# CouncilmanJeremyJamm/path_tracer

Hardware: AMD Instinct MI355X
Metric: Mray/s at 1920x1080, 256 spp; achieved HBM GB/s in traversal kernel (higher is better)
Workload: dtype f32; 1 GPU; Cornell box (36 triangles, 6 BLAS) 1920x1080, 256 spp, depth 8, NEE+MIS; parallelism=rows/1, bvh_in_lds=True, scene_bytes=4208

## Files before the change

include/pt_api.h:

```cpp
#ifndef PT_API_H
#define PT_API_H
#include <stdint.h>
#ifdef __cplusplus
extern "C" {
#endif

typedef struct pt_ctx pt_ctx;

enum pt_status
{
    PT_OK = 0,
    PT_ERR_ARG = -1,
    PT_ERR_HIP = -2,
    PT_ERR_STATE = -3,
    PT_ERR_NONRIGID = -4,
    PT_ERR_LIMIT = -5,
    PT_ERR_IO = -6,
    PT_ERR_PARSE = -7,
    PT_ERR_NCCL = -8
};

enum pt_material_kind
{
    PT_LAMBERTIAN = 0,
    PT_EMISSIVE = 1,
    PT_SPECULAR = 2,
    PT_GGX_METAL = 3,
    PT_GGX_DIELECTRIC = 4,
    PT_DIELECTRIC = 5
};

typedef struct pt_material_desc
{
    int32_t kind;
    float colour[3];
    float roughness;
    float ior;
    int32_t has_volume;
    float vol_absorption[3];
    float vol_k, vol_c, vol_g;
} pt_material_desc;

typedef struct pt_config
{
    uint32_t width, height;
    uint32_t max_bounces;
    uint32_t n_sobol;
    uint32_t enable_nee;
    uint64_t seed;
    uint32_t rank, world_size, strip_rows;
    uint32_t batch_spp;
    int32_t device;
    uint32_t flags;
    uint32_t stack_lds_levels;
    uint32_t queue_slack;
    uint32_t pipelines;
    uint32_t reserved;
} pt_config;

enum
{
    PT_FLAG_TIMING = 1u,
    PT_FLAG_NO_LDS_SCENE = 2u,
    PT_FLAG_TIMING_ALL = 4u,
    PT_FLAG_NO_PRIMARY_CULL = 8u
};

pt_ctx* pt_create(const pt_config* cfg);
void pt_destroy(pt_ctx* ctx);
const char* pt_last_error(pt_ctx* ctx);
int pt_set_config(pt_ctx* ctx, const pt_config* cfg);

int pt_add_material(pt_ctx* ctx, const pt_material_desc* desc);
int pt_add_model(pt_ctx* ctx, const float* positions_xyz, const float* normals_xyz, uint32_t n_tris, int material,
                 const float* affine3x4_rowmajor, uint32_t n_instances);
int pt_add_model_obj(pt_ctx* ctx, const char* path, int material, const float* affine3x4_rowmajor, uint32_t n_instances);
int pt_model_vertices(pt_ctx* ctx, int model, float* positions_xyz, float* normals_xyz, uint32_t cap_tris, uint32_t* n_tris);
int pt_build(pt_ctx* ctx);

int pt_set_camera(pt_ctx* ctx, const float eye[3], const float target[3], float fov_y_deg, float aspect);
enum pt_event { PT_EV_MOUSE_MOTION = 0, PT_EV_KEY_W = 1, PT_EV_KEY_S = 2, PT_EV_KEY_A = 3, PT_EV_KEY_D = 4 };
int pt_camera_input(pt_ctx* ctx, int event, float a, float b, float dt);
int pt_camera_angles(pt_ctx* ctx, float pitch_yaw[2]);
int pt_camera_matrices(pt_ctx* ctx, float cam_to_world_3x4[12], float inv_proj_4x4_colmajor[16]);
int pt_set_environment(pt_ctx* ctx, uint32_t width, uint32_t height, const float* rgb_linear);
int pt_create_ray(pt_ctx* ctx, float s, float t, float o[3], float d[3]);

int pt_render(pt_ctx* ctx, uint32_t first_sample, uint32_t n_samples, float* data_rgba, float* position_xyzt, uint32_t* id);
int pt_active_pixels(pt_ctx* ctx, uint32_t rect[4], float root_box[6]);
int pt_render_device(pt_ctx* ctx, uint32_t first_sample, uint32_t n_samples);
int pt_reset_accumulation(pt_ctx* ctx);
int pt_accum_device_ptr(pt_ctx* ctx, void** dev_ptr, uint64_t* n_pixels);
int pt_read_accumulation(pt_ctx* ctx, float* data_rgba);
int pt_read_frame(pt_ctx* ctx, float* data_rgba, float* position_xyzt, uint32_t* id);
int pt_write_accumulation(pt_ctx* ctx, const float* data_rgba, const float* position_xyzt, const uint32_t* id);
int pt_render_samples(pt_ctx* ctx, uint32_t first_sample, uint32_t n_samples, float* samples_rgba);
int pt_local_rows(pt_ctx* ctx, uint32_t* n_rows, uint32_t* rows, uint32_t cap);
int pt_set_stream(pt_ctx* ctx, void* hip_stream);
int pt_synchronize(pt_ctx* ctx);

int pt_frame(pt_ctx* ctx, uint32_t frame_index, const float* last_inv_projection, float* data_rgba, float* position_xyzt, uint32_t* id);
int pt_inv_projection(pt_ctx* ctx, float out16_colmajor[16]);
int pt_present(pt_ctx* ctx, float* rgba);
int pt_present_rgb8(pt_ctx* ctx, uint8_t* rgb);
int pt_write_image(pt_ctx* ctx, const char* path);
int pt_post_velocity(pt_ctx* ctx, uint32_t w, uint32_t h, const float* position, const float* last_inv_projection, float* velocity);
int pt_post_reproject(pt_ctx* ctx, uint32_t w, uint32_t h, const float* input, const float* accum, const float* velocity, const uint32_t* id,
                      float* output);
int pt_post_tonemap(pt_ctx* ctx, uint32_t w, uint32_t h, const float* accum, float* out);
int pt_post_rgb8(pt_ctx* ctx, uint32_t w, uint32_t h, const float* accum, uint8_t* rgb);

int pt_trace_closest(pt_ctx* ctx, int which, uint32_t n, const float* o_xyz, const float* d_xyz, const float* t_max, float* t,
                     float* u, float* v, uint32_t* inst, uint32_t* prim);
int pt_trace_any(pt_ctx* ctx, int which, uint32_t n, const float* o_xyz, const float* d_xyz, const float* t_max, uint8_t* hit);
int pt_ss_sobol(pt_ctx* ctx, uint32_t n_points, uint32_t n, const uint32_t* index, const uint32_t* seed, float* out_xy);
int pt_math_batch(pt_ctx* ctx, int fn, uint32_t n, const float* a, const float* b, float* out0, float* out1);
int pt_material_eval(pt_ctx* ctx, int material, uint32_t n, const float* incoming_xyz, const float* normal_xyz, const uint8_t* front,
                     const uint32_t* pixel, const uint32_t* sample, uint32_t draws_consumed, float* out9);
int pt_volume_eval(pt_ctx* ctx, int material, uint32_t n, const float* incoming_xyz, const float* t_max, const float* dist,
                   const uint32_t* pixel, const uint32_t* sample, uint32_t draws_consumed, float* out9);

int pt_blas_count(pt_ctx* ctx);
int pt_blas_dump(pt_ctx* ctx, int blas, uint32_t* n_nodes, uint32_t* root, float* boxes6, uint32_t* kind, uint32_t* a, uint32_t* b,
                 uint32_t* n_prim_ids, uint32_t* prim_ids, uint32_t cap_nodes, uint32_t cap_ids);
int pt_tlas_dump(pt_ctx* ctx, int which, uint32_t* n_nodes, uint32_t* root, float* boxes6, uint32_t* kind, uint32_t* a, uint32_t* b,
                 uint32_t cap_nodes);
int pt_tlas_instances(pt_ctx* ctx, int which, uint32_t* n, float* matrix12, float* inv_matrix12, uint32_t cap);
int pt_instance_materials(pt_ctx* ctx, int which, uint32_t* n, uint32_t* material, uint32_t* blas, uint32_t cap);
int pt_light_cdf(pt_ctx* ctx, uint32_t* n, float* pdf, float* cdf, uint32_t* blas, uint32_t* prim, float* max_weight, uint32_t cap);
int pt_triangle_dump(pt_ctx* ctx, int blas, uint32_t prim, float out36[36]);

typedef struct pt_multi pt_multi;
pt_multi* pt_multi_create(const pt_config* cfg, const int32_t* devices, uint32_t n_devices);
void pt_multi_destroy(pt_multi* m);
const char* pt_multi_last_error(pt_multi* m);
pt_ctx* pt_multi_ctx(pt_multi* m, uint32_t rank);
int pt_multi_render(pt_multi* m, uint32_t first_sample, uint32_t n_samples, float* data_rgba);
int pt_multi_framebuffer_device_ptr(pt_multi* m, void** dev_ptr);
int pt_multi_reset_accumulation(pt_multi* m);
int pt_multi_write_image(pt_multi* m, const char* path);
int pt_multi_used_rccl(pt_multi* m);

typedef struct pt_stats
{
    uint64_t rays_closest;
    uint64_t rays_any;
    uint64_t rays_light_closest;
    uint64_t paths;
    uint64_t launches_trace_closest;
    double ms_trace_closest;
    double ms_trace_any, ms_trace_light, ms_shade, ms_generate, ms_accumulate;
    double ms_total;
    uint64_t scene_bytes;
    uint32_t lds_scene;
    uint32_t stack_entries;
    uint64_t state_bytes;
    uint64_t rays_light_closest_traced;
    uint64_t rays_primary_culled;
} pt_stats;
int pt_get_stats(pt_ctx* ctx, pt_stats* out);
int pt_multi_get_stats(pt_multi* m, pt_stats* sum);
int pt_last_batch_counters(pt_ctx* ctx, uint32_t* rows16, uint32_t cap_rows, uint32_t* n_rows);
int pt_last_batch_shade_pids(pt_ctx* ctx, uint32_t qclass, uint32_t first, uint32_t count, uint32_t* pids);
int pt_last_batch_step_stats(pt_ctx* ctx, uint32_t* rows8, uint32_t cap_rows, uint32_t* n_rows);
int pt_reset_stats(pt_ctx* ctx);

#ifdef __cplusplus
}
#endif
#endif
```

path_tracer_amd/api.py:

```python
from __future__ import annotations

import ctypes as C
import os
from typing import Optional

import numpy as np

from . import build as _build
from .scene_desc import CameraDesc, SceneDesc

PT_OK = 0
FLAG_TIMING = 1
FLAG_NO_LDS_SCENE = 2
FLAG_TIMING_ALL = 4
FLAG_NO_PRIMARY_CULL = 8
DEFAULT_SEED = 0x5EED5EED

EXPORTS = [
    "pt_create", "pt_destroy", "pt_last_error", "pt_set_config", "pt_add_material", "pt_add_model", "pt_add_model_obj", "pt_model_vertices", "pt_build", "pt_set_camera",
    "pt_camera_matrices", "pt_set_environment", "pt_create_ray", "pt_render", "pt_render_device", "pt_reset_accumulation", "pt_accum_device_ptr",
    "pt_read_accumulation", "pt_read_frame", "pt_write_accumulation", "pt_render_samples", "pt_active_pixels", "pt_local_rows", "pt_set_stream", "pt_synchronize", "pt_camera_input", "pt_camera_angles", "pt_frame", "pt_inv_projection", "pt_present", "pt_post_velocity", "pt_post_reproject", "pt_post_tonemap", "pt_post_rgb8", "pt_present_rgb8", "pt_write_image", "pt_trace_closest", "pt_trace_any",
    "pt_ss_sobol", "pt_math_batch", "pt_material_eval", "pt_volume_eval", "pt_blas_count", "pt_blas_dump", "pt_tlas_dump", "pt_tlas_instances", "pt_instance_materials", "pt_light_cdf",
    "pt_triangle_dump", "pt_get_stats", "pt_reset_stats", "pt_last_batch_counters", "pt_last_batch_shade_pids", "pt_last_batch_step_stats",
    "pt_multi_create", "pt_multi_destroy", "pt_multi_last_error", "pt_multi_ctx", "pt_multi_render", "pt_multi_framebuffer_device_ptr",
    "pt_multi_reset_accumulation", "pt_multi_get_stats", "pt_multi_used_rccl", "pt_multi_write_image",
]


EV_MOUSE_MOTION, EV_KEY_W, EV_KEY_S, EV_KEY_A, EV_KEY_D = range(5)


class MaterialDesc(C.Structure):
    _fields_ = [("kind", C.c_int32), ("colour", C.c_float * 3), ("roughness", C.c_float), ("ior", C.c_float), ("has_volume", C.c_int32),
                ("vol_absorption", C.c_float * 3), ("vol_k", C.c_float), ("vol_c", C.c_float), ("vol_g", C.c_float)]


class Config(C.Structure):
    _fields_ = [("width", C.c_uint32), ("height", C.c_uint32), ("max_bounces", C.c_uint32), ("n_sobol", C.c_uint32),
                ("enable_nee", C.c_uint32), ("seed", C.c_uint64), ("rank", C.c_uint32), ("world_size", C.c_uint32),
                ("strip_rows", C.c_uint32), ("batch_spp", C.c_uint32), ("device", C.c_int32), ("flags", C.c_uint32),
                ("stack_lds_levels", C.c_uint32), ("queue_slack", C.c_uint32), ("pipelines", C.c_uint32), ("reserved", C.c_uint32)]


class Stats(C.Structure):
    _fields_ = [("rays_closest", C.c_uint64), ("rays_any", C.c_uint64), ("rays_light_closest", C.c_uint64), ("paths", C.c_uint64),
                ("launches_trace_closest", C.c_uint64), ("ms_trace_closest", C.c_double), ("ms_trace_any", C.c_double),
                ("ms_trace_light", C.c_double), ("ms_shade", C.c_double), ("ms_generate", C.c_double), ("ms_accumulate", C.c_double),
                ("ms_total", C.c_double), ("scene_bytes", C.c_uint64), ("lds_scene", C.c_uint32), ("stack_entries", C.c_uint32),
                ("state_bytes", C.c_uint64), ("rays_light_closest_traced", C.c_uint64), ("rays_primary_culled", C.c_uint64)]

    def as_dict(self):
        return {n: getattr(self, n) for n, _ in self._fields_}

    @property
    def rays(self):
        return self.rays_closest + self.rays_any + self.rays_light_closest


class PtError(RuntimeError):
    def __init__(self, code, msg):
        super().__init__(f"libptmi error {code}: {msg}")
        self.code = code


_lib = None


def lib():
    global _lib
    if _lib is None:
        path = os.environ.get("PTMI_LIB")
        if not path:
            path = _build.LIB_PATH
            if _build.is_stale():
                path = _build.build()
        try:
            import torch
        except ImportError:
            pass
        L = C.CDLL(path)
        vp, u32, f32p = C.c_void_p, C.c_uint32, C.c_void_p
        L.pt_create.restype = vp
        L.pt_create.argtypes = [C.POINTER(Config)]
        L.pt_destroy.argtypes = [vp]
        L.pt_last_error.restype = C.c_char_p
        L.pt_last_error.argtypes = [vp]
        L.pt_set_config.argtypes = [vp, C.POINTER(Config)]
        L.pt_add_material.argtypes = [vp, C.POINTER(MaterialDesc)]
        L.pt_add_model.argtypes = [vp, f32p, f32p, u32, C.c_int, f32p, u32]
        L.pt_add_model_obj.argtypes = [vp, C.c_char_p, C.c_int, f32p, u32]
        L.pt_model_vertices.argtypes = [vp, C.c_int, f32p, f32p, u32, C.POINTER(u32)]
        L.pt_build.argtypes = [vp]
        L.pt_set_camera.argtypes = [vp, C.POINTER(C.c_float), C.POINTER(C.c_float), C.c_float, C.c_float]
        L.pt_camera_matrices.argtypes = [vp, vp, vp]
        L.pt_set_environment.argtypes = [vp, u32, u32, vp]
        L.pt_create_ray.argtypes = [vp, C.c_float, C.c_float, vp, vp]
        L.pt_render.argtypes = [vp, u32, u32, vp, vp, vp]
        L.pt_render_device.argtypes = [vp, u32, u32]
        L.pt_active_pixels.argtypes = [vp, vp, vp]
        L.pt_reset_accumulation.argtypes = [vp]
        L.pt_accum_device_ptr.argtypes = [vp, C.POINTER(vp), C.POINTER(C.c_uint64)]
        L.pt_read_accumulation.argtypes = [vp, vp]
        L.pt_write_accumulation.argtypes = [vp, vp, vp, vp]
        L.pt_read_frame.argtypes = [vp, vp, vp, vp]
        L.pt_render_samples.argtypes = [vp, u32, u32, vp]
        L.pt_local_rows.argtypes = [vp, C.POINTER(u32), vp, u32]
        L.pt_set_stream.argtypes = [vp, vp]
        L.pt_synchronize.argtypes = [vp]
        L.pt_frame.argtypes = [vp, u32, vp, vp, vp, vp]
        L.pt_camera_input.argtypes = [vp, C.c_int, C.c_float, C.c_float, C.c_float]
        L.pt_camera_angles.argtypes = [vp, vp]
        L.pt_inv_projection.argtypes = [vp, vp]
        L.pt_present.argtypes = [vp, vp]
        L.pt_multi_create.restype = vp
        L.pt_multi_create.argtypes = [C.POINTER(Config), vp, u32]
        L.pt_multi_destroy.argtypes = [vp]
        L.pt_multi_last_error.restype = C.c_char_p
        L.pt_multi_last_error.argtypes = [vp]
        L.pt_multi_ctx.restype = vp
        L.pt_multi_ctx.argtypes = [vp, u32]
        L.pt_multi_render.argtypes = [vp, u32, u32, vp]
        L.pt_multi_framebuffer_device_ptr.argtypes = [vp, C.POINTER(vp)]
        L.pt_multi_reset_accumulation.argtypes = [vp]
        L.pt_multi_get_stats.argtypes = [vp, C.POINTER(Stats)]
        L.pt_multi_used_rccl.argtypes = [vp]
        L.pt_multi_write_image.argtypes = [vp, C.c_char_p]
        L.pt_post_velocity.argtypes = [vp, u32, u32, vp, vp, vp]
        L.pt_post_reproject.argtypes = [vp, u32, u32, vp, vp, vp, vp, vp]
        L.pt_post_tonemap.argtypes = [vp, u32, u32, vp, vp]
        L.pt_post_rgb8.argtypes = [vp, u32, u32, vp, vp]
        L.pt_present_rgb8.argtypes = [vp, vp]
        L.pt_write_image.argtypes = [vp, C.c_char_p]
# ... 440 lines not shown
```

path_tracer_amd/csrc/pt_api.cpp:

```cpp
#include "../../include/pt_api.h"

#include <hip/hip_runtime.h>

#include <algorithm>
#include <chrono>
#include <cmath>
#include <cstdio>
#include <cstdlib>
#include <cstring>
#include <mutex>
#include <string>
#include <vector>

#include "pt_kernels.h"
#include "pt_png.h"
#include "pt_scene.h"

using namespace pt;

#ifndef PT_SHADE_BLOCKS_PER_CU
#define PT_SHADE_BLOCKS_PER_CU 16
#endif
#ifndef PT_JOIN_LATE
#define PT_JOIN_LATE 0
// ... 7 lines not shown
#ifndef PT_SIDE_MIN_PATHS
#define PT_SIDE_MIN_PATHS (4u << 20)
#endif
#ifndef PT_SIDE_PRIORITY
#define PT_SIDE_PRIORITY 0
#endif
#ifndef PT_SPLIT_MIN_PATHS
#define PT_SPLIT_MIN_PATHS (24u << 20)
#endif
#ifndef PT_SPLIT_MIN_PATHS_LDS
#define PT_SPLIT_MIN_PATHS_LDS (24u << 20)
#endif
#ifndef PT_PIPES4_MIN_PATHS
#define PT_PIPES4_MIN_PATHS (~0ull)
#endif
#ifndef PT_PID_BLOCK
#define PT_PID_BLOCK 16
#endif
#ifndef PT_FUSED_TRACE
#define PT_FUSED_TRACE 1
#endif
#ifndef PT_TRACE_BLOCKS_PER_CU_MAX
#define PT_TRACE_BLOCKS_PER_CU_MAX 8
#endif

namespace {

enum TimeCat { T_GEN = 0, T_WORLD, T_ANY, T_LIGHT, T_SHADE, T_ACCUM, T_COUNT };

struct DevBuf
{
    void* p = nullptr;
    size_t bytes = 0;
};

}

struct pt_ctx
{
    pt_config cfg{};
    HostScene scene;
    std::string err;
    std::mutex mu;

    bool dev_ready = false;
    int device = 0;
    int n_cus = 256;
    hipStream_t own_stream = nullptr, stream = nullptr;
    hipEvent_t ev_start = nullptr;

    struct Pipe
    {
        hipStream_t own_stream = nullptr, side_stream = nullptr;
        hipEvent_t ev_fork = nullptr, ev_join = nullptr, ev_done = nullptr;
        size_t cap_paths = 0, cap_slots = 0, cap_slots_term = 0;
        uint32_t cap_rows = 0;
        std::vector<DevBuf> pool;
        WavefrontBuffers wb{};
        Counters* h_counters = nullptr;
        uint32_t* h_heads = nullptr;
        struct Ev { hipEvent_t a, b; int cat; };
        std::vector<Ev> ev_pool;
        size_t ev_used = 0;
        uint32_t slack_cfg = 0;
        uint32_t pixels_cfg = 0;
        size_t state_bytes = 0;
        bool busy = false;
        uint32_t busy_rows = 0;
        uint64_t busy_paths = 0, busy_culled = 0;
    };
    static constexpr int kMaxPipes = 4;
    Pipe pipe[kMaxPipes];
    hipStream_t pipe_stream(int i) const { return i == 0 ? stream : pipe[i].own_stream; }

    bool scene_uploaded = false;
    DevBuf d_spill;
    size_t spill_region_words = 0;
    DevBuf d_blob, d_tri_shade, d_tri_pos, d_tri_orig, d_materials, d_lights, d_env;
    std::vector<f4> h_env;
    uint32_t env_w = 0, env_h = 0;
    bool env_uploaded = false;
    SceneView sv{};
    bool lds_scene = false;
    uint32_t block_threads = 256, trace_blocks = 1024;
    bool class_present[Q_COUNT] = {true, false, false, false, false};

    std::vector<uint32_t> rows;
    uint32_t local_pixels = 0;
    uint32_t pad_rows = 0;
    uint64_t scene_version = 0;
    DevBuf d_accum, d_position, d_id;
    DevBuf d_input, d_velocity, d_output;

    pt_stats stats{};
    int last_pipe = 0;
};

namespace {

int fail(pt_ctx* c, int code, const std::string& msg)
{
    c->err = msg;
    return code;
}

#define HIPCHK(c, call)                                                                                       \
    do {                                                                                                      \
        hipError_t e__ = (call);                                                                              \
        if (e__ != hipSuccess) return fail((c), PT_ERR_HIP, std::string(#call) + ": " + hipGetErrorString(e__)); \
    } while (0)

void dev_free(DevBuf& b)
{
    if (b.p) (void)hipFree(b.p);
    b = DevBuf();
}
int dev_alloc(pt_ctx* c, DevBuf& b, size_t bytes)
{
    if (b.bytes >= bytes && b.p) return PT_OK;
    dev_free(b);
    bytes = std::max<size_t>(bytes, 16);
    HIPCHK(c, hipMalloc(&b.p, bytes));
    b.bytes = bytes;
    return PT_OK;
}

void compute_rows(pt_ctx* c)
{
    const pt_config& g = c->cfg;
    c->rows.clear();
    const uint32_t world = std::max(1u, g.world_size), strip = std::max(1u, g.strip_rows);
    for (uint32_t y = 0; y < g.height; ++y)
        if ((y / strip) % world == g.rank) c->rows.push_back(y);
    c->local_pixels = (uint32_t)c->rows.size() * g.width;
    uint32_t r0 = 0;
    for (uint32_t y = 0; y < g.height; ++y) r0 += ((y / strip) % world == 0u) ? 1u : 0u;
    c->pad_rows = r0;
}

int normalise_config(pt_ctx* c, const pt_config* in)
{
    pt_config g = *in;
    if (g.width == 0 || g.height == 0) return fail(c, PT_ERR_ARG, "width/height must be non-zero");
    if (g.n_sobol == 0) g.n_sobol = 512;
    if (g.world_size == 0) g.world_size = 1;
    if (g.strip_rows == 0) g.strip_rows = 4;
    if (g.rank >= g.world_size) return fail(c, PT_ERR_ARG, "rank >= world_size");
    if ((uint64_t)g.width * g.height > 0x7fffffffull) return fail(c, PT_ERR_ARG, "image too large");
    c->cfg = g;
    compute_rows(c);
    return PT_OK;
}

int ensure_device(pt_ctx* c)
{
    if (c->dev_ready)
    {
        HIPCHK(c, hipSetDevice(c->device));
        return PT_OK;
    }
    int n = 0;
    hipError_t e = hipGetDeviceCount(&n);
    if (e != hipSuccess || n == 0) return fail(c, PT_ERR_HIP, "no HIP device available (libptmi has no CPU path)");
    if (c->cfg.device >= 0) HIPCHK(c, hipSetDevice(c->cfg.device));
    HIPCHK(c, hipGetDevice(&c->device));
    hipDeviceProp_t prop;
    HIPCHK(c, hipGetDeviceProperties(&prop, c->device));
    c->n_cus = prop.multiProcessorCount > 0 ? prop.multiProcessorCount : 256;
    HIPCHK(c, hipStreamCreateWithFlags(&c->own_stream, hipStreamNonBlocking));
    HIPCHK(c, hipEventCreateWithFlags(&c->ev_start, hipEventDisableTiming));
    for (int i = 0; i < pt_ctx::kMaxPipes; ++i)
    {
        pt_ctx::Pipe& pp = c->pipe[i];
        if (i > 0) HIPCHK(c, hipStreamCreateWithFlags(&pp.own_stream, hipStreamNonBlocking));
        HIPCHK(c, hipStreamCreateWithFlags(&pp.side_stream, hipStreamNonBlocking));
        HIPCHK(c, hipEventCreateWithFlags(&pp.ev_fork, hipEventDisableTiming));
        HIPCHK(c, hipEventCreateWithFlags(&pp.ev_join, hipEventDisableTiming));
        HIPCHK(c, hipEventCreateWithFlags(&pp.ev_done, hipEventDisableTiming));
    }
    if (!c->stream) c->stream = c->own_stream;
    c->dev_ready = true;
    return PT_OK;
}

int upload_scene(pt_ctx* c)
{
    if (c->scene_uploaded) return ensure_device(c);
    if (!c->scene.built) return fail(c, PT_ERR_STATE, "pt_build has not been called");
    int r = ensure_device(c);
    if (r) return r;
    const FlatScene& f = c->scene.flat;
    const size_t nb = f.nodes.size() * sizeof(DNode), tb = f.tri_isect.size() * sizeof(DTriIsect), ib = f.instances.size() * sizeof(DInstance);
    const size_t lb = (f.big_leaves.size() * 4 + 15) / 16 * 16;
    std::vector<uint8_t> blob(nb + tb + ib + lb);
    std::memcpy(blob.data(), f.nodes.data(), nb);
    std::memcpy(blob.data() + nb, f.tri_isect.data(), tb);
    std::memcpy(blob.data() + nb + tb, f.instances.data(), ib);
    if (lb) std::memcpy(blob.data() + nb + tb + ib, f.big_leaves.data(), f.big_leaves.size() * 4);
    if ((r = dev_alloc(c, c->d_blob, blob.size()))) return r;
    HIPCHK(c, hipMemcpy(c->d_blob.p, blob.data(), blob.size(), hipMemcpyHostToDevice));
    auto up = [&](DevBuf& b, const void* src, size_t bytes) -> int {
        int rr = dev_alloc(c, b, bytes);
        if (rr) return rr;
        if (bytes) HIPCHK(c, hipMemcpy(b.p, src, bytes, hipMemcpyHostToDevice));
        return PT_OK;
    };
    if ((r = up(c->d_tri_shade, f.tri_shade.data(), f.tri_shade.size() * sizeof(DTriVerts)))) return r;
    if ((r = up(c->d_tri_pos, f.tri_pos.data(), f.tri_pos.size() * sizeof(DTriVerts)))) return r;
    if ((r = up(c->d_tri_orig, f.tri_orig.data(), f.tri_orig.size() * 4))) return r;
    if ((r = up(c->d_materials, f.materials.data(), f.materials.size() * sizeof(DMaterial)))) return r;
    if ((r = up(c->d_lights, f.lights.data(), f.lights.size() * sizeof(DLight)))) return r;

    SceneView& sv = c->sv;
    uint8_t* base = (uint8_t*)c->d_blob.p;
    sv.nodes = (const DNode*)base;
    sv.tri_isect = (const DTriIsect*)(base + nb);
    sv.instances = (const DInstance*)(base + nb + tb);
    sv.tri_shade = (const DTriVerts*)c->d_tri_shade.p;
    sv.tri_pos = (const DTriVerts*)c->d_tri_pos.p;
    sv.tri_orig = (const uint32_t*)c->d_tri_orig.p;
    sv.materials = (const DMaterial*)c->d_materials.p;
    sv.lights = (const DLight*)c->d_lights.p;
    sv.n_nodes = (uint32_t)f.nodes.size();
    sv.n_tris = (uint32_t)f.tri_isect.size();
    sv.n_instances = (uint32_t)f.instances.size();
    sv.n_materials = (uint32_t)f.materials.size();
    sv.n_lights = (uint32_t)f.lights.size();
    sv.world_root = f.world_root;
    sv.lights_root = f.lights_root;
    sv.prim_bits = f.prim_bits;
    sv.light_weight_sum = f.light_weight_sum;
    sv.blob_bytes = (uint32_t)blob.size();
    sv.stack_entries = f.stack_entries;
    sv.has_volumes = f.has_volumes ? 1u : 0u;

    c->lds_scene = blob.size() <= 48 * 1024 && !(c->cfg.flags & PT_FLAG_NO_LDS_SCENE);
    uint32_t threads = 256;
#ifndef PT_STACK_LDS_LEVELS
#define PT_STACK_LDS_LEVELS 14
#endif
    sv.stack_lds = std::min<uint32_t>(sv.stack_entries, c->cfg.stack_lds_levels ? c->cfg.stack_lds_levels : PT_STACK_LDS_LEVELS);
    auto lds_need = [&](uint32_t t) { return trace_lds_bytes(c->lds_scene, sv.blob_bytes, sv.stack_lds, t); };
    while (threads > 64 && lds_need(threads) > 64 * 1024) threads >>= 1;
    if (lds_need(threads) > 160 * 1024) return fail(c, PT_ERR_LIMIT, "BVH too deep for the LDS traversal stack");
    c->block_threads = threads;
    const size_t lds = lds_need(threads);
    uint32_t per_cu = (uint32_t)std::min<size_t>((160 * 1024) / std::max<size_t>(lds, 1), 2048 / threads);
    per_cu = std::max(1u, std::min(per_cu, (uint32_t)PT_TRACE_BLOCKS_PER_CU_MAX));
    c->trace_blocks = (uint32_t)c->n_cus * per_cu;
    sv.stack_spill = nullptr;
    if (sv.stack_entries > sv.stack_lds)
    {
        const size_t lanes = (size_t)c->trace_blocks * threads;
        c->spill_region_words = (size_t)(sv.stack_entries - sv.stack_lds) * lanes;
        if ((r = dev_alloc(c, c->d_spill, 2 * pt_ctx::kMaxPipes * c->spill_region_words * 8))) return r;
        sv.stack_spill = (uint64_t*)c->d_spill.p;
    }

    for (uint32_t q = 0; q < Q_COUNT; ++q) c->class_present[q] = (q == Q_TERMINAL);
    for (const DInstance& in : f.instances) c->class_present[in.qclass & 0xffu] = true;
    c->scene_uploaded = true;
    c->stats.scene_bytes = blob.size();
    c->stats.lds_scene = c->lds_scene;
    c->stats.stack_entries = sv.stack_entries;
    return PT_OK;
}

TraceLaunch trace_launch(pt_ctx* c, int pipe = 0, bool side_stream = false)
{
    TraceLaunch tl;
    tl.scene = c->sv;
    if (tl.scene.stack_spill) tl.scene.stack_spill += (size_t)(2 * pipe + (side_stream ? 1 : 0)) * c->spill_region_words;
    tl.blob = c->d_blob.p;
    tl.lds_scene = c->lds_scene;
    tl.grid_blocks = c->trace_blocks;
    tl.n_cus = (uint32_t)c->n_cus;
    tl.block_threads = c->block_threads;
    return tl;
}

struct ActiveRect { uint32_t x0, w, ly0, rows; };
ActiveRect active_rect(pt_ctx* c)
{
    const uint32_t W = c->cfg.width, H = c->cfg.height, local_rows = (uint32_t)c->rows.size();
    const ActiveRect full{0u, W, 0u, local_rows};
    if ((c->cfg.flags & PT_FLAG_NO_PRIMARY_CULL) || c->env_w || !c->scene.built || !c->scene.camera.set) return full;
    const FlatScene& f = c->scene.flat;
    if (f.world_root == MISS_ID || f.world_root >= f.nodes.size()) return full;
    const DNode& root = f.nodes[f.world_root];
    double m[16], inv[16];
    for (int i = 0; i < 16; ++i) m[i] = c->scene.camera.ray_matrix[i];
    {
        double a[4][8];
        for (int r = 0; r < 4; ++r)
            for (int k = 0; k < 4; ++k) { a[r][k] = m[k * 4 + r]; a[r][4 + k] = r == k ? 1.0 : 0.0; }
        for (int col = 0; col < 4; ++col)
        {
            int piv = col;
            for (int r = col + 1; r < 4; ++r)
                if (std::fabs(a[r][col]) > std::fabs(a[piv][col])) piv = r;
            if (std::fabs(a[piv][col]) < 1e-300) return full;
            for (int k = 0; k < 8; ++k) std::swap(a[col][k], a[piv][k]);
            const double d = a[col][col];
            for (int k = 0; k < 8; ++k) a[col][k] /= d;
            for (int r = 0; r < 4; ++r)
                if (r != col)
                {
                    const double fct = a[r][col];
                    for (int k = 0; k < 8; ++k) a[r][k] -= fct * a[col][k];
                }
        }
        for (int r = 0; r < 4; ++r)
            for (int k = 0; k < 4; ++k) inv[k * 4 + r] = a[r][4 + k];
    }
    const double eye[3] = {c->scene.camera.matrix.t.x, c->scene.camera.matrix.t.y, c->scene.camera.matrix.t.z};
    double ctr[4];
    for (int r = 0; r < 4; ++r) ctr[r] = m[12 + r];
    if (!(std::fabs(ctr[3]) > 1e-300)) return full;
    double fwd[3] = {ctr[0] / ctr[3] - eye[0], ctr[1] / ctr[3] - eye[1], ctr[2] / ctr[3] - eye[2]};
    const double fl = std::sqrt(fwd[0] * fwd[0] + fwd[1] * fwd[1] + fwd[2] * fwd[2]);
    if (!(fl > 0.0) || !std::isfinite(fl)) return full;
    double ext = 0.0;
    for (int k = 0; k < 3; ++k) { fwd[k] /= fl; ext = std::max(ext, std::fabs((double)root.mx[k] - (double)root.mn[k])); }
    double px_lo = 1e300, px_hi = -1e300, py_lo = 1e300, py_hi = -1e300;
    for (int corner = 0; corner < 8; ++corner)
    {
        const double X[3] = {corner & 1 ? root.mx[0] : root.mn[0], corner & 2 ? root.mx[1] : root.mn[1], corner & 4 ? root.mx[2] : root.mn[2]};
        if (!std::isfinite(X[0]) || !std::isfinite(X[1]) || !std::isfinite(X[2])) return full;
        const double depth = (X[0] - eye[0]) * fwd[0] + (X[1] - eye[1]) * fwd[1] + (X[2] - eye[2]) * fwd[2];
        if (!(depth > 1e-3 * ext + 1e-6)) return full;
        double q[4];
        for (int r = 0; r < 4; ++r) q[r] = inv[r] * X[0] + inv[4 + r] * X[1] + inv[8 + r] * X[2] + inv[12 + r];
        if (!(std::fabs(q[3]) > 1e-300)) return full;
        const double nx = q[0] / q[3], ny = q[1] / q[3];
        if (!std::isfinite(nx) || !std::isfinite(ny)) return full;
        const double px = (nx + 1.0) * 0.5 * W, py = (ny + 1.0) * 0.5 * H;
        px_lo = std::min(px_lo, px); px_hi = std::max(px_hi, px);
        py_lo = std::min(py_lo, py); py_hi = std::max(py_hi, py);
    }
    const double margin = 3.0;
    const double gx0 = std::floor(px_lo - 0.5 - margin), gx1 = std::ceil(px_hi + 0.5 + margin) + 1.0;
    const double gy0 = std::floor(py_lo - 0.5 - margin), gy1 = std::ceil(py_hi + 0.5 + margin) + 1.0;
    const uint32_t x0 = (uint32_t)std::min<double>(std::max(gx0, 0.0), W), x1 = (uint32_t)std::min<double>(std::max(gx1, 0.0), W);
    const uint32_t y0 = (uint32_t)std::min<double>(std::max(gy0, 0.0), H), y1 = (uint32_t)std::min<double>(std::max(gy1, 0.0), H);
    uint32_t ly0 = 0, n = 0;
    while (ly0 < local_rows && c->rows[ly0] < y0) ++ly0;
    while (ly0 + n < local_rows && c->rows[ly0 + n] < y1) ++n;
    return ActiveRect{x0, x1 > x0 ? x1 - x0 : 0u, ly0, n};
}

int ensure_frame(pt_ctx* c)
{
    int r;
    const size_t px = std::max<size_t>(std::max<size_t>(c->local_pixels, (size_t)c->pad_rows * c->cfg.width), 1);
    const bool fresh = c->d_accum.bytes < px * 16;
    if ((r = dev_alloc(c, c->d_accum, px * 16))) return r;
    if ((r = dev_alloc(c, c->d_position, px * 16))) return r;
// ... 1537 lines not shown
        std::lock_guard<std::mutex> lk(g_rccl_mu);
        std::string e;
        if (!g_rccl.load(&e)) return mfail(m, PT_ERR_NCCL, e);
        if (m->comms.empty())
        {
            m->comms.resize(n);
            const ncclResult_t nr = g_rccl.CommInitAll(m->comms.data(), (int)n, m->devices.data());
            if (nr != ncclSuccess) { m->comms.clear(); return mfail(m, PT_ERR_NCCL, std::string("ncclCommInitAll: ") + g_rccl.GetErrorString(nr)); }
        }
        ncclResult_t nr = g_rccl.GroupStart();
        for (size_t i = 0; i < n && nr == ncclSuccess; ++i)
        {
            pt_ctx* c = m->ctx[i];
            if (hipSetDevice(c->device) != hipSuccess) { nr = ncclUnhandledCudaError; break; }
            nr = g_rccl.Gather(c->d_accum.p, i == 0 ? m->d_parts.p : nullptr, part_px * 4, ncclFloat, 0, m->comms[i], c->stream);
        }
        const ncclResult_t ne = g_rccl.GroupEnd();
        if (nr == ncclSuccess) nr = ne;
        if (nr != ncclSuccess) return mfail(m, PT_ERR_NCCL, std::string("ncclGather: ") + g_rccl.GetErrorString(nr));
        m->used_rccl = true;
        for (size_t i = 1; i < n; ++i)
        {
            MHIPCHK(m, hipSetDevice(m->ctx[i]->device));
            MHIPCHK(m, hipStreamSynchronize(m->ctx[i]->stream));
        }
        MHIPCHK(m, hipSetDevice(c0->device));
    }
    else
    {
        for (size_t i = 0; i < n; ++i)
            MHIPCHK(m, hipMemcpyAsync((uint8_t*)m->d_parts.p + i * part_px * 16, m->ctx[i]->d_accum.p, part_px * 16, hipMemcpyDeviceToDevice, c0->stream));
    }
    launch_post_deinterleave(c0->stream, g.width, g.height, (uint32_t)n, g.strip_rows, c0->pad_rows, (const f4*)m->d_parts.p, (f4*)m->d_full.p);
    if (data_rgba) MHIPCHK(m, hipMemcpyAsync(data_rgba, m->d_full.p, full_px * 16, hipMemcpyDeviceToHost, c0->stream));
    MHIPCHK(m, hipStreamSynchronize(c0->stream));
    MHIPCHK(m, hipGetLastError());
    return PT_OK;
}

int pt_multi_write_image(pt_multi* m, const char* path)
{
    if (!m || !path) return PT_ERR_ARG;
    if (!m->d_full.p) return mfail(m, PT_ERR_STATE, "pt_multi_render has not been called");
    pt_ctx* c0 = m->ctx[0];
    const size_t px = (size_t)c0->cfg.width * c0->cfg.height;
    MHIPCHK(m, hipSetDevice(c0->device));
    DevBuf d_rgb;
    int r = dev_alloc(c0, d_rgb, px * 3);
    if (r) return mfail(m, r, pt_last_error(c0));
    launch_post_rgb8(c0->stream, (uint32_t)px, (const f4*)m->d_full.p, (uint8_t*)d_rgb.p);
    std::vector<uint8_t> host(px * 3);
    hipError_t e = hipMemcpyAsync(host.data(), d_rgb.p, px * 3, hipMemcpyDeviceToHost, c0->stream);
    if (e == hipSuccess) e = hipStreamSynchronize(c0->stream);
    dev_free(d_rgb);
    if (e != hipSuccess) return mfail(m, PT_ERR_HIP, hipGetErrorString(e));
    std::string err;
    if (!write_png_rgb8(path, host.data(), c0->cfg.width, c0->cfg.height, &err)) return mfail(m, PT_ERR_IO, err);
    return PT_OK;
}

int pt_multi_framebuffer_device_ptr(pt_multi* m, void** dev_ptr)
{
    if (!m || !dev_ptr) return PT_ERR_ARG;
    if (!m->d_full.p) return mfail(m, PT_ERR_STATE, "pt_multi_render has not been called");
    *dev_ptr = m->d_full.p;
    return PT_OK;
}

int pt_multi_get_stats(pt_multi* m, pt_stats* sum)
{
    if (!m || !sum) return PT_ERR_ARG;
    *sum = pt_stats();
    for (pt_ctx* c : m->ctx)
    {
        const pt_stats& s = c->stats;
        sum->rays_closest += s.rays_closest; sum->rays_any += s.rays_any; sum->rays_light_closest += s.rays_light_closest;
        sum->rays_light_closest_traced += s.rays_light_closest_traced; sum->rays_primary_culled += s.rays_primary_culled; sum->paths += s.paths;
        sum->launches_trace_closest += s.launches_trace_closest; sum->ms_trace_closest += s.ms_trace_closest;
        sum->ms_trace_any += s.ms_trace_any; sum->ms_trace_light += s.ms_trace_light; sum->ms_shade += s.ms_shade;
        sum->ms_generate += s.ms_generate; sum->ms_accumulate += s.ms_accumulate;
        sum->ms_total = std::max(sum->ms_total, s.ms_total);
        sum->state_bytes += s.state_bytes;
        sum->scene_bytes = s.scene_bytes; sum->lds_scene = s.lds_scene; sum->stack_entries = s.stack_entries;
    }
    return PT_OK;
}

int pt_get_stats(pt_ctx* c, pt_stats* out)
{
    if (!c || !out) return PT_ERR_ARG;
    *out = c->stats;
    return PT_OK;
}

int pt_last_batch_counters(pt_ctx* c, uint32_t* rows16, uint32_t cap_rows, uint32_t* n_rows)
{
    if (!c || !rows16 || !n_rows) return PT_ERR_ARG;
    const pt_ctx::Pipe& pp = c->pipe[c->last_pipe];
    if (!pp.h_counters || !pp.h_heads) return PT_ERR_STATE;
    const uint32_t rows = std::min(cap_rows, c->cfg.max_bounces + 2);
    const uint32_t have = std::min(rows, pp.busy_rows);
    std::memset(rows16, 0, (size_t)rows * sizeof(Counters));
    std::memcpy(rows16, pp.h_counters, (size_t)have * sizeof(Counters));
    for (uint32_t r = 0; r < have; ++r)
    {
        uint32_t* o = rows16 + 16 * r;
        o[1] = o[3] = o[5] = 0;
        o[6] = o[7] = o[13] = o[14] = o[15] = 0;
        const uint32_t* hrow = pp.h_heads + (size_t)r * HEADS_PER_ROW * kHeadWordsPerQueue;
        for (uint32_t g = 0; g < kQueueHeads; ++g)
        {
            const uint32_t* cl = hrow + HEADS_CLOSEST * kHeadWordsPerQueue + g * kHeadStrideWords;
            const uint32_t* sh = hrow + HEADS_SHADOW * kHeadWordsPerQueue + g * kHeadStrideWords;
            const uint32_t* lc = hrow + HEADS_LCHAIN * kHeadWordsPerQueue + g * kHeadStrideWords;
            o[6] += lc[HEAD_TALLY0]; o[7] += lc[HEAD_TALLY1]; o[13] += cl[HEAD_TALLY0]; o[14] += sh[HEAD_TALLY0]; o[15] += lc[HEAD_TALLY2];
        }
    }
    *n_rows = rows;
    return PT_OK;
}

int pt_last_batch_shade_pids(pt_ctx* c, uint32_t qclass, uint32_t first, uint32_t count, uint32_t* pids)
{
    if (!c || !pids || qclass == Q_TERMINAL || qclass >= Q_COUNT) return PT_ERR_ARG;
    const pt_ctx::Pipe& pp = c->pipe[c->last_pipe];
    if (!pp.wb.q_shade_base || !((pp.wb.class_mask >> qclass) & 1u)) return PT_ERR_STATE;
    if ((uint64_t)first + count > pp.wb.q_stride) return PT_ERR_ARG;
    HIPCHK(c, hipSetDevice(c->device));
    const ShadeQueue q = shade_queue(pp.wb, qclass);
    HIPCHK(c, hipMemcpy2D(pids, 4, reinterpret_cast<const uint8_t*>(q.a + first) + 12, 16, 4, count, hipMemcpyDeviceToHost));
    return PT_OK;
}

int pt_last_batch_step_stats(pt_ctx* c, uint32_t* rows8, uint32_t cap_rows, uint32_t* n_rows)
{
    if (!c || !rows8 || !n_rows) return PT_ERR_ARG;
    const pt_ctx::Pipe& pp = c->pipe[c->last_pipe];
    if (!pp.h_heads) return PT_ERR_STATE;
    const uint32_t rows = std::min(cap_rows, c->cfg.max_bounces + 2);
#if PT_WAVE_TIMES
    {
        std::vector<uint32_t> rec((size_t)rows * kWaveTimeSlots * 4);
        const char* which = std::getenv("PTMI_WAVE_TIMES_KERNEL");
        const uint4* src = (which && which[0] == 'a') ? pp.wb.wave_times_any : pp.wb.wave_times;
        if (hipMemcpy(rec.data(), src, rec.size() * 4, hipMemcpyDeviceToHost) != hipSuccess) return PT_ERR_HIP;
        for (uint32_t r = 0; r < rows; ++r)
        {
            uint32_t* o = rows8 + 8 * r;
            std::memset(o, 0, 32);
            uint32_t t0 = 0; bool any = false;
            for (uint32_t w = 0; w < kWaveTimeSlots; ++w)
            {
                const uint32_t* q = &rec[((size_t)r * kWaveTimeSlots + w) * 4];
                if (q[3] == 0u) continue;
                if (!any || (int32_t)(q[0] - t0) < 0) t0 = q[0];
                any = true;
            }
            if (!any) continue;
            uint32_t max_end = 0, min_dr = 0xffffffffu, max_dr = 0;
            for (uint32_t w = 0; w < kWaveTimeSlots; ++w)
            {
                const uint32_t* q = &rec[((size_t)r * kWaveTimeSlots + w) * 4];
                if (q[3] == 0u) continue;
                max_end = std::max(max_end, q[3] - t0);
                min_dr = std::min(min_dr, q[2] - t0);
                max_dr = std::max(max_dr, q[2] - t0);
                o[2] += q[3] - q[0];
                o[3] += q[2] - q[0];
                o[4] += 1u;
                o[7] += q[1] - q[0];
            }
            o[0] = ~t0; o[1] = t0 + max_end; o[5] = ~(t0 + min_dr); o[6] = t0 + max_dr;
            if (std::getenv("PTMI_WAVE_TIMES_DUMP"))
            {
// ... 46 lines not shown
```

path_tracer_amd/csrc/pt_kernels.h:

```cpp
#pragma once
#include <hip/hip_runtime.h>

#include "pt_materials.h"
#include "pt_types.h"

namespace pt {

struct TraceLaunch
{
    SceneView scene;
    const void* blob;
    bool lds_scene;
    uint32_t grid_blocks;
    uint32_t n_cus;
    uint32_t block_threads;
};

inline size_t trace_lds_bytes(bool lds_scene, uint32_t blob_bytes, uint32_t stack_lds, uint32_t block_threads)
{
    return (lds_scene ? (size_t)blob_bytes : 0) + (size_t)stack_lds * block_threads * 8;
}
inline size_t trace_lds_bytes(const TraceLaunch& tl) { return trace_lds_bytes(tl.lds_scene, tl.scene.blob_bytes, tl.scene.stack_lds, tl.block_threads); }

struct WavefrontBuffers
{
    PathState st;
    RayQueue rq[2];
    RayQueue rq_shadow;
    RayQueue rq_lchain[2];
    f4* lchain_nb[2];
    f4* lchain_hit;
    f4* hits;
    f4* q_shade_base;
    uint32_t q_stride;
    uint32_t q_class_slot;
    uint2* q_term[2];
    Counters* counters;
    uint32_t* heads;
    uint4* wave_times;
    uint4* wave_times_any;
    uint32_t* tails;
    uint32_t cap_slots;
    uint32_t cap_slots_shade;
    uint32_t cap_slots_term;
    uint32_t class_mask;
};

inline ShadeQueue shade_queue(const WavefrontBuffers& wb, uint32_t q)
{
    const size_t slot = (wb.q_class_slot >> (4u * q)) & 0xfu;
    f4* a = wb.q_shade_base + 3u * slot * (size_t)wb.q_stride;
    return ShadeQueue{a, a + wb.q_stride, a + 2u * (size_t)wb.q_stride};
}

void launch_generate(hipStream_t s, const RenderParams& rp, const CameraView& cam, const WavefrontBuffers& wb);
void launch_trace_world(hipStream_t s, const TraceLaunch& tl, const WavefrontBuffers& wb, uint32_t b, const RenderParams& rp, const CameraView& cam,
                        const EnvView& env);
void launch_trace_fused(hipStream_t s, const TraceLaunch& tl, const WavefrontBuffers& wb, uint32_t b, const RenderParams& rp, const EnvView& env);
void launch_trace_shadow(hipStream_t s, const TraceLaunch& tl, const WavefrontBuffers& wb, uint32_t b);
void launch_trace_lchain(hipStream_t s, const TraceLaunch& tl, const WavefrontBuffers& wb, uint32_t b);
void launch_shade(hipStream_t s, uint32_t qclass, const SceneView& sv, const RenderParams& rp, const WavefrontBuffers& wb, uint32_t b,
                  uint32_t grid_blocks, const CameraView& cam, const EnvView& env, const TraceLaunch* tl = nullptr);
bool shade_traces_shadow(const TraceLaunch& tl);
void launch_accumulate(hipStream_t s, const RenderParams& rp, const CameraView& cam, const WavefrontBuffers& wb, f4* accum, f4* position, uint32_t* id,
                       uint32_t write_position, uint32_t add_to_accum);
void launch_store_samples(hipStream_t s, const RenderParams& rp, const WavefrontBuffers& wb, f4* out);

void launch_post_accumulate(hipStream_t s, uint32_t n, const f4* input, f4* accum);
void launch_post_velocity(hipStream_t s, int w, int h, const f4* position, const float* m16, float* velocity_xy);
void launch_post_reproject(hipStream_t s, int w, int h, const f4* input, const f4* accum, const float* velocity_xy, const uint32_t* id, f4* output);
void launch_post_tonemap(hipStream_t s, uint32_t n, const f4* accum, f4* out);
void launch_post_rgb8(hipStream_t s, uint32_t n, const f4* accum, uint8_t* out);
void launch_post_deinterleave(hipStream_t s, uint32_t w, uint32_t h, uint32_t world, uint32_t strip, uint32_t pad_rows, const f4* parts, f4* full);

void launch_trace_rays_closest(hipStream_t s, const TraceLaunch& tl, uint32_t root, RayQueue rq, uint32_t n, uint32_t* n_and_heads, f4* hits);
void launch_trace_rays_any(hipStream_t s, const TraceLaunch& tl, uint32_t root, RayQueue rq, uint32_t n, uint32_t* n_and_heads, uint32_t* occluded);
void launch_sobol_probe(hipStream_t s, uint32_t n_points, uint32_t n, const uint32_t* index, const uint32_t* seed, float* out_xy);
void launch_math_probe(hipStream_t s, int fn, uint32_t n, const float* a, const float* b, float* o0, float* o1, uint64_t seed);
void launch_material_probe(hipStream_t s, const SceneView& sv, int material, uint32_t n, const float* incoming, const float* normal,
                           const uint8_t* front, const uint32_t* pixel, const uint32_t* sample, uint32_t draws, uint64_t seed, float* out9);
void launch_volume_probe(hipStream_t s, const SceneView& sv, int material, uint32_t n, const float* incoming, const float* t_max, const float* dist,
                         const uint32_t* pixel, const uint32_t* sample, uint32_t draws, uint64_t seed, float* out9);

}
```

path_tracer_amd/csrc/pt_kernels.hip:

```cpp
#include "pt_kernels.h"
#include "pt_materials.h"

#include <algorithm>
#include <mutex>
#include <vector>

namespace pt {
namespace {

#ifndef PT_STEPS_PER_ROUND
#define PT_STEPS_PER_ROUND 8
#endif
#ifndef PT_REFILL_BELOW
#define PT_REFILL_BELOW 40
#endif
#ifndef PT_STEPS_PER_ROUND_GLOBAL_BVH
#define PT_STEPS_PER_ROUND_GLOBAL_BVH 4
#endif
#ifndef PT_REFILL_BELOW_GLOBAL_BVH
#define PT_REFILL_BELOW_GLOBAL_BVH 56
#endif
#ifndef PT_STEPS_ANY
#define PT_STEPS_ANY 4
#endif
#ifndef PT_REFILL_BELOW_ANY
#define PT_REFILL_BELOW_ANY PT_REFILL_BELOW
#endif
#ifndef PT_WAVES_LDS_BVH
#define PT_WAVES_LDS_BVH 5
#endif
#ifndef PT_WAVES_LDS_BVH_ANY
#define PT_WAVES_LDS_BVH_ANY 5
#endif
#ifndef PT_WAVES_GLOBAL_BVH
#define PT_WAVES_GLOBAL_BVH 5
#endif
#ifndef PT_WAVES_GLOBAL_BVH_ANY
#define PT_WAVES_GLOBAL_BVH_ANY 5
#endif
#ifndef PT_BRANCH_LEVELS
#define PT_BRANCH_LEVELS 4
#endif
#ifndef PT_BRANCH_LEVELS_ANY
#define PT_BRANCH_LEVELS_ANY 4
#endif
#ifndef PT_BRANCH_LEVELS_INLINE
#define PT_BRANCH_LEVELS_INLINE 6
#endif
#ifndef PT_ACC_QUAD_BELOW
#define PT_ACC_QUAD_BELOW (1u << 30)
#endif
#ifndef PT_STEP_STATS
#define PT_STEP_STATS 0
#endif
#ifndef PT_WAVE_TIMES
#define PT_WAVE_TIMES 0
#endif
#ifndef PT_MIN_GENERATIONS
#define PT_MIN_GENERATIONS 1
#endif
#ifndef PT_STRIPE_DIV
#define PT_STRIPE_DIV 64
#endif
#ifndef PT_REGIONS_PER_STRIPE
#define PT_REGIONS_PER_STRIPE 256
#endif
#ifndef PT_REGION_DIV
#define PT_REGION_DIV 16
#endif
#ifndef PT_TAPER
#define PT_TAPER 2
#endif
#ifndef PT_TAPER_ANY
#define PT_TAPER_ANY 0
#endif
#ifndef PT_RESERVICE
#define PT_RESERVICE 1
#endif
#ifndef PT_CLAIM_AHEAD
#define PT_CLAIM_AHEAD 0
#endif
#ifndef PT_SHADE_WAVES
#define PT_SHADE_WAVES 5
#endif
#ifndef PT_SHADE_WAVES_DIEL
#define PT_SHADE_WAVES_DIEL 5
#endif
#ifndef PT_SHADE_WAVES_GGX
#define PT_SHADE_WAVES_GGX 5
#endif
#ifndef PT_SHADE_WAVES_VOLUMES
#define PT_SHADE_WAVES_VOLUMES 4
#endif
constexpr int shade_waves(uint32_t qclass, bool volumes)
{
    return volumes ? PT_SHADE_WAVES_VOLUMES : (qclass == Q_GGX ? PT_SHADE_WAVES_GGX : (qclass == Q_DIELECTRIC ? PT_SHADE_WAVES_DIEL : PT_SHADE_WAVES));
}
#ifndef PT_INLINE_SHADOW
#define PT_INLINE_SHADOW 1
#endif
#ifndef PT_SHADE_WAVES_INLINE
#define PT_SHADE_WAVES_INLINE 5
#endif
#ifndef PT_SHADE_THREADS
#define PT_SHADE_THREADS 256
#endif
#ifndef PT_CHUNK_MAX
#define PT_CHUNK_MAX 1024
#endif
#ifndef PT_CHUNK_DIV
#define PT_CHUNK_DIV 4
#endif
#ifndef PT_CHUNK_DIV_GLOBAL_BVH
#define PT_CHUNK_DIV_GLOBAL_BVH 16
#endif
template <bool LDS_SCENE> struct Refill
{
    static constexpr int kSteps = LDS_SCENE ? PT_STEPS_PER_ROUND : PT_STEPS_PER_ROUND_GLOBAL_BVH;
    static constexpr int kStepsAny = LDS_SCENE ? PT_STEPS_ANY : PT_STEPS_PER_ROUND_GLOBAL_BVH;
    static constexpr int kBelow = LDS_SCENE ? PT_REFILL_BELOW : PT_REFILL_BELOW_GLOBAL_BVH;
    static constexpr int kBelowAny = LDS_SCENE ? PT_REFILL_BELOW_ANY : PT_REFILL_BELOW_GLOBAL_BVH;
};

__device__ __forceinline__ uint32_t fastdiv(uint32_t n, const FastDiv& f)
{
    const uint32_t q = __umulhi(f.magic, n);
    const uint32_t t = ((n - q) >> 1) + q;
    return f.one ? n : (t >> f.shift);
}
__device__ __forceinline__ uint32_t lane_id() { return threadIdx.x & 63u; }
__device__ __forceinline__ uint32_t mbcnt64(uint64_t m)
{
    return __builtin_amdgcn_mbcnt_hi((uint32_t)(m >> 32), __builtin_amdgcn_mbcnt_lo((uint32_t)m, 0u));
}
struct FetchPlan
{
    uint32_t n;
    uint32_t chunk;
    uint32_t n_static;
    uint32_t psize;
    uint32_t lvl;
    uint32_t blocks;
};
__device__ __forceinline__ bool chunk_of(const FetchPlan& pl, uint32_t i, uint32_t& start, uint32_t& len)
{
    uint32_t rem = pl.psize, base = 0u;
    const uint32_t e64 = min(rem, pl.lvl); rem -= e64;
    const uint32_t e128 = min(rem, 2u * pl.lvl); rem -= e128;
    const uint32_t e256 = min(rem, 4u * pl.lvl); rem -= e256;
    const uint32_t e512 = min(rem, 8u * pl.lvl); rem -= e512;
    const uint32_t e1024 = rem;
#define PT_LEVEL(E, C)                                                                                     \
    {                                                                                                      \
        const uint32_t c = min((uint32_t)(C), pl.chunk), cnt = ((E) + c - 1u) / c;                          \
        if (i < cnt) { start = base + i * c; len = min(c, (E) - i * c); return true; }                      \
        i -= cnt;                                                                                          \
        base += (E);                                                                                       \
    }
    PT_LEVEL(e1024, 1024u) PT_LEVEL(e512, 512u) PT_LEVEL(e256, 256u) PT_LEVEL(e128, 128u) PT_LEVEL(e64, 64u)
#undef PT_LEVEL
    return false;
}
__device__ __forceinline__ FetchPlan fetch_plan(uint32_t n, uint32_t chunk_div, uint32_t taper)
{
    FetchPlan pl;
    const uint32_t wpb = blockDim.x >> 6;
    const uint32_t need_waves = (n + 63u) >> 6;
    pl.blocks = min(gridDim.x, (need_waves + wpb * (uint32_t)PT_MIN_GENERATIONS - 1u) / (wpb * (uint32_t)PT_MIN_GENERATIONS));
    const uint32_t waves = max(pl.blocks, 1u) * wpb;
    uint32_t c = n / (waves * chunk_div);
    c = c < 64u ? 64u : (c > (uint32_t)PT_CHUNK_MAX ? (uint32_t)PT_CHUNK_MAX : c);
    pl.chunk = (c + 63u) & ~63u;
    pl.n = n;
    const uint64_t st = (uint64_t)waves * pl.chunk;
    pl.n_static = st >= n ? n : (uint32_t)st;
    const uint32_t units = (n - pl.n_static + 63u) >> 6;
    pl.psize = ((units + kQueueHeads - 1u) / kQueueHeads) << 6;
    pl.lvl = taper ? ((taper * waves * 64u / kQueueHeads + 63u) & ~63u) : 0u;
    return pl;
}
struct WaveRange
{
// ... 250 lines not shown
    td = -dot4(f4{mo.x, mo.y, mo.z, -1.0f}, n0);
    const bool out_t = sign_differs(td - det * t_min, det * t_mx - td);
    const f3 p = det * mo + td * d;
    const f4 p4{p.x, p.y, p.z, det};
    ud = dot4(p4, f4{asf(p1.x), asf(p1.y), asf(p1.z), asf(p1.w)});
    const bool out_u = sign_differs(ud, det - ud);
    vd = dot4(p4, f4{asf(p2.x), asf(p2.y), asf(p2.z), asf(p2.w)});
    const bool out_v = sign_differs(vd, det - ud - vd);
    return !(out_t | out_u | out_v);
}

struct TriEval { float td, ud, vd, det; bool uv_ok; };
__device__ __forceinline__ TriEval tri_eval(const uint4* tp, const f3 mo, const f3 d)
{
    TriEval e;
    const uint4 p0 = tp[0], p1 = tp[1], p2 = tp[2];
    const f4 n0{asf(p0.x), asf(p0.y), asf(p0.z), asf(p0.w)};
    e.det = dot3(d, xyz(n0));
    e.td = -dot4(f4{mo.x, mo.y, mo.z, -1.0f}, n0);
    const f3 p = e.det * mo + e.td * d;
    const f4 p4{p.x, p.y, p.z, e.det};
    e.ud = dot4(p4, f4{asf(p1.x), asf(p1.y), asf(p1.z), asf(p1.w)});
    e.vd = dot4(p4, f4{asf(p2.x), asf(p2.y), asf(p2.z), asf(p2.w)});
    const bool out_u = sign_differs(e.ud, e.det - e.ud), out_v = sign_differs(e.vd, e.det - e.ud - e.vd);
    e.uv_ok = !out_u && !out_v;
    return e;
}
__device__ __forceinline__ bool tri_in_range(const TriEval& e, float t_min, float t_mx) { return !sign_differs(e.td - e.det * t_min, e.det * t_mx - e.td); }

struct Blob
{
    const uint4* nodes;
    const uint4* tris;
    const uint4* inst;
    const uint2* leaves;
};
__device__ __forceinline__ void leaf_range(const Blob& bl, uint32_t kind, uint32_t payload, uint32_t& first, uint32_t& count)
{
    if (kind == NODE_TRIS) { first = payload & LEAF_FIRST_MASK; count = (payload >> LEAF_FIRST_BITS) + 1u; }
    else { const uint2 lf = bl.leaves[payload]; first = lf.x; count = lf.y; }
}

struct LaneRay { f3 o, d, inv; };

__device__ __forceinline__ void pin(uint4& v) { asm volatile("" : "+v"(v.x), "+v"(v.y), "+v"(v.z), "+v"(v.w)); }
template <bool EAGER, bool ROOT_BOX>
__device__ __forceinline__ LaneRay to_object(const Blob& bl, uint32_t inst, const LaneRay& w, bool ray_finite, uint4& root0, uint4& root1)
{
    const uint4* ip = bl.inst + INST_WORDS * inst;
    uint4 r0, r1, r2;
    if (EAGER)
    {
        r0 = ip[0]; r1 = ip[1]; r2 = ip[2];
    }
    const uint4 meta = ip[INST_META_WORD];
    if (ROOT_BOX) { root0 = ip[INST_ROOT_WORD]; root1 = ip[INST_ROOT_WORD + 1u]; }
    else root0.w = reinterpret_cast<const uint32_t*>(ip + INST_ROOT_WORD)[3];
    if (EAGER) { pin(r0); pin(r1); pin(r2); }
    LaneRay r;
    if ((meta.w & INSTANCE_IDENTITY) != 0u && ray_finite)
    {
        const uint32_t so = asu(w.o.x) & asu(w.o.y) & asu(w.o.z) & 0x80000000u;
        const uint32_t sd = asu(w.d.x) & asu(w.d.y) & asu(w.d.z) & 0x80000000u;
        r.o.x = w.o.x != 0.0f ? w.o.x : asf(so);
        r.o.y = w.o.y != 0.0f ? w.o.y : asf(so);
        r.o.z = w.o.z != 0.0f ? w.o.z : asf(so);
        r.d.x = w.d.x != 0.0f ? w.d.x : asf(sd);
        r.d.y = w.d.y != 0.0f ? w.d.y : asf(sd);
        r.d.z = w.d.z != 0.0f ? w.d.z : asf(sd);
        r.inv.x = w.d.x != 0.0f ? w.inv.x : asf(sd | 0x7f800000u);
        r.inv.y = w.d.y != 0.0f ? w.inv.y : asf(sd | 0x7f800000u);
        r.inv.z = w.d.z != 0.0f ? w.inv.z : asf(sd | 0x7f800000u);
        return r;
    }
    if (!EAGER) { r0 = ip[0]; r1 = ip[1]; r2 = ip[2]; }
    r.o.x = ((asf(r0.x) * w.o.x + asf(r0.y) * w.o.y) + asf(r0.z) * w.o.z) + asf(r0.w);
    r.o.y = ((asf(r1.x) * w.o.x + asf(r1.y) * w.o.y) + asf(r1.z) * w.o.z) + asf(r1.w);
    r.o.z = ((asf(r2.x) * w.o.x + asf(r2.y) * w.o.y) + asf(r2.z) * w.o.z) + asf(r2.w);
    r.d.x = (asf(r0.x) * w.d.x + asf(r0.y) * w.d.y) + asf(r0.z) * w.d.z;
    r.d.y = (asf(r1.x) * w.d.x + asf(r1.y) * w.d.y) + asf(r1.z) * w.d.z;
    r.d.z = (asf(r2.x) * w.d.x + asf(r2.y) * w.d.y) + asf(r2.z) * w.d.z;
    r.inv = rcp3(r.d);
    return r;
}

template <bool LDS_SCENE>
__device__ __forceinline__ Blob stage_scene(const SceneView& sv, const uint4* __restrict__ gblob, uint4* smem, uint32_t& words)
{
    Blob b;
    const uint4* base = gblob;
    words = 0;
    if (LDS_SCENE)
    {
        words = sv.blob_bytes >> 4;
        for (uint32_t i = threadIdx.x; i < words; i += blockDim.x) smem[i] = gblob[i];
        __syncthreads();
        base = smem;
    }
    b.nodes = base;
    b.tris = base + 2u * sv.n_nodes;
    b.inst = base + 2u * sv.n_nodes + 3u * sv.n_tris;
    b.leaves = reinterpret_cast<const uint2*>(base + 2u * sv.n_nodes + 3u * sv.n_tris + INST_WORDS * sv.n_instances);
    return b;
}

enum { CLOSEST_WORLD = 0, CLOSEST_LIGHTS = 1, CLOSEST_HOOK = 2, CLOSEST_PRIMARY = 3 };

struct ClosestOut
{
    f4* hits;
    f4* q_base;
    uint32_t q_stride, q_class_slot;
    uint2* q_term;
    uint32_t* n_shade;
    uint4* wave_times;
    uint32_t* tails;
    uint32_t cap_shade, cap_term;
    uint32_t class_mask;
    uint32_t* overflow;
    uint32_t world_root;
    uint8_t* occl;
    f3 eye;
    f4* radiance;
    f4* first_pos;
    uint32_t* first_id;
    uint32_t keep_s_id, keep_s_pos, blk_log, n_blk, blk_last, act_pixels;
    FastDiv div_blk_paths, div_blk_last;
    uint32_t finalize_miss;
    const DPathRec* rec;
    uint32_t enable_nee;
};

template <bool SPILL>
struct Stack8;
template <>
struct Stack8<false>
{
    char* base;
    uint32_t bottom, step;
    __device__ __forceinline__ static Stack8 make(uint4* smem, uint32_t blob_words, const SceneView&)
    {
        return Stack8{reinterpret_cast<char*>(smem), blob_words * 16u + threadIdx.x * 8u, blockDim.x * 8u};
    }
    __device__ __forceinline__ uint32_t empty() const { return bottom; }
    __device__ __forceinline__ uint32_t up(uint32_t sp) const { return sp + step; }
    __device__ __forceinline__ uint32_t down(uint32_t sp) const { return sp - step; }
    __device__ __forceinline__ uint2 get(uint32_t sp) const { return *reinterpret_cast<const uint2*>(base + sp); }
    __device__ __forceinline__ void put(uint32_t sp, uint2 v) const { *reinterpret_cast<uint2*>(base + sp) = v; }
};
template <>
struct Stack8<true>
{
    uint2* lds;
    uint2* spill;
    uint32_t stride, lds_levels, spill_stride;
    __device__ __forceinline__ static Stack8 make(uint4* smem, uint32_t blob_words, const SceneView& sv)
    {
        return Stack8{reinterpret_cast<uint2*>(smem + blob_words) + threadIdx.x,
                      reinterpret_cast<uint2*>(sv.stack_spill) + (blockIdx.x * blockDim.x + threadIdx.x), blockDim.x, sv.stack_lds, gridDim.x * blockDim.x};
    }
    __device__ __forceinline__ uint32_t empty() const { return 0u; }
    __device__ __forceinline__ uint32_t up(uint32_t sp) const { return sp + 1u; }
    __device__ __forceinline__ uint32_t down(uint32_t sp) const { return sp - 1u; }
    __device__ __forceinline__ uint2 get(uint32_t sp) const
    {
        uint2 v;
        if (sp < lds_levels) v = lds[__umul24(sp, stride)];
        else v = spill[(size_t)(sp - lds_levels) * spill_stride];
        return v;
    }
    __device__ __forceinline__ void put(uint32_t sp, uint2 v) const
    {
        if (sp < lds_levels) lds[__umul24(sp, stride)] = v;
        else spill[(size_t)(sp - lds_levels) * spill_stride] = v;
    }
};

#if PT_WAVE_TIMES
__device__ uint4* g_any_times = nullptr;
#endif
struct ClosestKArgs
{
    SceneView sv;
    const uint4* gblob;
    const f4* ra;
    const f4* rb;
    const uint32_t* n_ptr;
    uint32_t* heads;
    uint32_t root, cap_in;
    ClosestOut out;
};
typedef const __attribute__((address_space(4))) ClosestKArgs* ClosestKArgsPtr;
typedef const __attribute__((address_space(4))) ClosestOut* ClosestOutPtr;
__device__ __forceinline__ ClosestOutPtr launder_args(ClosestOutPtr p)
{
    asm volatile("" : "+s"(p));
    return p;
}
template <int BVH, int MODE, bool SPILL>
__device__ __forceinline__ void closest_body(const SceneView& sv, const Blob& bl, const uint32_t blob_words, uint4* smem, const uint32_t root, const f4* __restrict__ ra,
                                             const f4* __restrict__ rb, const uint32_t* __restrict__ n_ptr, const uint32_t cap_in,
                                             uint32_t* __restrict__ heads, const ClosestOutPtr outp)
{
    constexpr bool LDS_SCENE = BVH != 0;
    const FetchPlan plan = fetch_plan(min(*n_ptr, cap_in), LDS_SCENE ? (uint32_t)PT_CHUNK_DIV : (uint32_t)PT_CHUNK_DIV_GLOBAL_BVH, (uint32_t)PT_TAPER);
    if (blockIdx.x >= plan.blocks) return;
    const Stack8<SPILL> stk = Stack8<SPILL>::make(smem, blob_words, sv);
    const uint32_t prim_bits = sv.prim_bits;

    bool active = false, pending = false, ray_finite = false;
    uint32_t ray_idx = 0, pid = 0;
    LaneRay w{}, ob{};
    float t_max = 0.0f, bt = 0.0f;
    float hud = 0.0f, hvd = 0.0f, hdet = 1.0f;
    uint32_t bid = MISS_ID, sp = stk.empty(), blas_base = 0, inst = 0;
    bool in_blas = false;
    bool any_phase = false;
    uint32_t chain_code = 0u;
    WaveRange wr = first_range(plan, heads);
    uint32_t light_hits = 0, valid_rays = 0;
#if PT_STEP_STATS
    uint32_t st_iter = 0, st_lane_active = 0, st_lane_inst = 0, st_lane_branch = 0, st_lane_leaf = 0, st_wave_inst = 0, st_wave_branch = 0, st_wave_leaf = 0;
#endif
#if PT_WAVE_TIMES
    const uint32_t tw_start = (uint32_t)wall_clock64();
    uint32_t tw_first = 0u, tw_drained = 0u;
#endif
    Region bin_region[Q_COUNT];
#pragma unroll
    for (uint32_t c = 0; c < Q_COUNT; ++c) bin_region[c] = Region{0u, 0u};
    const uint32_t lights_world_root = MODE == CLOSEST_LIGHTS ? outp->world_root : 0u;
    const uint32_t rsize = outp->finalize_miss != 0u ? 64u : region_size(plan.n, plan.blocks * (blockDim.x >> 6), 64u);
    const Stripes stripes = stripes_for(plan.n);
    uint32_t stripe_rot = blockIdx.x * (blockDim.x >> 6) + __builtin_amdgcn_readfirstlane(threadIdx.x >> 6);

    for (;;)
    {
        uint64_t act = __ballot(active);
        const bool no_more = wr.drained && wr.cur >= wr.end;
#if PT_WAVE_TIMES
        if (no_more && tw_drained == 0u) tw_drained = (uint32_t)wall_clock64() | 1u;
#endif
        const bool service = no_more ? (act == 0ull) : (__popcll(act) <= Refill<LDS_SCENE>::kBelow);
        if (service)
        {
            const ClosestOutPtr out = launder_args(outp);
            const uint64_t pm = __ballot(pending);
            if (pm != 0ull)
            {
                if (MODE == CLOSEST_WORLD || MODE == CLOSEST_PRIMARY)
                {
                    uint64_t qm = pm;
                    if (MODE == CLOSEST_PRIMARY)
                    {
                        const bool missed = pending && bid == MISS_ID && out->finalize_miss != 0u;
                        if (pending) out->occl[ray_idx] = missed ? (uint8_t)PRIMARY_MISS : (uint8_t)0u;
                        if (!missed && pending && bid == MISS_ID)
                        {
                            const FastDiv dbp{out->div_blk_paths.magic, out->div_blk_paths.shift, out->div_blk_paths.one, out->div_blk_paths.d};
                            const FastDiv dbl{out->div_blk_last.magic, out->div_blk_last.shift, out->div_blk_last.one, out->div_blk_last.d};
                            const uint32_t b = fastdiv(ray_idx, dbp), rem = ray_idx - b * (out->act_pixels << out->blk_log);
                            const bool short_blk = b + 1u == out->n_blk;
                            const uint32_t k = short_blk ? fastdiv(rem, dbl) : (rem >> out->blk_log);
                            const uint32_t sl = (b << out->blk_log) + (rem - k * (short_blk ? out->blk_last : (1u << out->blk_log)));
                            if (sl >= out->keep_s_id) out->first_id[(sl - out->keep_s_id) * out->act_pixels + k] = 255u;
                            if (sl == out->keep_s_pos)
                            {
                                const f3 far = fma3(w.d, bc3(1e5f), w.o);
                                out->first_pos[k] = f4{far.x, far.y, far.z, 1e5f};
                            }
                        }
                        qm = __ballot(pending && !missed);
                        pending = pending && !missed;
                    }
                    if (MODE == CLOSEST_WORLD)
                    {
                        bool ends = false, emissive = false;
                        uint32_t mat_id = 0;
                        if (pending)
                        {
                            if (bid == MISS_ID) ends = out->finalize_miss != 0u;
                            else
                            {
                                const uint4 meta = bl.inst[INST_WORDS * (bid >> prim_bits) + INST_META_WORD];
                                emissive = ends = (meta.w & 0xffu) == (uint32_t)Q_TERMINAL;
                                mat_id = meta.z;
                            }
                        }
                        if (ends)
                        {
                            const DPathRec& rec = out->rec[pid];
                            const f4 acc4 = rec.acc;
                            const uint32_t flags = asu(acc4.w);
                            if (!(flags & FLAG_BSDF_CAST))
                            {
                                f3 acc = xyz(acc4);
                                if (flags & FLAG_NEE_PENDING) acc = acc + xyz(rec.nee_pw) * (xyz(rec.nee_e) + f3{0.0f, 0.0f, 0.0f});
                                const f3 pw = xyz(rec.pw);
                                if (!emissive) acc = acc + f3{0.006f, 0.006f, 0.006f} * pw;
                                else if (!out->enable_nee || (flags & FLAG_LAST_DELTA))
                                {
                                    const DMaterial& m = sv.materials[mat_id];
                                    acc = fma3(f3{m.colour[0], m.colour[1], m.colour[2]}, pw, acc);
                                }
                                out->radiance[pid] = f4{acc.x, acc.y, acc.z, 0.0f};
                                pending = false;
                            }
                        }
                        qm = __ballot(pending);
                    }
                    if (qm != 0ull)
                    {
                        uint32_t cls = Q_COUNT;
                        if (pending) cls = bid != MISS_ID ? (bl.inst[INST_WORDS * (bid >> prim_bits) + INST_META_WORD].w & 0xffu) : (uint32_t)Q_TERMINAL;
                        const f4 hit{bt, hud / hdet, hvd / hdet, asf(bid)};
#pragma unroll
                        for (uint32_t c = 0; c < Q_COUNT; ++c)
                        {
                            if (!((out->class_mask >> c) & 1u)) continue;
                            const uint64_t m = __ballot(cls == c);
                            if (m == 0ull) continue;
                            const Placement pl = c == Q_TERMINAL
                                ? wave_reserve(bin_region[c], out->n_shade + c, (uint32_t)__popcll(m), rsize, out->cap_term, out->overflow)
                                : wave_reserve_striped(bin_region[c], out->tails + c * kTailWordsPerQueue, stripes, stripe_rot, (uint32_t)__popcll(m), out->cap_shade, out->overflow);
                            if (cls == c)
                            {
                                const uint32_t pos = place(pl, mbcnt64(m));
                                if (c == Q_TERMINAL)
                                {
                                    out->hits[ray_idx] = hit;
                                    out->q_term[pos] = make_uint2(ray_idx, pid);
                                }
                                else
                                {
                                    f4* const qa = out->q_base + (size_t)(3u * ((out->q_class_slot >> (4u * c)) & 0xfu)) * out->q_stride + pos;
                                    nt_store(qa, f4{w.d.x, w.d.y, w.d.z, asf(pid)});
                                    nt_store(qa + out->q_stride, hit);
                                    if (MODE != CLOSEST_PRIMARY) nt_store(qa + 2u * (size_t)out->q_stride, f4{w.o.x, w.o.y, w.o.z, 0.0f});
                                }
                            }
                        }
                    }
                }
                else if (MODE == CLOSEST_LIGHTS)
                {
                    if (pending)
                    {
                        out->occl[pid] = (uint8_t)chain_code;
                        if (chain_code == 0u) out->hits[ray_idx] = f4{bt, hud / hdet, hvd / hdet, asf(bid)};
                    }
                }
                else
                {
                    if (pending) out->hits[ray_idx] = f4{bt, hud / hdet, hvd / hdet, asf(bid)};
                }
                pending = false;
            }
            if (no_more) break;
            const uint64_t idle = ~act;
            uint32_t first;
            const uint32_t take = claim_rays(wr, heads, plan, (uint32_t)__popcll(idle), first);
            const uint32_t rank = mbcnt64(idle);
            if (!active && rank < take)
            {
                const uint32_t mine = first + rank;
                const f4 b = rb[mine];
                ray_idx = mine;
                pid = asu(b.w);
                if (pid != HOLE) {
                valid_rays += 1u;
                if (MODE == CLOSEST_PRIMARY)
                {
                    w.o = f3{out->eye.x, out->eye.y, out->eye.z};
                    t_max = asf(0x7f800000u);
                }
                else
                {
                    const f4 a = ra[mine];
                    w.o = xyz(a);
                    t_max = a.w;
                }
                w.d = xyz(b);
                w.inv = rcp3(w.d);
                ray_finite = finite3(w.o) && finite3(w.d);
                bid = MISS_ID;
                any_phase = false;
                chain_code = 2u;
                bt = asf(0x7f800000u);
                hud = 0.0f;
                hvd = 0.0f;
                hdet = 1.0f;
                in_blas = false;
                sp = stk.empty();
                float te;
                const uint4 root0 = bl.nodes[2u * root];
                const bool ok = (t_max == t_max) && slab(root0, bl.nodes[2u * root + 1u], w.o, w.inv, t_max, te);
                if (ok)
                {
                    stk.put(sp, make_uint2(root0.w, 0u));
                    sp = stk.up(sp);
                    active = true;
                }
                else { pending = true; }
                }
            }
#if PT_WAVE_TIMES
            if (tw_first == 0u && take != 0u) tw_first = (uint32_t)wall_clock64() | 1u;
#endif
            act = __ballot(active);
            if (act == 0ull) continue;
            if (PT_RESERVICE && take < (uint32_t)__popcll(idle) && !wr.drained && (uint32_t)__popcll(act) <= (uint32_t)Refill<LDS_SCENE>::kBelow) continue;
        }

#pragma unroll 1
        for (int it = 0; it < Refill<LDS_SCENE>::kSteps; ++it)
        {
#if PT_STEP_STATS
            {
                const uint64_t am = __ballot(active);
                if (am != 0ull) { st_iter += 1u; st_lane_active += (uint32_t)__popcll(am); }
            }
#endif
            if (!active) continue;
            if (in_blas && sp == blas_base) in_blas = false;
            if (MODE == CLOSEST_LIGHTS && any_phase)
            {
                if (sp == stk.empty()) { active = false; pending = true; chain_code = 0u; continue; }
                sp = stk.down(sp);
                const uint2 e = stk.get(sp);
                uint32_t link = e.x;
                float t_enter = asf(e.y);
                if ((link >> NODE_KIND_SHIFT) == NODE_INSTANCE)
                {
                    uint4 r0, r1;
                    ob = to_object<!LDS_SCENE, true>(bl, link & NODE_PAYLOAD_MASK, w, ray_finite, r0, r1);
                    in_blas = true;
                    blas_base = sp;
                    if (!slab(r0, r1, ob.o, ob.inv, t_max, t_enter)) continue;
                    link = r0.w;
                }
                const uint32_t kkind = link >> NODE_KIND_SHIFT, kpay = link & NODE_PAYLOAD_MASK;
                if (kkind == NODE_BRANCH)
                {
                    const uint4* cp = bl.nodes + 2u * kpay;
                    const uint4 l0 = cp[0], l1 = cp[1], r0 = cp[2], r1 = cp[3];
                    const f3 so = in_blas ? ob.o : w.o, sinv = in_blas ? ob.inv : w.inv;
                    float tl, tr;
                    const bool hl = slab(l0, l1, so, sinv, t_max, tl);
                    const bool hr = slab(r0, r1, so, sinv, t_max, tr);
                    if (hl) { stk.put(sp, make_uint2(l0.w, asu(tl))); sp = stk.up(sp); }
                    if (hr) { stk.put(sp, make_uint2(r0.w, asu(tr))); sp = stk.up(sp); }
                }
                else
                {
                    uint32_t first, count;
                    leaf_range(bl, kkind, kpay, first, count);
                    for (uint32_t k = 0; k < count; ++k)
                    {
                        const uint4* tp = bl.tris + 3u * (first + k);
                        float td, ud, vd, det;
                        if (tri_planes(tp[0], tp[1], tp[2], ob.o, ob.d, t_max, t_enter, td, ud, vd, det))
                        {
                            active = false;
                            pending = true;
                            chain_code = 1u;
                            break;
                        }
                    }
                }
                continue;
            }
            if (sp == stk.empty())
            {
                if (MODE == CLOSEST_LIGHTS && bid != MISS_ID)
                {
                    light_hits += 1u;
                    any_phase = true;
                    in_blas = false;
                    t_max = bt * (1.0f - PT_EPSILON);
                    float te = 0.0f;
                    const uint4 wr0 = bl.nodes[2u * lights_world_root];
                    if (t_max == t_max && slab(wr0, bl.nodes[2u * lights_world_root + 1u], w.o, w.inv, t_max, te)) { stk.put(sp, make_uint2(wr0.w, asu(te))); sp = stk.up(sp); }
                    else { active = false; pending = true; chain_code = 0u; }
                    continue;
                }
                active = false;
                pending = true;
                continue;
            }
            sp = stk.down(sp);
            const uint2 e = stk.get(sp);
            if (asf(e.y) > t_max) continue;
            uint32_t link = e.x;
            float t_est = asf(e.y);
#if PT_STEP_STATS
            { const bool x = (link >> NODE_KIND_SHIFT) == NODE_INSTANCE; const uint64_t m = __ballot(x); st_lane_inst += x ? 1u : 0u; if (m != 0ull && lane_id() == (uint32_t)__builtin_ctzll(m)) st_wave_inst += 1u; }
#endif
            if ((link >> NODE_KIND_SHIFT) == NODE_INSTANCE)
            {
                uint4 root0, root1;
                inst = link & NODE_PAYLOAD_MASK;
                ob = to_object<!LDS_SCENE, false>(bl, inst, w, ray_finite, root0, root1);
                in_blas = true;
                blas_base = sp;
                if (0.0f > t_max) continue;
                link = root0.w;
                t_est = 0.0f;
            }
            uint32_t kind = link >> NODE_KIND_SHIFT, payload = link & NODE_PAYLOAD_MASK;
#if PT_STEP_STATS
            { const bool x = kind == NODE_BRANCH; const uint64_t m = __ballot(x); st_lane_branch += x ? 1u : 0u; if (m != 0ull && lane_id() == (uint32_t)__builtin_ctzll(m)) st_wave_branch += 1u; }
#endif
#pragma unroll 1
            for (int lvl = 0; lvl < PT_BRANCH_LEVELS && kind == NODE_BRANCH; ++lvl)
            {
                const uint4* cp = bl.nodes + 2u * payload;
                const uint4 l0 = cp[0], l1 = cp[1], r0 = cp[2], r1 = cp[3];
                const f3 o = in_blas ? ob.o : w.o, inv = in_blas ? ob.inv : w.inv;
                float tl, tr;
                const bool hl = slab(l0, l1, o, inv, t_max, tl);
                const bool hr = slab(r0, r1, o, inv, t_max, tr);
                const bool left_near = tl < tr;
                const uint2 le = make_uint2(l0.w, asu(tl)), re = make_uint2(r0.w, asu(tr));
                if (hl && hr) { stk.put(sp, left_near ? re : le); sp = stk.up(sp); }
                kind = NODE_INSTANCE;
                if (hl || hr)
                {
                    const uint2 near = (hl && (left_near || !hr)) ? le : re;
                    const uint32_t nk = near.x >> NODE_KIND_SHIFT;
                    if ((nk & 1u) != 0u || (nk == NODE_BRANCH && lvl + 1 < PT_BRANCH_LEVELS))
                    {
                        kind = nk;
                        payload = near.x & NODE_PAYLOAD_MASK;
                        t_est = asf(near.y);
                    }
                    else { stk.put(sp, near); sp = stk.up(sp); }
                }
            }
#if PT_STEP_STATS
            { const bool x = (kind & 1u) != 0u; const uint64_t m = __ballot(x); st_lane_leaf += x ? 1u : 0u; if (m != 0ull && lane_id() == (uint32_t)__builtin_ctzll(m)) st_wave_leaf += 1u; }
#endif
            if (kind & 1u)
            {
                uint32_t first, count;
                leaf_range(bl, kind, payload, first, count);
                const f3 mo = fma3(ob.d, bc3(t_est), ob.o);
                const float t_min = PT_EPSILON - t_est;
                auto accept = [&](const TriEval& e, uint32_t tri) {
                    if (e.uv_ok && tri_in_range(e, t_min, t_max - t_est))
                    {
                        bt = e.td / e.det + t_est;
                        hud = e.ud;
                        hvd = e.vd;
                        hdet = e.det;
                        t_max = bt;
                        bid = (inst << prim_bits) | tri;
                    }
                };
                for (uint32_t k = 0; k < count; ++k) accept(tri_eval(bl.tris + 3u * (first + k), mo, ob.d), first + k);
                if (bt != bt) { sp = stk.empty(); in_blas = false; }
            }
        }
    }
    if (MODE == CLOSEST_WORLD || MODE == CLOSEST_PRIMARY)
    {
        const ClosestOutPtr out = launder_args(outp);
        const f4 hole{0.0f, 0.0f, 0.0f, asf(HOLE)};
        for (uint32_t i = bin_region[Q_TERMINAL].cur + lane_id(); i < bin_region[Q_TERMINAL].end; i += 64u) out->q_term[i] = make_uint2(HOLE, 0u);
#pragma unroll
        for (uint32_t c = 1; c < Q_COUNT; ++c)
        {
            f4* const qa = out->q_base + (size_t)(3u * ((out->q_class_slot >> (4u * c)) & 0xfu)) * out->q_stride;
            for (uint32_t i = bin_region[c].cur + lane_id(); i < bin_region[c].end; i += 64u) qa[i] = hole;
        }
    }
#if PT_WAVE_TIMES
    if (lane_id() == 0u && outp->wave_times)
    {
        const uint32_t tw_end = (uint32_t)wall_clock64();
        if (tw_drained == 0u) tw_drained = tw_end;
        if (tw_first == 0u) tw_first = tw_start;
        const uint32_t wave = blockIdx.x * (blockDim.x >> 6) + (threadIdx.x >> 6);
        if (wave < kWaveTimeSlots) outp->wave_times[wave] = make_uint4(tw_start, tw_first, tw_drained, tw_end | 1u);
    }
#endif
#if PT_STEP_STATS
    {
        const uint32_t wave = blockIdx.x * (blockDim.x >> 6) + (threadIdx.x >> 6);
        uint32_t* line = heads + ((wave * 7u) & (kQueueHeads - 1u)) * kHeadStrideWords;
        if (lane_id() == 0u) { atomicAdd(line + 8, st_iter); atomicAdd(line + 9, st_lane_active); }
        uint32_t a = st_lane_inst, b = st_lane_branch, c2 = st_lane_leaf;
        for (int off = 32; off > 0; off >>= 1) { a += __shfl_xor(a, off); b += __shfl_xor(b, off); c2 += __shfl_xor(c2, off); }
        if (lane_id() == 0u) { atomicAdd(line + 10, a); atomicAdd(line + 11, b); atomicAdd(line + 12, c2); }
        a = st_wave_inst; b = st_wave_branch; c2 = st_wave_leaf;
        for (int off = 32; off > 0; off >>= 1) { a += __shfl_xor(a, off); b += __shfl_xor(b, off); c2 += __shfl_xor(c2, off); }
        if (lane_id() == 0u) { atomicAdd(line + 13, a); atomicAdd(line + 14, b); atomicAdd(line + 15, c2); }
    }
#endif
    if (MODE != CLOSEST_HOOK) add_tally(heads, valid_rays, HEAD_TALLY0);
    if (MODE == CLOSEST_LIGHTS) add_tally(heads, light_hits, HEAD_TALLY1);
}
template <int BVH, int MODE, bool SPILL>
__global__ void __launch_bounds__(256, BVH != 0 ? PT_WAVES_LDS_BVH : PT_WAVES_GLOBAL_BVH) k_closest(const ClosestKArgs a)
{
    constexpr bool LDS_SCENE = BVH != 0;
    extern __shared__ uint4 smem[];
    if (blockIdx.x >= fetch_plan(min(*a.n_ptr, a.cap_in), LDS_SCENE ? (uint32_t)PT_CHUNK_DIV : (uint32_t)PT_CHUNK_DIV_GLOBAL_BVH, (uint32_t)PT_TAPER).blocks) return;
    uint32_t blob_words;
    const Blob bl = stage_scene<LDS_SCENE>(a.sv, a.gblob, smem, blob_words);
    const ClosestOutPtr outp = &((ClosestKArgsPtr)__builtin_amdgcn_kernarg_segment_ptr())->out;
    closest_body<BVH, MODE, SPILL>(a.sv, bl, blob_words, smem, a.root, a.ra, a.rb, a.n_ptr, a.cap_in, a.heads, outp);
}

enum { ANY_SHADOW = 0, ANY_HOOK = 2 };

template <int BVH, int MODE, bool SPILL>
__device__ __forceinline__ void any_body(const SceneView& sv, const Blob& bl, const uint32_t blob_words, uint4* smem, const uint32_t root, const f4* __restrict__ ra,
                                         const f4* __restrict__ rb, const uint32_t* __restrict__ n_ptr, const uint32_t cap_in,
                                         uint32_t* __restrict__ heads, uint32_t* __restrict__ occluded,
                                         f4* __restrict__ radiance)
{
    constexpr bool LDS_SCENE = BVH != 0;
    const FetchPlan plan = fetch_plan(min(*n_ptr, cap_in), LDS_SCENE ? (uint32_t)PT_CHUNK_DIV : (uint32_t)PT_CHUNK_DIV_GLOBAL_BVH, (uint32_t)PT_TAPER_ANY);
    if (blockIdx.x >= plan.blocks) return;
    const Stack8<SPILL> stk = Stack8<SPILL>::make(smem, blob_words, sv);

    bool active = false, ray_finite = false;
    uint32_t out_idx = 0, valid_rays = 0;
    LaneRay w{}, ob{};
    float t_max = 0.0f;
    uint32_t sp = stk.empty(), blas_base = 0;
    bool path_ends = false;
    auto put_result_at = [&](uint32_t idx, bool ends, uint32_t v) {
        if (MODE == ANY_SHADOW)
        {
            DPathRec* rec = reinterpret_cast<DPathRec*>(occluded) + idx;
            if (ends)
            {
                const f3 e = v != 0u ? f3{0.0f, 0.0f, 0.0f} : xyz(rec->nee_e);
                const f3 acc = xyz(rec->acc) + xyz(rec->nee_pw) * (e + f3{0.0f, 0.0f, 0.0f});
                radiance[idx] = f4{acc.x, acc.y, acc.z, 0.0f};
            }
            else if (v != 0u)
            {
                float* e = reinterpret_cast<float*>(&rec->nee_e);
                e[0] = 0.0f; e[1] = 0.0f; e[2] = 0.0f;
            }
        }
        else occluded[idx] = v;
    };
    auto put_result = [&](uint32_t v) { put_result_at(out_idx, path_ends, v); };
    bool in_blas = false;
#if PT_WAVE_TIMES
    const uint32_t tw_start = (uint32_t)wall_clock64();
    uint32_t tw_drained = 0u;
#endif
#if PT_STEP_STATS
    uint32_t st_iter = 0, st_lane_active = 0, st_lane_inst = 0, st_lane_branch = 0, st_lane_leaf = 0, st_wave_inst = 0, st_wave_branch = 0, st_wave_leaf = 0;
#endif
    WaveRange wr = first_range(plan, heads);

    for (;;)
    {
        uint64_t act = __ballot(active);
        const bool no_more = wr.drained && wr.cur >= wr.end;
#if PT_WAVE_TIMES
        if (no_more && tw_drained == 0u) tw_drained = (uint32_t)wall_clock64() | 1u;
#endif
        const bool service = no_more ? (act == 0ull) : (__popcll(act) <= Refill<LDS_SCENE>::kBelowAny);
        if (service)
        {
            if (no_more) break;
            const uint64_t idle = ~act;
            uint32_t first;
            const uint32_t take = claim_rays(wr, heads, plan, (uint32_t)__popcll(idle), first);
            const uint32_t rank = mbcnt64(idle);
            if (!active && rank < take)
            {
                const uint32_t mine = first + rank;
                const f4 a = ra[mine], b = rb[mine];
                const uint32_t tag = asu(b.w);
                if (tag != HOLE) {
                valid_rays += 1u;
                path_ends = MODE == ANY_SHADOW && (tag & PATH_ENDS) != 0u;
                out_idx = (MODE == ANY_HOOK) ? mine : (tag & ~PATH_ENDS);
                w.o = xyz(a);
                w.d = xyz(b);
                w.inv = rcp3(w.d);
                ray_finite = finite3(w.o) && finite3(w.d);
                t_max = a.w;
                in_blas = false;
                sp = stk.empty();
                float te;
                const uint4 root0 = bl.nodes[2u * root];
                const bool ok = (t_max == t_max) && slab(root0, bl.nodes[2u * root + 1u], w.o, w.inv, t_max, te);
                if (ok)
                {
                    stk.put(sp, make_uint2(root0.w, asu(te)));
                    sp = stk.up(sp);
                    active = true;
                }
                else put_result(0u);
                }
            }
            act = __ballot(active);
            if (act == 0ull) continue;
            if (PT_RESERVICE && take < (uint32_t)__popcll(idle) && !wr.drained && (uint32_t)__popcll(act) <= (uint32_t)Refill<LDS_SCENE>::kBelowAny) continue;
        }

#pragma unroll 1
        for (int it = 0; it < Refill<LDS_SCENE>::kStepsAny; ++it)
        {
#if PT_STEP_STATS
            {
                const uint64_t am = __ballot(active);
                if (am != 0ull) { st_iter += 1u; st_lane_active += (uint32_t)__popcll(am); }
            }
#endif
            if (!active) continue;
            if (in_blas && sp == blas_base) in_blas = false;
            if (sp == stk.empty())
            {
                active = false;
                put_result(0u);
                continue;
            }
            sp = stk.down(sp);
            const uint2 e = stk.get(sp);
            uint32_t link = e.x;
            float t_enter = asf(e.y);
#if PT_STEP_STATS
            { const bool x = (link >> NODE_KIND_SHIFT) == NODE_INSTANCE; const uint64_t m = __ballot(x); st_lane_inst += x ? 1u : 0u; if (m != 0ull && lane_id() == (uint32_t)__builtin_ctzll(m)) st_wave_inst += 1u; }
#endif
            if ((link >> NODE_KIND_SHIFT) == NODE_INSTANCE)
            {
                uint4 r0, r1;
                ob = to_object<!LDS_SCENE, true>(bl, link & NODE_PAYLOAD_MASK, w, ray_finite, r0, r1);
                in_blas = true;
                blas_base = sp;
                if (!slab(r0, r1, ob.o, ob.inv, t_max, t_enter)) continue;
                link = r0.w;
            }
            uint32_t kind = link >> NODE_KIND_SHIFT, payload = link & NODE_PAYLOAD_MASK;
#if PT_STEP_STATS
            { const bool x = kind == NODE_BRANCH; const uint64_t m = __ballot(x); st_lane_branch += x ? 1u : 0u; if (m != 0ull && lane_id() == (uint32_t)__builtin_ctzll(m)) st_wave_branch += 1u; }
#endif
#pragma unroll 1
            for (int lvl = 0; lvl < PT_BRANCH_LEVELS_ANY && kind == NODE_BRANCH; ++lvl)
            {
                const uint4* cp = bl.nodes + 2u * payload;
                const uint4 l0 = cp[0], l1 = cp[1], r0 = cp[2], r1 = cp[3];
                const f3 o = in_blas ? ob.o : w.o, inv = in_blas ? ob.inv : w.inv;
                float tl, tr;
                const bool hl = slab(l0, l1, o, inv, t_max, tl);
                const bool hr = slab(r0, r1, o, inv, t_max, tr);
                if (hl && hr) { stk.put(sp, make_uint2(l0.w, asu(tl))); sp = stk.up(sp); }
                kind = NODE_INSTANCE;
                if (hl || hr)
                {
                    const uint2 next = hr ? make_uint2(r0.w, asu(tr)) : make_uint2(l0.w, asu(tl));
                    const uint32_t nk = next.x >> NODE_KIND_SHIFT;
                    if ((nk & 1u) != 0u || (nk == NODE_BRANCH && lvl + 1 < PT_BRANCH_LEVELS_ANY))
                    {
                        kind = nk;
                        payload = next.x & NODE_PAYLOAD_MASK;
                        t_enter = asf(next.y);
                    }
                    else { stk.put(sp, next); sp = stk.up(sp); }
                }
            }
#if PT_STEP_STATS
            { const bool x = (kind & 1u) != 0u; const uint64_t m = __ballot(x); st_lane_leaf += x ? 1u : 0u; if (m != 0ull && lane_id() == (uint32_t)__builtin_ctzll(m)) st_wave_leaf += 1u; }
#endif
            if (kind & 1u)
            {
                uint32_t first, count;
                leaf_range(bl, kind, payload, first, count);
                for (uint32_t k = 0; k < count; ++k)
                {
                    const uint4* tp = bl.tris + 3u * (first + k);
                    float td, ud, vd, det;
                    if (tri_planes(tp[0], tp[1], tp[2], ob.o, ob.d, t_max, t_enter, td, ud, vd, det))
                    {
                        active = false;
                        put_result(1u);
                        break;
                    }
                }
            }
        }
    }
#if PT_STEP_STATS
    if (MODE == ANY_SHADOW)
    {
        const uint32_t wave = blockIdx.x * (blockDim.x >> 6) + (threadIdx.x >> 6);
        uint32_t* line = heads + ((wave * 7u) & (kQueueHeads - 1u)) * kHeadStrideWords;
        if (lane_id() == 0u) { atomicAdd(line + 8, st_iter); atomicAdd(line + 9, st_lane_active); }
        uint32_t x = st_lane_inst, y = st_lane_branch, z = st_lane_leaf;
        for (int off = 32; off > 0; off >>= 1) { x += __shfl_xor(x, off); y += __shfl_xor(y, off); z += __shfl_xor(z, off); }
        if (lane_id() == 0u) { atomicAdd(line + 10, x); atomicAdd(line + 11, y); atomicAdd(line + 12, z); }
        x = st_wave_inst; y = st_wave_branch; z = st_wave_leaf;
        for (int off = 32; off > 0; off >>= 1) { x += __shfl_xor(x, off); y += __shfl_xor(y, off); z += __shfl_xor(z, off); }
        if (lane_id() == 0u) { atomicAdd(line + 13, x); atomicAdd(line + 14, y); atomicAdd(line + 15, z); }
    }
#endif
    if (MODE == ANY_SHADOW) add_tally(heads, valid_rays, HEAD_TALLY0);
#if PT_WAVE_TIMES
    if (MODE == ANY_SHADOW && lane_id() == 0u && g_any_times)
    {
        const uint32_t tw_end = (uint32_t)wall_clock64();
        if (tw_drained == 0u) tw_drained = tw_end;
        const uint32_t wave = blockIdx.x * (blockDim.x >> 6) + (threadIdx.x >> 6);
        if (wave < kWaveTimeSlots) g_any_times[wave] = make_uint4(tw_start, tw_start, tw_drained, tw_end | 1u);
    }
#endif
}
template <int BVH, int MODE, bool SPILL>
__global__ void __launch_bounds__(256, BVH != 0 ? PT_WAVES_LDS_BVH_ANY : PT_WAVES_GLOBAL_BVH_ANY) k_any(const SceneView sv, const uint4* __restrict__ gblob, const uint32_t root, const f4* __restrict__ ra,
                                              const f4* __restrict__ rb, const uint32_t* __restrict__ n_ptr, const uint32_t cap_in,
                                              uint32_t* __restrict__ heads, uint32_t* __restrict__ occluded,
                                              f4* __restrict__ radiance)
{
    constexpr bool LDS_SCENE = BVH != 0;
    extern __shared__ uint4 smem[];
    if (blockIdx.x >= fetch_plan(min(*n_ptr, cap_in), LDS_SCENE ? (uint32_t)PT_CHUNK_DIV : (uint32_t)PT_CHUNK_DIV_GLOBAL_BVH, (uint32_t)PT_TAPER_ANY).blocks) return;
    uint32_t blob_words;
    const Blob bl = stage_scene<LDS_SCENE>(sv, gblob, smem, blob_words);
    any_body<BVH, MODE, SPILL>(sv, bl, blob_words, smem, root, ra, rb, n_ptr, cap_in, heads, occluded, radiance);
}

struct FusedArgs
{
    const f4 *wa, *wb;
    const uint32_t* wn;
    uint32_t* wheads;
    const f4 *la, *lb;
    const uint32_t* ln;
    uint32_t* lheads;
    uint32_t world_root, lights_root, cap_in;
};
struct FusedKArgs
{
    SceneView sv;
    const uint4* gblob;
    FusedArgs fa;
    ClosestOut wout, lout;
};
template <int BVH, bool SPILL>
__global__ void __launch_bounds__(256, BVH != 0 ? PT_WAVES_LDS_BVH : PT_WAVES_GLOBAL_BVH) k_trace_fused(const FusedKArgs a)
{
    constexpr bool LDS_SCENE = BVH != 0;
    extern __shared__ uint4 smem[];
    const uint32_t cdiv = LDS_SCENE ? (uint32_t)PT_CHUNK_DIV : (uint32_t)PT_CHUNK_DIV_GLOBAL_BVH;
    const uint32_t need = max(fetch_plan(min(*a.fa.wn, a.fa.cap_in), cdiv, (uint32_t)PT_TAPER).blocks, fetch_plan(min(*a.fa.ln, a.fa.cap_in), cdiv, (uint32_t)PT_TAPER).blocks);
    if (blockIdx.x >= need) return;
    uint32_t blob_words;
    const Blob bl = stage_scene<LDS_SCENE>(a.sv, a.gblob, smem, blob_words);
    typedef const __attribute__((address_space(4))) FusedKArgs* FusedKArgsPtr;
    const FusedKArgsPtr k = (FusedKArgsPtr)__builtin_amdgcn_kernarg_segment_ptr();
    closest_body<BVH, CLOSEST_WORLD, SPILL>(a.sv, bl, blob_words, smem, a.fa.world_root, a.fa.wa, a.fa.wb, a.fa.wn, a.fa.cap_in, a.fa.wheads, &k->wout);
    closest_body<BVH, CLOSEST_LIGHTS, SPILL>(a.sv, bl, blob_words, smem, a.fa.lights_root, a.fa.la, a.fa.lb, a.fa.ln, a.fa.cap_in, a.fa.lheads, &k->lout);
}

struct PixelId { uint32_t gpixel, sample, lpixel, gx, gy; };

__device__ __forceinline__ uint32_t global_row(const RenderParams& rp, uint32_t ly)
{
    const uint32_t strip = fastdiv(ly, rp.div_strip_rows);
    return (strip * rp.world_size + rp.rank) * rp.strip_rows + (ly - strip * rp.strip_rows);
}
struct PidParts { uint32_t s, k; };
__device__ __forceinline__ PidParts pid_split(const RenderParams& rp, uint32_t pid)
{
    const uint32_t b = fastdiv(pid, rp.div_blk_paths), rem = pid - b * (rp.act_pixels << rp.blk_log);
    const bool short_blk = b + 1u == rp.n_blk;
    const uint32_t k = short_blk ? fastdiv(rem, rp.div_blk_last) : (rem >> rp.blk_log);
    return PidParts{(b << rp.blk_log) + (rem - k * (short_blk ? rp.blk_last : (1u << rp.blk_log))), k};
}
__device__ __forceinline__ uint32_t pid_join(const RenderParams& rp, uint32_t s, uint32_t k)
{
    const uint32_t b = s >> rp.blk_log;
    return b * (rp.act_pixels << rp.blk_log) + k * (b + 1u == rp.n_blk ? rp.blk_last : (1u << rp.blk_log)) + (s - (b << rp.blk_log));
}
__device__ __forceinline__ PixelId path_pixel(const RenderParams& rp, uint32_t pid, uint32_t* s_local = nullptr, uint32_t* k_out = nullptr)
{
    const PidParts pp = pid_split(rp, pid);
    if (s_local) *s_local = pp.s;
    if (k_out) *k_out = pp.k;
    const uint32_t r = fastdiv(pp.k, rp.div_act_w), x = rp.act_x0 + (pp.k - r * rp.act_w);
    const uint32_t ly = rp.act_ly0 + r;
    const uint32_t gy = global_row(rp, ly);
    return PixelId{gy * rp.width + x, rp.first_sample + pp.s, ly * rp.width + x, x, gy};
}

__device__ __forceinline__ f3 camera_ray_dir(const RenderParams& rp, const CameraView& cam, uint32_t gx, uint32_t gy, uint32_t sample)
{
    Stream rng{stream_key(rp.seed, gy * rp.width + gx, sample), 0u};
    const uint32_t seed = rng.u32();
    float jx, jy;
    ss_sobol(rp.n_sobol, sample, seed, &jx, &jy);
    const float ox = jx - 0.5f, oy = jy - 0.5f;
    const float u = ((float)gx + ox) / (float)rp.width;
    const float v = ((float)gy + oy) / (float)rp.height;
    const float nx = u * 2.0f - 1.0f, ny = v * 2.0f - 1.0f, nz = 0.0f;
    const float* M = cam.ray_matrix;
    float r[4];
#pragma unroll
    for (int i = 0; i < 4; ++i)
    {
        float t = M[i] * nx;
        t = M[4 + i] * ny + t;
        t = M[8 + i] * nz + t;
        t = M[12 + i] + t;
        r[i] = t;
    }
    const float rw = 1.0f / r[3];
    const f3 eye{cam.eye[0], cam.eye[1], cam.eye[2]};
    return unit3(f3{r[0] * rw, r[1] * rw, r[2] * rw} - eye);
}

__global__ void __launch_bounds__(256) k_generate(const RenderParams rp, const CameraView cam, const RayQueue rq, Counters* ctr)
{
    const uint32_t pid = blockIdx.x * blockDim.x + threadIdx.x;
    if (pid == 0u) ctr[0].n_closest = rp.n_paths;
    if (pid >= rp.n_paths) return;
    const PixelId px = path_pixel(rp, pid);
    const f3 dir = camera_ray_dir(rp, cam, px.gx, px.gy, px.sample);
    rq.b[pid] = f4{dir.x, dir.y, dir.z, asf(pid)};
}

struct ShadeIO
{
    PathState st;
    RayQueue rq_in, rq_out, rq_shadow, rq_lchain_prev, rq_lchain;
    f4* lchain_nb;
    const f4* lchain_nb_prev;
    const f4* lchain_hit;
    const f4* hits;
    const uint2* entries;
    ShadeQueue q_in;
    const uint32_t* tails_in;
    uint2* q_term_next;
    uint32_t cap_slots, cap_slots_term, cap_slots_shade;
    Counters* ctr;
// ... 39 lines not shown
            const f4 b4 = io.lchain_nb_prev[slot];
            const uint32_t inst = lid >> sv.prim_bits, tri = lid & ((1u << sv.prim_bits) - 1u);
            const DInstance& in = sv.instances[inst];
            const DMaterial& lm = sv.materials[in.material];
            const f3 emitted{lm.colour[0], lm.colour[1], lm.colour[2]};
            const DTriIsect ti = sv.tri_isect[tri];
            const float area = 0.5f * len3(xyz(ti.n0));
            const float sample_pdf = (area * len3(emitted) / sv.light_weight_sum) / area;
            const f3 dir = xyz(io.rq_lchain_prev.b[slot]);
            bool ff;
            const f3 ln = hit_normal(sv, inst, tri, lh.y, lh.z, dir, ff);
            const float cosine = fabsf(dot3(dir, ln));
            const float light_pdf = sample_pdf * (lh.x * lh.x / cosine);
            const float weight = mis2(pw4.w, light_pdf);
            s = emitted * weight * b4.w * xyz(b4) / pw4.w;
        }
    }
    acc = acc + xyz(pw4) * (e + s);
    flags &= ~(FLAG_NEE_PENDING | FLAG_BSDF_CAST);
}

__global__ void __launch_bounds__(256) k_shade_terminal(const SceneView sv, const RenderParams rp, const ShadeIO io, const uint32_t bounce)
{
    const uint32_t n = min(io.ctr->n_shade[Q_TERMINAL], io.cap_slots_term);
    for (uint32_t idx = blockIdx.x * blockDim.x + threadIdx.x; idx < n; idx += gridDim.x * blockDim.x)
    {
        const uint2 e2 = io.entries[idx];
        const uint32_t entry = e2.x, pid = e2.y;
        if (entry == HOLE) continue;
        const bool dead = (entry & ENTRY_DEAD) != 0u;
        f4 ra{}, rb{}, hit{};
        if (!dead)
        {
            hit = io.hits[entry];
            if (asu(hit.w) != MISS_ID)
            {
                ra = bounce == 0u ? io.primary_a : io.rq_in.a[entry];
                rb = io.rq_in.b[entry];
            }
            else if (io.env.w != 0u) rb = io.rq_in.b[entry];
        }
        f3 acc{0.0f, 0.0f, 0.0f};
        uint32_t flags = 0u;
        if (bounce != 0u)
        {
            const DPathRec& rec = io.st.rec[pid];
            const f4 acc4 = rec.acc;
            acc = xyz(acc4);
            flags = asu(acc4.w);
            resolve_nee(sv, io, pid, rec, acc, flags);
        }
        if (!dead)
        {
            const f3 pw = bounce == 0u ? f3{1.0f, 1.0f, 1.0f} : xyz(io.st.rec[pid].pw);
            const uint32_t hid = asu(hit.w);
            if (hid == MISS_ID)
            {
                if (io.env.w != 0u) acc = acc + env_lookup(io.env, xyz(rb)) * pw;
                else acc = acc + f3{0.006f, 0.006f, 0.006f} * pw;
            }
            else
            {
                const uint32_t inst = hid >> sv.prim_bits;
                const DInstance& in = sv.instances[inst];
                if (bounce == 0u)
                {
                    const PidParts pp = pid_split(rp, pid);
                    if (pp.s == rp.keep_s_pos)
                    {
                        const f3 p = fma3(xyz(rb), bc3(hit.x), xyz(ra));
                        io.st.first_pos[pp.k] = f4{p.x, p.y, p.z, hit.x};
                    }
                    if (pp.s >= rp.keep_s_id) io.st.first_id[(pp.s - rp.keep_s_id) * rp.act_pixels + pp.k] = in.blas & 0xffu;
                }
                const DMaterial& m = sv.materials[in.material];
                if (!rp.enable_nee || (flags & FLAG_LAST_DELTA) || bounce == 0u)
                    acc = fma3(f3{m.colour[0], m.colour[1], m.colour[2]}, pw, acc);
            }
        }
        io.st.radiance[pid] = f4{acc.x, acc.y, acc.z, 0.0f};
    }
}

__device__ __forceinline__ bool inline_any(const Blob& bl, const Stack8<false>& stk, const uint32_t root, const f4 ra, const f4 rb, const bool want)
{
    bool active = false, blocked = false, in_blas = false, ray_finite = false;
    LaneRay w{}, ob{};
    const float t_max = ra.w;
    uint32_t sp = stk.empty(), blas_base = 0u;
    if (want)
    {
        w.o = xyz(ra);
        w.d = xyz(rb);
        w.inv = rcp3(w.d);
        ray_finite = finite3(w.o) && finite3(w.d);
        float te;
        const uint4 root0 = bl.nodes[2u * root];
        if ((t_max == t_max) && slab(root0, bl.nodes[2u * root + 1u], w.o, w.inv, t_max, te))
        {
            stk.put(sp, make_uint2(root0.w, asu(te)));
            sp = stk.up(sp);
            active = true;
        }
    }
    while (__ballot(active) != 0ull)
    {
        if (!active) continue;
        if (in_blas && sp == blas_base) in_blas = false;
        if (sp == stk.empty()) { active = false; continue; }
        sp = stk.down(sp);
        const uint2 e = stk.get(sp);
        uint32_t link = e.x;
        float t_enter = asf(e.y);
        if ((link >> NODE_KIND_SHIFT) == NODE_INSTANCE)
        {
            uint4 r0, r1;
            ob = to_object<false, true>(bl, link & NODE_PAYLOAD_MASK, w, ray_finite, r0, r1);
            in_blas = true;
            blas_base = sp;
            if (!slab(r0, r1, ob.o, ob.inv, t_max, t_enter)) continue;
            link = r0.w;
        }
        uint32_t kind = link >> NODE_KIND_SHIFT, payload = link & NODE_PAYLOAD_MASK;
#pragma unroll 1
        for (int lvl = 0; lvl < PT_BRANCH_LEVELS_INLINE && kind == NODE_BRANCH; ++lvl)
        {
            const uint4* cp = bl.nodes + 2u * payload;
            const uint4 l0 = cp[0], l1 = cp[1], r0 = cp[2], r1 = cp[3];
            const f3 o = in_blas ? ob.o : w.o, inv = in_blas ? ob.inv : w.inv;
            float tl, tr;
            const bool hl = slab(l0, l1, o, inv, t_max, tl);
            const bool hr = slab(r0, r1, o, inv, t_max, tr);
            if (hl && hr) { stk.put(sp, make_uint2(l0.w, asu(tl))); sp = stk.up(sp); }
            kind = NODE_INSTANCE;
            if (hl || hr)
            {
                const uint2 next = hr ? make_uint2(r0.w, asu(tr)) : make_uint2(l0.w, asu(tl));
                const uint32_t nk = next.x >> NODE_KIND_SHIFT;
                if ((nk & 1u) != 0u || (nk == NODE_BRANCH && lvl + 1 < PT_BRANCH_LEVELS_INLINE))
                {
                    kind = nk;
                    payload = next.x & NODE_PAYLOAD_MASK;
                    t_enter = asf(next.y);
                }
                else { stk.put(sp, next); sp = stk.up(sp); }
            }
        }
        if (kind & 1u)
        {
            uint32_t first, count;
            leaf_range(bl, kind, payload, first, count);
            for (uint32_t k = 0; k < count; ++k)
            {
                const uint4* tp = bl.tris + 3u * (first + k);
                float td, ud, vd, det;
                if (tri_planes(tp[0], tp[1], tp[2], ob.o, ob.d, t_max, t_enter, td, ud, vd, det))
                {
                    active = false;
                    blocked = true;
                    break;
                }
            }
        }
    }
    return blocked;
}

struct ShadeKArgs { SceneView sv; RenderParams rp; ShadeIO io; uint32_t bounce; const uint4* gblob; uint32_t world_root; };
typedef const __attribute__((address_space(4))) ShadeKArgs* ShadeKArgsPtr;
__device__ __forceinline__ const ShadeKArgs& shade_args()
{
    ShadeKArgsPtr p = (ShadeKArgsPtr)__builtin_amdgcn_kernarg_segment_ptr();
    asm volatile("" : "+s"(p));
    return *(const ShadeKArgs*)p;
}
#define PT_SHADE_ARGS                                                                                                              \
    const ShadeKArgs& ka_ = shade_args();                                                                                          \
    [[maybe_unused]] const SceneView& sv = ka_.sv;                                                                                 \
    [[maybe_unused]] const RenderParams& rp = ka_.rp;                                                                              \
    [[maybe_unused]] const ShadeIO& io = ka_.io;
template <uint32_t QCLASS, bool VOLUMES, bool INLINE = false>
__global__ void __launch_bounds__(PT_SHADE_THREADS, INLINE ? PT_SHADE_WAVES_INLINE : shade_waves(QCLASS, VOLUMES)) k_shade_surface(const ShadeKArgs kargs)
{
    extern __shared__ uint4 smem_dyn[];
    const ShadeIO& io = kargs.io;
    const uint32_t bounce = kargs.bounce;
    __shared__ BlockAppend sh_append;
    __shared__ uint32_t sh_tail[kTailStripes];
    __shared__ uint32_t sh_extent;
    const Stripes stripes = stripes_for(min(io.ctr->n_closest, io.cap_slots));
    if (threadIdx.x < kTailStripes)
    {
        uint32_t mine;
        const uint32_t ext = stripe_load(io.tails_in, stripes, io.cap_slots_shade, mine);
        sh_tail[threadIdx.x] = mine;
        if (threadIdx.x == 0u)
        {
            sh_extent = ext;
            if (blockIdx.x == 0u) io.ctr->n_shade[QCLASS] = ext;
        }
    }
    if (INLINE) { uint32_t words; (void)stage_scene<true>(kargs.sv, kargs.gblob, smem_dyn, words); }
    else __syncthreads();
    uint32_t traced = 0u;
    const uint32_t n = sh_extent;
    const uint32_t total = ((n + blockDim.x - 1u) / blockDim.x) * blockDim.x;
    uint32_t culled = 0;
    const uint32_t stride = gridDim.x * blockDim.x;
    uint32_t idx = blockIdx.x * blockDim.x + threadIdx.x;
    const f4 hole_a{0.0f, 0.0f, 0.0f, asf(HOLE)};
    f4 a_next = idx < n ? nt_load(io.q_in.a + idx) : hole_a;
    for (; idx < total; idx += stride)
    {
        const f4 rb = a_next;
        if (!INLINE) a_next = (idx + stride) < n ? nt_load(io.q_in.a + idx + stride) : hole_a;
        bool valid = idx < n && stripe_valid(sh_tail, stripes, idx) && asu(rb.w) != HOLE;
        bool want_shadow = false, want_lchain = false, want_next = false, want_dead = false, ends_with_shadow = false, cull_now = false;
        f4 sh_a{}, sh_b{}, lc_a{}, lc_b{}, nx_a{}, nx_b{};
        uint32_t pid = 0, flags = 0;
        f3 acc{}, pw{};
        f4 nee_e{}, nee_pw{}, nee_b{};
        uint32_t draws = 0;
        if (valid)
        {
            PT_SHADE_ARGS
            pid = asu(rb.w);
            const f4 hit = nt_load(io.q_in.b + idx);
            const f4 ra = bounce == 0u ? io.primary_a : nt_load(io.q_in.c + idx);
            f4 pw4{1.0f, 1.0f, 1.0f, asf(1u)};
            acc = f3{0.0f, 0.0f, 0.0f};
            flags = 0u;
            if (bounce != 0u)
            {
                const DPathRec& rec = io.st.rec[pid];
                const f4 acc4 = rec.acc;
                pw4 = rec.pw;
                acc = xyz(acc4);
                flags = asu(acc4.w);
                resolve_nee(sv, io, pid, rec, acc, flags);
            }
            pw = xyz(pw4);

            const f3 ro = xyz(ra), rd = xyz(rb);
            const uint32_t hid = asu(hit.w);
            const uint32_t inst = hid >> sv.prim_bits, tri = hid & ((1u << sv.prim_bits) - 1u);
            const DInstance& in = sv.instances[inst];
            MatView mat = load_material(sv.materials, in.material);
            if (QCLASS == Q_LAMBERT) mat.kind = (VOLUMES && mat.kind == MAT_EMISSIVE) ? (uint32_t)MAT_EMISSIVE : (uint32_t)MAT_LAMBERTIAN;
            else if (QCLASS == Q_SPECULAR) mat.kind = MAT_SPECULAR;
            else if (QCLASS == Q_DIELECTRIC) mat.kind = MAT_DIELECTRIC;
            else mat.kind = mat.kind == MAT_GGX_DIELECTRIC ? (uint32_t)MAT_GGX_DIELECTRIC : (uint32_t)MAT_GGX_METAL;
            bool front;
            const f3 normal = hit_normal(sv, inst, tri, hit.y, hit.z, rd, front);
            const f3 p = fma3(rd, bc3(hit.x), ro);
            uint32_t s_local, k_pix;
            const PixelId px = path_pixel(rp, pid, &s_local, &k_pix);
            if (bounce == 0u)
            {
                if (s_local == rp.keep_s_pos) io.st.first_pos[k_pix] = f4{p.x, p.y, p.z, hit.x};
                if (s_local >= rp.keep_s_id) io.st.first_id[(s_local - rp.keep_s_id) * rp.act_pixels + k_pix] = in.blas & 0xffu;
            }
            Stream rng{stream_key(rp.seed, px.gpixel, px.sample), asu(pw4.w)};
            const f3 wi = -rd;
            const bool is_delta = mat_is_delta(mat.kind);
// ... 151 lines not shown
            if (alive)
            {
                pw = pw * (mat_weakening(mat.kind, ndir, normal) * info.bsdf / info.pdf);
                flags = is_delta ? (flags | FLAG_LAST_DELTA) : (flags & ~FLAG_LAST_DELTA);
            }
            }
            if (alive)
            {
                {
                const uint32_t nb = bounce + 1u;
                if (nb > rp.max_bounces) alive = false;
                else if (nb > 3u)
                {
                    const float survive = min_num(hmax3(pw), 0.9999f);
                    if (rng.f32() > survive) alive = false;
                    else pw = pw / survive;
                }
                }
            }
            if (alive && VOLUMES && (vst != vst_in || bounce == 0u)) io.st.vstack[pid] = vst;
            draws = rng.k;
            if (alive)
            {
                want_next = true;
                nx_a = f4{next_o.x, next_o.y, next_o.z, asf(0x7f800000u)};
                nx_b = f4{ndir.x, ndir.y, ndir.z, asf(pid)};
            }
            else if (flags & FLAG_NEE_PENDING)
            {
                if (flags & FLAG_BSDF_CAST) want_dead = true;
                else if (want_shadow) { ends_with_shadow = true; sh_b.w = asf(pid | PATH_ENDS); }
                else acc = acc + xyz(nee_pw) * (xyz(nee_e) + f3{0.0f, 0.0f, 0.0f});
            }
        }
        PT_SHADE_ARGS
        uint32_t* const ctrs[4] = {&io.ctr->n_shadow, &io.ctr->n_lchain, &io.ctr_next->n_closest, &io.ctr_next->n_shade[Q_TERMINAL]};
        const bool preds[4] = {want_shadow && !INLINE, want_lchain, want_next, want_dead};
        const uint32_t caps[4] = {io.cap_slots, io.cap_slots, io.cap_slots, io.cap_slots_term};
        uint32_t pos[4];
        block_append4(sh_append, ctrs, preds, caps, &io.ctr->overflow, pos);
        if (want_shadow && !INLINE) { nt_store(io.rq_shadow.a + pos[0], sh_a); nt_store(io.rq_shadow.b + pos[0], sh_b); }
        if (want_lchain) { io.rq_lchain.a[pos[1]] = lc_a; io.rq_lchain.b[pos[1]] = lc_b; io.lchain_nb[pos[1]] = nee_b; nee_e.w = asf(pos[1]); }
        if (want_next) { nt_store(io.rq_out.a + pos[2], nx_a); nt_store(io.rq_out.b + pos[2], nx_b); }
        if (want_dead) io.q_term_next[pos[3]] = make_uint2(pid | ENTRY_DEAD, pid);
        const bool write_rec = valid && (want_next || want_dead || ends_with_shadow);
        if (valid && !write_rec) io.st.radiance[pid] = f4{acc.x, acc.y, acc.z, 0.0f};
        {
            float m[4][4] = {{pw.x, pw.y, pw.z, asf(draws)}, {acc.x, acc.y, acc.z, asf(flags)}, {nee_e.x, nee_e.y, nee_e.z, nee_e.w}, {nee_pw.x, nee_pw.y, nee_pw.z, nee_pw.w}};
            const uint32_t q = threadIdx.x & 3u;
#pragma unroll
            for (int c = 0; c < 4; ++c)
            {
                float a0 = m[0][c], a1 = m[1][c], a2 = m[2][c], a3 = m[3][c];
                { const float t = (q & 1u) ? a0 : a1; const float r = asf(__builtin_amdgcn_mov_dpp(asu(t), 0xB1, 0xF, 0xF, true)); if (q & 1u) a0 = r; else a1 = r; }
                { const float t = (q & 1u) ? a2 : a3; const float r = asf(__builtin_amdgcn_mov_dpp(asu(t), 0xB1, 0xF, 0xF, true)); if (q & 1u) a2 = r; else a3 = r; }
                { const float t = (q & 2u) ? a0 : a2; const float r = asf(__builtin_amdgcn_mov_dpp(asu(t), 0x4E, 0xF, 0xF, true)); if (q & 2u) a0 = r; else a2 = r; }
                { const float t = (q & 2u) ? a1 : a3; const float r = asf(__builtin_amdgcn_mov_dpp(asu(t), 0x4E, 0xF, 0xF, true)); if (q & 2u) a1 = r; else a3 = r; }
                m[0][c] = a0; m[1][c] = a1; m[2][c] = a2; m[3][c] = a3;
            }
            const uint32_t wr = write_rec ? 1u : 0u;
#define PT_QUAD_STORE(K, SEL)                                                                                                   \
            {                                                                                                                      \
                const uint32_t pid_k = __builtin_amdgcn_mov_dpp(pid, SEL, 0xF, 0xF, true);                \
                const uint32_t wr_k = __builtin_amdgcn_mov_dpp(wr, SEL, 0xF, 0xF, true);                                           \
                if (wr_k != 0u) reinterpret_cast<f4*>(io.st.rec + pid_k)[q] = f4{m[K][0], m[K][1], m[K][2], m[K][3]};             \
            }
            PT_QUAD_STORE(0, 0x00) PT_QUAD_STORE(1, 0x55) PT_QUAD_STORE(2, 0xAA) PT_QUAD_STORE(3, 0xFF)
#undef PT_QUAD_STORE
        }
        if (INLINE)
        {
            uint32_t tid = threadIdx.x;
            asm volatile("" : "+v"(tid));
            const ShadeKArgs& ka2 = shade_args();
            const uint32_t blob_words = ka2.sv.blob_bytes >> 4;
            Blob bl;
            bl.nodes = smem_dyn;
            bl.tris = smem_dyn + 2u * ka2.sv.n_nodes;
            bl.inst = smem_dyn + 2u * ka2.sv.n_nodes + 3u * ka2.sv.n_tris;
            bl.leaves = reinterpret_cast<const uint2*>(smem_dyn + 2u * ka2.sv.n_nodes + 3u * ka2.sv.n_tris + INST_WORDS * ka2.sv.n_instances);
            const Stack8<false> stk{reinterpret_cast<char*>(smem_dyn), blob_words * 16u + tid * 8u, blockDim.x * 8u};
            traced += (uint32_t)__popcll(__ballot(want_shadow));
            culled += (uint32_t)__popcll(__ballot(cull_now));
            const bool blocked = inline_any(bl, stk, ka2.world_root, sh_a, sh_b, want_shadow);
            if (want_shadow)
            {
                DPathRec* rec = shade_args().io.st.rec + pid;
                if (ends_with_shadow)
                {
                    const f3 e = blocked ? f3{0.0f, 0.0f, 0.0f} : xyz(rec->nee_e);
                    const f3 a2 = xyz(rec->acc) + xyz(rec->nee_pw) * (e + f3{0.0f, 0.0f, 0.0f});
                    shade_args().io.st.radiance[pid] = f4{a2.x, a2.y, a2.z, 0.0f};
                }
                else if (blocked)
                {
                    float* e = reinterpret_cast<float*>(&rec->nee_e);
                    e[0] = 0.0f; e[1] = 0.0f; e[2] = 0.0f;
                }
            }
            a_next = (idx + stride) < n ? nt_load(shade_args().io.q_in.a + idx + stride) : hole_a;
        }
    }
    if (!INLINE) add_tally(io.lchain_heads, culled, HEAD_TALLY2);
    else if (lane_id() == 0u)
    {
        const uint32_t wave = blockIdx.x * (blockDim.x >> 6) + (threadIdx.x >> 6);
        const uint32_t line = ((wave * 7u) & (kQueueHeads - 1u)) * kHeadStrideWords;
        if (culled != 0u) atomicAdd(io.lchain_heads + line + HEAD_TALLY2, culled);
        if (traced != 0u) atomicAdd(io.shadow_heads + line + HEAD_TALLY0, traced);
    }
}

#undef PT_SHADE_ARGS

__device__ __forceinline__ f3 finalise(f3 acc)
{
    if (!finite3(acc)) return f3{0.0f, 0.0f, 0.0f};
    return clamp_len_max(acc, 100.0f);
}

template <bool FEW_PIXELS>
__global__ void __launch_bounds__(256) k_accumulate(const RenderParams rp, const CameraView cam, const PathState st, f4* accum, f4* position, uint32_t* id,
                                                     const uint32_t write_position, const uint32_t add_to_accum)
{
    const uint32_t tid = blockIdx.x * blockDim.x + threadIdx.x;
    const uint32_t lp = FEW_PIXELS ? tid >> 2 : tid, q = FEW_PIXELS ? (tid & 3u) : 0u;
    if (lp >= rp.local_pixels) return;
    f4 a = accum[lp];
    uint32_t idv = id[lp];
    const uint32_t ly = fastdiv(lp, rp.div_width), x = lp - ly * rp.width;
    if (x - rp.act_x0 >= rp.act_w || ly - rp.act_ly0 >= rp.act_rows)
    {
        for (uint32_t s = 0; s < rp.batch_samples; ++s) a = f4{a.x + 0.006f, a.y + 0.006f, a.z + 0.006f, a.w + 1.0f};
        for (uint32_t s = rp.batch_samples >= 2u ? rp.batch_samples - 2u : 0u; s < rp.batch_samples; ++s) idv = (idv << 16) | 255u;
        if (q != 0u) return;
        if (add_to_accum) accum[lp] = a;
        id[lp] = idv;
        if (write_position)
        {
            const f3 d = camera_ray_dir(rp, cam, x, global_row(rp, ly), rp.first_sample + rp.batch_samples - 1u);
            const f3 far = fma3(d, bc3(1e5f), f3{cam.eye[0], cam.eye[1], cam.eye[2]});
            position[lp] = f4{far.x, far.y, far.z, 1e5f};
        }
        return;
    }
    const uint32_t k = (ly - rp.act_ly0) * rp.act_w + (x - rp.act_x0);
    if (FEW_PIXELS)
    {
        constexpr uint32_t G = 4;
        for (uint32_t s0 = 0; s0 < rp.batch_samples; s0 += 4u * G)
        {
            uint32_t oc[G];
            f4 rad[G];
#pragma unroll
            for (uint32_t j = 0; j < G; ++j)
            {
                const uint32_t s = s0 + 4u * j + q;
                const uint32_t pid = pid_join(rp, s, k);
                oc[j] = s < rp.batch_samples ? (uint32_t)st.occl[pid] : (uint32_t)PRIMARY_MISS;
                rad[j] = s < rp.batch_samples ? st.radiance[pid] : f4{};
            }
            f3 c[G];
#pragma unroll
            for (uint32_t j = 0; j < G; ++j) c[j] = finalise(oc[j] != PRIMARY_MISS ? xyz(rad[j]) : f3{0.006f, 0.006f, 0.006f});
#pragma unroll
            for (uint32_t j = 0; j < G; ++j)
            {
// ... 92 lines not shown
        Stream r{stream_key(seed, asu(a[i]), asu(b[i])), 0u};
        o0[i] = asf(r.u32());
        o1[i] = r.f32();
        break;
    }
    }
}
__global__ void k_material_probe(const SceneView sv, int material, uint32_t n, const float* incoming, const float* normal, const uint8_t* front,
                                 const uint32_t* pixel, const uint32_t* sample, uint32_t draws, uint64_t seed, float* out9)
{
    const uint32_t i = blockIdx.x * blockDim.x + threadIdx.x;
    if (i >= n) return;
    const MatView m = load_material(sv.materials, (uint32_t)material);
    Stream rng{stream_key(seed, pixel[i], sample[i]), draws};
    const f3 in{incoming[3 * i], incoming[3 * i + 1], incoming[3 * i + 2]}, nn{normal[3 * i], normal[3 * i + 1], normal[3 * i + 2]};
    const bool ff = front[i] != 0;
    const f3 wo = mat_scatter(m, rng, in, nn, ff);
    const BsdfSample bp = mat_bsdf_pdf(m, -in, wo, nn, ff);
    float* o = out9 + 9 * i;
    o[0] = wo.x; o[1] = wo.y; o[2] = wo.z;
    o[3] = bp.bsdf.x; o[4] = bp.bsdf.y; o[5] = bp.bsdf.z;
    o[6] = bp.pdf;
    o[7] = mat_weakening(m.kind, wo, nn);
    o[8] = (float)(rng.k - draws);
}

__global__ void k_volume_probe(const SceneView sv, int material, uint32_t n, const float* incoming, const float* t_max, const float* dist,
                               const uint32_t* pixel, const uint32_t* sample, uint32_t draws, uint64_t seed, float* out9)
{
    const uint32_t i = blockIdx.x * blockDim.x + threadIdx.x;
    if (i >= n) return;
    const DMaterial& dm = sv.materials[material];
    Stream rng{stream_key(seed, pixel[i], sample[i]), draws};
    const f3 rd{incoming[3 * i], incoming[3 * i + 1], incoming[3 * i + 2]};
    float* o = out9 + 9 * i;
    o[0] = 0.0f; o[1] = 0.0f; o[2] = 0.0f; o[3] = 0.0f; o[4] = 0.0f;
    if (dm.vol_flags & 2u)
    {
        const float t = -ln_det(rng.f32()) / dm.vol_c;
        if (!(t > t_max[i]))
        {
            const f3 d = hg_direction(dm.vol_g, rng, rd);
            o[0] = 1.0f; o[1] = t; o[2] = d.x; o[3] = d.y; o[4] = d.z;
        }
    }
    f3 w{1.0f, 1.0f, 1.0f};
    if (dm.vol_flags & 1u) w = beer_lambert(f3{dm.vol_abs[0], dm.vol_abs[1], dm.vol_abs[2]}, dist[i]);
    o[5] = w.x; o[6] = w.y; o[7] = w.z;
    o[8] = (float)(rng.k - draws);
}

}

void launch_generate(hipStream_t s, const RenderParams& rp, const CameraView& cam, const WavefrontBuffers& wb)
{
    const uint32_t blocks = (rp.n_paths + 255u) / 256u;
    hipLaunchKernelGGL(k_generate, dim3(blocks), dim3(256), 0, s, rp, cam, wb.rq[0], wb.counters);
}

#ifndef PT_RESIDENT_GRID
#define PT_RESIDENT_GRID 1
#endif
template <typename K>
static uint32_t resident_grid(K kernel, const TraceLaunch& tl, size_t lds)
{
#if PT_RESIDENT_GRID
    struct Key { const void* f; uint32_t threads; size_t lds; int dev; int per_cu; };
    static std::mutex mu;
    static std::vector<Key> cache;
    int dev = 0;
    (void)hipGetDevice(&dev);
    std::lock_guard<std::mutex> lk(mu);
    for (const Key& k : cache)
        if (k.f == (const void*)kernel && k.threads == tl.block_threads && k.lds == lds && k.dev == dev) return std::min<uint32_t>(tl.grid_blocks, tl.n_cus * (uint32_t)k.per_cu);
    int per_cu = 0;
    if (hipOccupancyMaxActiveBlocksPerMultiprocessor(&per_cu, kernel, (int)tl.block_threads, lds) != hipSuccess || per_cu < 1) per_cu = 1;
    cache.push_back(Key{(const void*)kernel, tl.block_threads, lds, dev, per_cu});
    return std::min<uint32_t>(tl.grid_blocks, tl.n_cus * (uint32_t)per_cu);
#else
    return tl.grid_blocks;
#endif
}

template <int MODE>
static void launch_closest_impl(hipStream_t s, const TraceLaunch& tl, uint32_t root, const RayQueue& rq, const uint32_t* n_ptr, uint32_t cap_in,
                                uint32_t* heads, const ClosestOut& out)
{
    const bool spill = tl.scene.stack_entries > tl.scene.stack_lds;
    const dim3 block(tl.block_threads);
    const uint4* blob = (const uint4*)tl.blob;
    const size_t lds = trace_lds_bytes(tl);
    const ClosestKArgs ka{tl.scene, blob, rq.a, rq.b, n_ptr, heads, root, cap_in, out};
#define PT_LAUNCH1(K) hipLaunchKernelGGL(K, dim3(resident_grid(K, tl, lds)), block, lds, s, ka)
    if (tl.lds_scene && !spill) PT_LAUNCH1((k_closest<1, MODE, false>));
    else if (tl.lds_scene) PT_LAUNCH1((k_closest<1, MODE, true>));
    else if (!spill) PT_LAUNCH1((k_closest<0, MODE, false>));
    else PT_LAUNCH1((k_closest<0, MODE, true>));
#undef PT_LAUNCH1
}
template <int MODE>
static void launch_any_impl(hipStream_t s, const TraceLaunch& tl, uint32_t root, const RayQueue& rq, const uint32_t* n_ptr, uint32_t cap_in,
                            uint32_t* heads, uint32_t* occluded, f4* radiance = nullptr)
{
    const size_t lds = trace_lds_bytes(tl);
    const bool spill = tl.scene.stack_entries > tl.scene.stack_lds;
    const dim3 block(tl.block_threads);
    const uint4* blob = (const uint4*)tl.blob;
#define PT_LAUNCH(K) hipLaunchKernelGGL(K, dim3(resident_grid(K, tl, lds)), block, lds, s, tl.scene, blob, root, rq.a, rq.b, n_ptr, cap_in, heads, occluded, radiance)
    if (tl.lds_scene && !spill) PT_LAUNCH((k_any<1, MODE, false>));
    else if (tl.lds_scene) PT_LAUNCH((k_any<1, MODE, true>));
    else if (!spill) PT_LAUNCH((k_any<0, MODE, false>));
    else PT_LAUNCH((k_any<0, MODE, true>));
#undef PT_LAUNCH
}

static uint32_t* row_heads(const WavefrontBuffers& wb, uint32_t row, uint32_t which)
{
    return wb.heads + ((size_t)row * HEADS_PER_ROW + which) * kHeadWordsPerQueue;
}

void launch_trace_world(hipStream_t s, const TraceLaunch& tl, const WavefrontBuffers& wb, uint32_t b, const RenderParams& rp, const CameraView& cam,
                        const EnvView& env)
{
    Counters* row = wb.counters + b;
    ClosestOut out{};
    out.hits = wb.hits;
    out.q_base = wb.q_shade_base;
    out.q_stride = wb.q_stride;
    out.q_class_slot = wb.q_class_slot;
    out.q_term = wb.q_term[b & 1u];
    out.n_shade = row->n_shade;
    out.tails = wb.tails + (size_t)b * Q_COUNT * kTailWordsPerQueue;
    out.wave_times = wb.wave_times ? wb.wave_times + (size_t)b * kWaveTimeSlots : nullptr;
    out.cap_shade = wb.cap_slots_shade;
    out.cap_term = wb.cap_slots_term;
    out.class_mask = wb.class_mask | (1u << Q_TERMINAL);
    out.overflow = &row->overflow;
    if (b == 0u)
    {
        out.eye = f3{cam.eye[0], cam.eye[1], cam.eye[2]};
        out.radiance = wb.st.radiance;
        out.occl = wb.st.occl;
        out.first_pos = wb.st.first_pos;
        out.first_id = wb.st.first_id;
        out.keep_s_id = rp.keep_s_id; out.keep_s_pos = rp.keep_s_pos;
        out.blk_log = rp.blk_log; out.n_blk = rp.n_blk; out.blk_last = rp.blk_last; out.act_pixels = rp.act_pixels;
        out.div_blk_paths = rp.div_blk_paths; out.div_blk_last = rp.div_blk_last;
        out.finalize_miss = env.w == 0u ? 1u : 0u;
        launch_closest_impl<CLOSEST_PRIMARY>(s, tl, tl.scene.world_root, wb.rq[0], &row->n_closest, wb.cap_slots, row_heads(wb, b, HEADS_CLOSEST), out);
    }
    else
    {
        out.rec = wb.st.rec;
        out.radiance = wb.st.radiance;
        out.enable_nee = rp.enable_nee;
        out.finalize_miss = env.w == 0u ? 1u : 0u;
        launch_closest_impl<CLOSEST_WORLD>(s, tl, tl.scene.world_root, wb.rq[b & 1u], &row->n_closest, wb.cap_slots, row_heads(wb, b, HEADS_CLOSEST), out);
    }
}
void launch_trace_fused(hipStream_t s, const TraceLaunch& tl, const WavefrontBuffers& wb, uint32_t b, const RenderParams& rp, const EnvView& env)
{
    Counters* row = wb.counters + b;
    Counters* prev = wb.counters + (b - 1u);
    ClosestOut wout{};
    wout.hits = wb.hits;
    wout.q_base = wb.q_shade_base;
    wout.q_stride = wb.q_stride;
    wout.q_class_slot = wb.q_class_slot;
    wout.q_term = wb.q_term[b & 1u];
    wout.n_shade = row->n_shade;
    wout.tails = wb.tails + (size_t)b * Q_COUNT * kTailWordsPerQueue;
    wout.wave_times = nullptr;
    wout.cap_shade = wb.cap_slots_shade;
    wout.cap_term = wb.cap_slots_term;
    wout.class_mask = wb.class_mask | (1u << Q_TERMINAL);
    wout.overflow = &row->overflow;
    wout.rec = wb.st.rec;
    wout.radiance = wb.st.radiance;
    wout.enable_nee = rp.enable_nee;
    wout.finalize_miss = env.w == 0u ? 1u : 0u;
    ClosestOut lout{};
    lout.hits = wb.lchain_hit;
    lout.world_root = tl.scene.world_root;
    lout.occl = wb.st.occl;
    FusedArgs fa{};
    fa.wa = wb.rq[b & 1u].a; fa.wb = wb.rq[b & 1u].b; fa.wn = &row->n_closest; fa.wheads = row_heads(wb, b, HEADS_CLOSEST);
    fa.la = wb.rq_lchain[(b - 1u) & 1u].a; fa.lb = wb.rq_lchain[(b - 1u) & 1u].b; fa.ln = &prev->n_lchain; fa.lheads = row_heads(wb, b - 1u, HEADS_LCHAIN);
    fa.world_root = tl.scene.world_root; fa.lights_root = tl.scene.lights_root; fa.cap_in = wb.cap_slots;
    const size_t lds = trace_lds_bytes(tl);
    const bool spill = tl.scene.stack_entries > tl.scene.stack_lds;
    const dim3 block(tl.block_threads);
    const uint4* blob = (const uint4*)tl.blob;
    const FusedKArgs ka{tl.scene, blob, fa, wout, lout};
#define PT_LAUNCH(K) hipLaunchKernelGGL(K, dim3(resident_grid(K, tl, lds)), block, lds, s, ka)
    if (tl.lds_scene && !spill) PT_LAUNCH((k_trace_fused<1, false>));
    else if (tl.lds_scene) PT_LAUNCH((k_trace_fused<1, true>));
    else if (!spill) PT_LAUNCH((k_trace_fused<0, false>));
    else PT_LAUNCH((k_trace_fused<0, true>));
#undef PT_LAUNCH
}
void launch_trace_shadow(hipStream_t s, const TraceLaunch& tl, const WavefrontBuffers& wb, uint32_t b)
{
    Counters* row = wb.counters + b;
#if PT_WAVE_TIMES
    {
        uint4* where = wb.wave_times_any ? wb.wave_times_any + (size_t)b * kWaveTimeSlots : nullptr;
        (void)hipMemcpyToSymbolAsync(HIP_SYMBOL(g_any_times), &where, sizeof(where), 0, hipMemcpyHostToDevice, s);
    }
#endif
    launch_any_impl<ANY_SHADOW>(s, tl, tl.scene.world_root, wb.rq_shadow, &row->n_shadow, wb.cap_slots, row_heads(wb, b, HEADS_SHADOW),
                                reinterpret_cast<uint32_t*>(wb.st.rec), wb.st.radiance);
}
void launch_trace_lchain(hipStream_t s, const TraceLaunch& tl, const WavefrontBuffers& wb, uint32_t b)
{
    Counters* row = wb.counters + b;
    ClosestOut out{};
    out.hits = wb.lchain_hit;
    out.n_shade = nullptr;
    out.world_root = tl.scene.world_root;
    out.occl = wb.st.occl;
    launch_closest_impl<CLOSEST_LIGHTS>(s, tl, tl.scene.lights_root, wb.rq_lchain[b & 1u], &row->n_lchain, wb.cap_slots, row_heads(wb, b, HEADS_LCHAIN), out);
}
bool shade_traces_shadow(const TraceLaunch& tl)
{
    return PT_INLINE_SHADOW != 0 && tl.lds_scene && tl.scene.stack_entries <= tl.scene.stack_lds && !tl.scene.has_volumes && tl.block_threads == PT_SHADE_THREADS &&
           trace_lds_bytes(tl) + 1024 <= 32 * 1024;
}
void launch_shade(hipStream_t s, uint32_t qclass, const SceneView& sv, const RenderParams& rp, const WavefrontBuffers& wb, uint32_t b,
                  uint32_t grid_blocks, const CameraView& cam, const EnvView& env, const TraceLaunch* tl)
{
    ShadeIO io{};
    io.env = env;
    io.primary_a = f4{cam.eye[0], cam.eye[1], cam.eye[2], __builtin_inff()};
    io.st = wb.st;
    io.rq_in = wb.rq[b & 1u];
    io.rq_out = wb.rq[(b + 1u) & 1u];
    io.rq_shadow = wb.rq_shadow;
    io.rq_lchain = wb.rq_lchain[b & 1u];
    io.rq_lchain_prev = wb.rq_lchain[(b + 1u) & 1u];
    io.lchain_nb = wb.lchain_nb[b & 1u];
    io.lchain_nb_prev = wb.lchain_nb[(b + 1u) & 1u];
    io.lchain_hit = wb.lchain_hit;
    io.hits = wb.hits;
    io.entries = wb.q_term[b & 1u];
    if (qclass != Q_TERMINAL)
    {
        io.q_in = shade_queue(wb, qclass);
        io.tails_in = wb.tails + ((size_t)b * Q_COUNT + qclass) * kTailWordsPerQueue;
    }
    io.q_term_next = wb.q_term[(b + 1u) & 1u];
    io.cap_slots = wb.cap_slots;
    io.cap_slots_term = wb.cap_slots_term;
    io.cap_slots_shade = wb.cap_slots_shade;
    io.ctr = wb.counters + b;
    io.lchain_heads = row_heads(wb, b, HEADS_LCHAIN);
    io.shadow_heads = row_heads(wb, b, HEADS_SHADOW);
    io.ctr_next = wb.counters + b + 1u;
    const uint32_t surface_blocks = (grid_blocks * 256u + PT_SHADE_THREADS - 1u) / PT_SHADE_THREADS;
    const bool inl = tl && shade_traces_shadow(*tl);
    const ShadeKArgs ka{sv, rp, io, b, inl ? (const uint4*)tl->blob : nullptr, inl ? tl->scene.world_root : 0u};
    const size_t lds = inl ? trace_lds_bytes(*tl) : 0;
    switch (qclass)
    {
    case Q_TERMINAL: hipLaunchKernelGGL(k_shade_terminal, dim3(grid_blocks), dim3(256), 0, s, sv, rp, io, b); break;
    case Q_LAMBERT:
        if (inl) hipLaunchKernelGGL((k_shade_surface<Q_LAMBERT, false, true>), dim3(surface_blocks), dim3(PT_SHADE_THREADS), lds, s, ka);
        else if (sv.has_volumes) hipLaunchKernelGGL((k_shade_surface<Q_LAMBERT, true>), dim3(surface_blocks), dim3(PT_SHADE_THREADS), 0, s, ka);
        else hipLaunchKernelGGL((k_shade_surface<Q_LAMBERT, false>), dim3(surface_blocks), dim3(PT_SHADE_THREADS), 0, s, ka);
        break;
    case Q_SPECULAR:
        if (sv.has_volumes) hipLaunchKernelGGL((k_shade_surface<Q_SPECULAR, true>), dim3(surface_blocks), dim3(PT_SHADE_THREADS), 0, s, ka);
        else hipLaunchKernelGGL((k_shade_surface<Q_SPECULAR, false>), dim3(surface_blocks), dim3(PT_SHADE_THREADS), 0, s, ka);
        break;
    case Q_DIELECTRIC:
        if (sv.has_volumes) hipLaunchKernelGGL((k_shade_surface<Q_DIELECTRIC, true>), dim3(surface_blocks), dim3(PT_SHADE_THREADS), 0, s, ka);
        else hipLaunchKernelGGL((k_shade_surface<Q_DIELECTRIC, false>), dim3(surface_blocks), dim3(PT_SHADE_THREADS), 0, s, ka);
        break;
    case Q_GGX:
        if (sv.has_volumes) hipLaunchKernelGGL((k_shade_surface<Q_GGX, true>), dim3(surface_blocks), dim3(PT_SHADE_THREADS), 0, s, ka);
        else hipLaunchKernelGGL((k_shade_surface<Q_GGX, false>), dim3(surface_blocks), dim3(PT_SHADE_THREADS), 0, s, ka);
        break;
    default: break;
    }
}

void launch_accumulate(hipStream_t s, const RenderParams& rp, const CameraView& cam, const WavefrontBuffers& wb, f4* accum, f4* position, uint32_t* id,
                       uint32_t write_position, uint32_t add_to_accum)
{
    const uint32_t blocks = (rp.local_pixels + 255u) / 256u;
    if (rp.local_pixels < (uint32_t)PT_ACC_QUAD_BELOW) hipLaunchKernelGGL(k_accumulate<true>, dim3((rp.local_pixels * 4u + 255u) / 256u), dim3(256), 0, s, rp, cam, wb.st, accum, position, id, write_position, add_to_accum);
    else hipLaunchKernelGGL(k_accumulate<false>, dim3(blocks), dim3(256), 0, s, rp, cam, wb.st, accum, position, id, write_position, add_to_accum);
}
void launch_store_samples(hipStream_t s, const RenderParams& rp, const WavefrontBuffers& wb, f4* out)
{
    const uint32_t blocks = (uint32_t)(((uint64_t)rp.local_pixels * rp.batch_samples + 255u) / 256u);
    hipLaunchKernelGGL(k_store_samples, dim3(blocks), dim3(256), 0, s, rp, wb.st, out);
}

void launch_trace_rays_closest(hipStream_t s, const TraceLaunch& tl, uint32_t root, RayQueue rq, uint32_t n, uint32_t* n_and_heads, f4* hits)
{
    ClosestOut out{};
    out.hits = hits;
    launch_closest_impl<CLOSEST_HOOK>(s, tl, root, rq, n_and_heads, n, n_and_heads + 32, out);
}
void launch_trace_rays_any(hipStream_t s, const TraceLaunch& tl, uint32_t root, RayQueue rq, uint32_t n, uint32_t* n_and_heads, uint32_t* occluded)
{
    launch_any_impl<ANY_HOOK>(s, tl, root, rq, n_and_heads, n, n_and_heads + 32, occluded);
}
void launch_sobol_probe(hipStream_t s, uint32_t n_points, uint32_t n, const uint32_t* index, const uint32_t* seed, float* out_xy)
{
    hipLaunchKernelGGL(k_sobol_probe, dim3((n + 255u) / 256u), dim3(256), 0, s, n_points, n, index, seed, out_xy);
}
void launch_math_probe(hipStream_t s, int fn, uint32_t n, const float* a, const float* b, float* o0, float* o1, uint64_t seed)
{
    hipLaunchKernelGGL(k_math_probe, dim3((n + 255u) / 256u), dim3(256), 0, s, fn, n, a, b, o0, o1, seed);
}
void launch_material_probe(hipStream_t s, const SceneView& sv, int material, uint32_t n, const float* incoming, const float* normal,
                           const uint8_t* front, const uint32_t* pixel, const uint32_t* sample, uint32_t draws, uint64_t seed, float* out9)
{
    hipLaunchKernelGGL(k_material_probe, dim3((n + 255u) / 256u), dim3(256), 0, s, sv, material, n, incoming, normal, front, pixel, sample, draws, seed,
                       out9);
}

void launch_volume_probe(hipStream_t s, const SceneView& sv, int material, uint32_t n, const float* incoming, const float* t_max, const float* dist,
                         const uint32_t* pixel, const uint32_t* sample, uint32_t draws, uint64_t seed, float* out9)
{
    hipLaunchKernelGGL(k_volume_probe, dim3((n + 255u) / 256u), dim3(256), 0, s, sv, material, n, incoming, t_max, dist, pixel, sample, draws, seed, out9);
}

}
```

path_tracer_amd/csrc/pt_scene.cpp:

```cpp
#include "pt_scene.h"

#include <algorithm>
#include <chrono>
#include <cctype>
#include <cstdio>
#include <cstdlib>
#include <cstring>
#include <exception>
#include <numeric>
#include <system_error>
#include <thread>
#include <utility>

namespace pt {

namespace {

const float kInf = __builtin_inff();

HostBox box_empty() { return HostBox{bc3(kInf), bc3(-kInf)}; }
HostBox box_join(const HostBox& a, const HostBox& b) { return HostBox{min3(a.mn, b.mn), max3(a.mx, b.mx)}; }
float box_area(const HostBox& b)
{
    f3 v = b.mx - b.mn;
// ... 624 lines not shown
            frontier.push_back({n.b, frontier[k].second + 1});
        }
        for (const auto& d : deep)
        {
            std::vector<uint32_t> stack{d.first};
            while (!stack.empty())
            {
                const uint32_t i = stack.back();
                stack.pop_back();
                const HostNode& n = nodes[i];
                if (n.kind != NODE_BRANCH) continue;
                where[n.a] = next;
                where[n.b] = next + 1u;
                next += 2u;
                stack.push_back(n.b);
                stack.push_back(n.a);
            }
        }
        return next == base + nodes.size();
    };
    auto leaf_link = [&](uint32_t first, uint32_t count) -> uint32_t {
        if (count >= 1u && count <= LEAF_MAX_COUNT && first <= LEAF_FIRST_MASK)
            return (NODE_TRIS << NODE_KIND_SHIFT) | ((count - 1u) << LEAF_FIRST_BITS) | first;
        f.big_leaves.push_back(first);
        f.big_leaves.push_back(count);
        return (NODE_TRIS_BIG << NODE_KIND_SHIFT) | (uint32_t)(f.big_leaves.size() / 2u - 1u);
    };
    std::vector<uint32_t> slot_of;
    auto put_tlas = [&](const HostTlas& t, uint32_t base, uint32_t inst_base) -> bool {
        if (!layout(t.nodes, t.root, base, slot_of)) return false;
        for (size_t i = 0; i < t.nodes.size(); ++i)
        {
            DNode& d = f.nodes[slot_of[i]];
            put_box(d, t.nodes[i].box);
            if (t.nodes[i].kind == NODE_BRANCH) { d.link = (NODE_BRANCH << NODE_KIND_SHIFT) | slot_of[t.nodes[i].a]; d.aux = slot_of[t.nodes[i].b]; }
            else { d.link = (NODE_INSTANCE << NODE_KIND_SHIFT) | (inst_base + t.nodes[i].a); d.aux = 0u; }
        }
        return true;
    };
    if (!put_tlas(world, world_base, f.inst_base[0]) || !put_tlas(lights, lights_base, f.inst_base[1]))
    {
        if (err) *err = "internal: TLAS arena holds nodes outside the tree";
        return -5;
    }
    f.world_root = world.root == MISS_ID ? MISS_ID : world_base;
    f.lights_root = lights.root == MISS_ID ? MISS_ID : lights_base;

    uint32_t max_blas_depth = 0;
    std::vector<uint32_t> blas_root_at(blas.size(), MISS_ID);
    f.tri_isect.reserve(tri_cursor);
    f.tri_shade.reserve(tri_cursor);
    f.tri_pos.reserve(tri_cursor);
    f.tri_orig.reserve(tri_cursor);
    for (size_t i = 0; i < blas.size(); ++i)
    {
        const HostBlas& bl = blas[i];
        max_blas_depth = std::max(max_blas_depth, bl.depth);
        if (!layout(bl.nodes, bl.root, blas_base[i], slot_of)) { if (err) *err = "internal: BLAS arena holds nodes outside the tree"; return -5; }
        blas_root_at[i] = blas_base[i];
        for (size_t n = 0; n < bl.nodes.size(); ++n)
        {
            DNode& d = f.nodes[slot_of[n]];
            put_box(d, bl.nodes[n].box);
            if (bl.nodes[n].kind == NODE_BRANCH) { d.link = (NODE_BRANCH << NODE_KIND_SHIFT) | slot_of[bl.nodes[n].a]; d.aux = slot_of[bl.nodes[n].b]; }
            else { d.link = leaf_link(f.tri_base[i] + bl.nodes[n].a, bl.nodes[n].b); d.aux = bl.nodes[n].b; }
        }
        const size_t at = f.tri_orig.size();
        f.tri_isect.resize(at + bl.prim_ids.size());
        f.tri_shade.resize(at + bl.prim_ids.size());
        f.tri_pos.resize(at + bl.prim_ids.size());
        f.tri_orig.resize(at + bl.prim_ids.size());
        parallel_slices(bl.prim_ids.size(), [&](size_t lo, size_t hi) {
            for (size_t k = lo; k < hi; ++k)
            {
                const uint32_t id = bl.prim_ids[k];
                const HostTriangle& t = bl.tris[id];
                f.tri_isect[at + k] = DTriIsect{t.n0, t.n1, t.n2};
                f.tri_shade[at + k] = DTriVerts{f4{t.n[0].x, t.n[0].y, t.n[0].z, 0}, f4{t.n[1].x, t.n[1].y, t.n[1].z, 0}, f4{t.n[2].x, t.n[2].y, t.n[2].z, 0}};
                f.tri_pos[at + k] = DTriVerts{f4{t.p[0].x, t.p[0].y, t.p[0].z, 0}, f4{t.p[1].x, t.p[1].y, t.p[1].z, 0}, f4{t.p[2].x, t.p[2].y, t.p[2].z, 0}};
                f.tri_orig[at + k] = id;
            }
        });
    }
    auto put_instances = [&](const HostTlas& t) {
        for (const HostInstance& hi : t.instances)
        {
            DInstance d;
            std::memset(&d, 0, sizeof(d));
            const xf34* src[2] = {&hi.inv, &hi.fwd};
            float* dst[2] = {d.inv, d.fwd};
            for (int k = 0; k < 2; ++k)
            {
                const xf34& x = *src[k];
                const float rows[12] = {x.m.c0.x, x.m.c1.x, x.m.c2.x, x.t.x, x.m.c0.y, x.m.c1.y, x.m.c2.y, x.t.y, x.m.c0.z, x.m.c1.z, x.m.c2.z, x.t.z};
                std::memcpy(dst[k], rows, sizeof(rows));
            }
            d.root = blas_root_at[hi.model];
            d.root_node = f.nodes[d.root];
            d.blas = hi.blas;
            d.material = blas_material[hi.model];
            switch (f.materials[d.material].kind)
            {
            case MAT_LAMBERTIAN: d.qclass = Q_LAMBERT; break;
            case MAT_SPECULAR: d.qclass = Q_SPECULAR; break;
            case MAT_DIELECTRIC: d.qclass = Q_DIELECTRIC; break;
            case MAT_GGX_METAL:
            case MAT_GGX_DIELECTRIC: d.qclass = Q_GGX; break;
            default: d.qclass = Q_TERMINAL; break;
            }
            if (f.has_volumes && f.materials[d.material].kind == MAT_EMISSIVE) d.qclass = Q_LAMBERT;
            {
                static const uint32_t ident[12] = {0x3f800000u, 0, 0, 0x80000000u, 0, 0x3f800000u, 0, 0x80000000u, 0, 0, 0x3f800000u, 0x80000000u};
                if (std::memcmp(d.inv, ident, sizeof(ident)) == 0) d.qclass |= INSTANCE_IDENTITY;
            }
            f.instances.push_back(d);
        }
    };
    put_instances(world);
    put_instances(lights);

    std::vector<std::vector<uint32_t>> where(blas.size());
    for (size_t i = 0; i < blas.size(); ++i)
    {
        where[i].assign(blas[i].tris.size(), 0);
        for (size_t k = 0; k < blas[i].prim_ids.size(); ++k) where[i][blas[i].prim_ids[k]] = f.tri_base[i] + (uint32_t)k;
    }
    for (const HostLight& l : light_items)
    {
        const uint32_t mi = lights.models[l.blas];
        f.lights.push_back(DLight{where[mi][l.prim], (uint32_t)blas[mi].material, l.pdf, l.cdf});
    }
    f.light_weight_sum = light_weight_sum;

    uint32_t pb = 1;
    while ((1ull << pb) < (uint64_t)std::max<uint32_t>(tri_cursor, 2)) ++pb;
    f.prim_bits = pb;
    if ((uint64_t)f.instances.size() >= (1ull << (32 - pb)) - 1) { if (err) *err = "instance x triangle id does not fit 32 bits"; return -5; }
    const uint32_t tlas_depth = std::max(world.depth, lights.depth);
    f.stack_entries = std::max(tlas_depth, (tlas_depth > 0 ? tlas_depth - 1 : 0) + max_blas_depth);
    flat = std::move(f);
    return 0;
}

namespace {
struct quat { float x, y, z, w; };

quat quat_mul(quat l, quat r)
{
    return quat{(l.w * r.x + l.x * r.w) + (l.y * r.z + -(l.z * r.y)),
                (l.w * r.y + -(l.x * r.z)) + (l.y * r.w + l.z * r.x),
                (l.w * r.z + l.x * r.y) + (-(l.y * r.x) + l.z * r.w),
                (l.w * r.w + -(l.x * r.x)) + (-(l.y * r.y) + -(l.z * r.z))};
}

quat quat_from_axes(f3 ax, f3 ay, f3 az)
{
    const float m00 = ax.x, m01 = ax.y, m02 = ax.z, m10 = ay.x, m11 = ay.y, m12 = ay.z, m20 = az.x, m21 = az.y, m22 = az.z;
    if (m22 <= 0.0f)
    {
        const float dif10 = m11 - m00, omm22 = 1.0f - m22;
        if (dif10 <= 0.0f)
        {
            const float four_xsq = omm22 - dif10, inv4x = 0.5f / std::sqrt(four_xsq);
            return quat{four_xsq * inv4x, (m01 + m10) * inv4x, (m02 + m20) * inv4x, (m12 - m21) * inv4x};
        }
        const float four_ysq = omm22 + dif10, inv4y = 0.5f / std::sqrt(four_ysq);
        return quat{(m01 + m10) * inv4y, four_ysq * inv4y, (m12 + m21) * inv4y, (m20 - m02) * inv4y};
    }
    const float sum10 = m11 + m00, opm22 = 1.0f + m22;
    if (sum10 <= 0.0f)
    {
        const float four_zsq = opm22 - sum10, inv4z = 0.5f / std::sqrt(four_zsq);
        return quat{(m02 + m20) * inv4z, (m12 + m21) * inv4z, four_zsq * inv4z, (m01 - m10) * inv4z};
    }
    const float four_wsq = opm22 + sum10, inv4w = 0.5f / std::sqrt(four_wsq);
    return quat{(m12 - m21) * inv4w, (m20 - m02) * inv4w, (m01 - m10) * inv4w, four_wsq * inv4w};
}

void euler_yxz_of(quat q, float* first, float* second)
{
    *first = atan2_det(2.0f * (q.x * q.z + q.w * q.y), q.w * q.w - q.x * q.x - q.y * q.y + q.z * q.z);
    float v = -2.0f * (q.y * q.z - q.w * q.x);
    v = v < -1.0f ? -1.0f : v;
    v = v > 1.0f ? 1.0f : v;
    *second = asin_det(v);
}

m33 mat3_of_quat(quat q)
{
    const float x2 = q.x + q.x, y2 = q.y + q.y, z2 = q.z + q.z;
    const float xx = q.x * x2, xy = q.x * y2, xz = q.x * z2, yy = q.y * y2, yz = q.y * z2, zz = q.z * z2, wx = q.w * x2, wy = q.w * y2, wz = q.w * z2;
    return m33{f3{1.0f - (yy + zz), xy + wz, xz - wy}, f3{xy - wz, 1.0f - (xx + zz), yz + wx}, f3{xz + wy, yz - wx, 1.0f - (xx + yy)}};
}

}

void HostScene::set_camera(const float eye_[3], const float target_[3], float fov_deg, float aspect)
{
    const f3 eye{eye_[0], eye_[1], eye_[2]}, target{target_[0], target_[1], target_[2]};
    const f3 up{0.0f, 1.0f, 0.0f};
    const f3 fwd = unit3_recip(-(target - eye));
    const f3 side = unit3_recip(cross3(up, fwd));
// ... 73 lines not shown
```

path_tracer_amd/csrc/pt_scene.h:

```cpp
#pragma once
#include <string>
#include <vector>

#include "pt_types.h"

namespace pt {

struct HostBox { f3 mn, mx; };

struct HostNode
{
    HostBox box;
    uint32_t kind;
    uint32_t a, b;
};

struct HostTriangle
{
    f3 p[3], n[3];
    f4 n0, n1, n2;
};

struct HostBlas
{
    std::vector<HostTriangle> tris;
    std::vector<HostNode> nodes;
    std::vector<uint32_t> prim_ids;
    uint32_t root = 0;
    uint32_t depth = 0;
    int material = 0;
};

struct HostInstance
{
    uint32_t blas;
    uint32_t model;
    xf34 fwd, inv;
};

struct HostTlas
{
    std::vector<HostNode> nodes;
    std::vector<HostInstance> instances;
    uint32_t root = MISS_ID;
    uint32_t depth = 0;
    std::vector<uint32_t> models;
};

struct HostModel
{
    std::vector<float> positions, normals;
    uint32_t n_tris = 0;
    int material = 0;
    std::vector<xf34> matrices;
};

struct HostLight { uint32_t blas, prim; float pdf, cdf; };

struct HostCamera
{
    bool set = false;
    float yaw = 0, pitch = 0;
    xf34 matrix;
    float inv_proj[16];
    float ray_matrix[16];
};

struct FlatScene
{
    std::vector<DNode> nodes;
    std::vector<DTriIsect> tri_isect;
    std::vector<DTriVerts> tri_shade, tri_pos;
    std::vector<uint32_t> tri_orig;
    std::vector<DInstance> instances;
    std::vector<uint32_t> big_leaves;
    std::vector<DMaterial> materials;
    std::vector<DLight> lights;
    std::vector<uint32_t> tri_base;
    std::vector<uint32_t> inst_base;
    uint32_t world_root = MISS_ID, lights_root = MISS_ID;
    uint32_t prim_bits = 0;
    uint32_t stack_entries = 0;
    float light_weight_sum = 0;
    bool has_volumes = false;
};

class HostScene
{
public:
    std::vector<DMaterial> materials;
    std::vector<HostModel> models;
    std::vector<HostBlas> blas;
    HostTlas world, lights;
    std::vector<HostLight> light_items;
    float light_weight_sum = 0;
    HostCamera camera;
    FlatScene flat;
    bool built = false;

    int add_material(int kind, const float colour[3], float roughness, float ior, bool has_volume, const float vol_abs[3], float k, float c,
                     float g);
    int add_model(const float* positions, const float* normals, uint32_t n_tris, int material, const float* affines, uint32_t n_inst);
    int add_model_obj(const char* path, int material, const float* affines, uint32_t n_inst, std::string* err);
    int build(std::string* err);
    void set_camera(const float eye[3], const float target[3], float fov_deg, float aspect);
    void create_ray(float s, float t, float o[3], float d[3]) const;
    void inv_projection(float out16[16]) const;
    void camera_move(float dx, float dz, float dt);
    void camera_rotate(float dx, float dy, float dt);

private:
    void build_blas(HostBlas& out, const HostModel& m);
    void build_tlas(HostTlas& out, const std::vector<uint32_t>& model_ids);
    void build_lights();
    int flatten(std::string* err);
    void refresh_ray_matrix();
};

}
```

path_tracer_amd/csrc/pt_types.h:

```cpp
#pragma once
#include <stdint.h>
#include "pt_math.h"

namespace pt {

enum : uint32_t
{
    NODE_BRANCH = 0u,
    NODE_TRIS = 1u,
    NODE_INSTANCE = 2u,
    NODE_TRIS_BIG = 3u,
    NODE_KIND_SHIFT = 30u,
    NODE_PAYLOAD_MASK = 0x3fffffffu,
    LEAF_FIRST_BITS = 24u,
    LEAF_FIRST_MASK = 0x00ffffffu,
    LEAF_MAX_COUNT = 64u,
    MISS_ID = 0xffffffffu
};

struct alignas(16) DNode
{
    float mn[3];
    uint32_t link;
    float mx[3];
    uint32_t aux;
};
static_assert(sizeof(DNode) == 32, "node is two 16-byte words");

struct alignas(16) DTriIsect { f4 n0, n1, n2; };
static_assert(sizeof(DTriIsect) == 48, "");
struct alignas(16) DTriVerts { f4 a, b, c; };

struct alignas(16) DInstance
{
    float inv[12];
    uint32_t root;
    uint32_t blas;
    uint32_t material;
    uint32_t qclass;
    DNode root_node;
    float fwd[12];
};
static_assert(sizeof(DInstance) == 144, "");
enum : uint32_t { INST_WORDS = 9u, INST_META_WORD = 3u, INST_ROOT_WORD = 4u };

enum : uint32_t { MAT_LAMBERTIAN = 0, MAT_EMISSIVE = 1, MAT_SPECULAR = 2, MAT_GGX_METAL = 3, MAT_GGX_DIELECTRIC = 4, MAT_DIELECTRIC = 5 };

struct alignas(16) DMaterial
{
    float colour[3];
    uint32_t kind;
    float alpha;
    float ior;
    uint32_t has_volume;
    uint32_t vol_flags;
    float vol_abs[3];
    float vol_c;
    float vol_g;
    float pad[3];
};
static_assert(sizeof(DMaterial) == 64, "");

struct alignas(16) DLight
{
    uint32_t tri;
    uint32_t material;
    float pdf;
    float cdf;
};

enum : uint32_t { Q_TERMINAL = 0, Q_LAMBERT = 1, Q_SPECULAR = 2, Q_DIELECTRIC = 3, Q_GGX = 4, Q_COUNT = 5 };
enum : uint32_t { ENTRY_DEAD = 0x80000000u };
enum : uint32_t { INSTANCE_IDENTITY = 0x100u };

struct Counters
{
    uint32_t n_closest;
    uint32_t overflow;
    uint32_t n_shadow;
    uint32_t vstack_full;
    uint32_t n_lchain;
    uint32_t spare1;
    uint32_t spare2, spare3;
    uint32_t n_shade[Q_COUNT];
    uint32_t spare4, spare5, spare6;
};
static_assert(sizeof(Counters) == 64, "");

struct SceneView
{
    const DNode* nodes;
    const DTriIsect* tri_isect;
    const DTriVerts* tri_shade;
    const DTriVerts* tri_pos;
    const uint32_t* tri_orig;
    const DInstance* instances;
    const DMaterial* materials;
    const DLight* lights;
    uint32_t n_nodes, n_tris, n_instances, n_materials, n_lights;
    uint32_t world_root, lights_root;
    uint32_t prim_bits;
    float light_weight_sum;
    uint32_t has_volumes;
    uint32_t blob_bytes;
    uint32_t stack_entries;
    uint32_t stack_lds;
    uint64_t* stack_spill;
};
struct CameraView
{
    float ray_matrix[16];
    float eye[3];
    float pad;
};

struct FastDiv
{
    uint32_t magic, shift, one, d;
};
inline FastDiv fastdiv_make(uint32_t d)
{
    FastDiv f{0u, 0u, d <= 1u ? 1u : 0u, d};
    if (d <= 1u) return f;
    uint32_t l = 31u;
    while (!((d >> l) & 1u)) --l;
    if ((d & (d - 1u)) == 0u) { f.magic = 0u; f.shift = l - 1u; return f; }
    const uint64_t num = (uint64_t)1 << (32u + l);
    uint64_t m = num / d;
    const uint64_t rem = num - m * d;
    m += m;
    const uint64_t twice_rem = rem + rem;
    if (twice_rem >= d) m += 1u;
    f.magic = (uint32_t)(m + 1u);
    f.shift = l;
    return f;
}

struct RenderParams
{
    uint32_t width, height;
    uint32_t local_rows, local_pixels;
    uint32_t rank, world_size, strip_rows;
    uint32_t first_sample;
    uint32_t batch_samples;
    uint32_t n_paths;
    uint32_t max_bounces, n_sobol, enable_nee;
    uint32_t keep_s_id;
    uint32_t keep_s_pos;
    uint32_t blk_log, n_blk, blk_last;
    uint32_t act_x0, act_w, act_ly0, act_rows, act_pixels;
    uint32_t pad[1];
    uint64_t seed;
    FastDiv div_blk_paths, div_blk_last, div_act_w, div_width, div_strip_rows;
};

struct DPathRec
// ... 42 lines not shown
```

Before: 14200 Mray/s.

## Specialize traversal kernels for TLAS with all-identity instance transforms

At scene build, the code detects when every instance in the world or lights TLAS has an identity transform and records this as bits. It then launches IDENT-specialised closest, any, fused-trace and inline-shadow kernels that skip the per-instance ray-to-object transform and BLAS enter/exit bookkeeping, using a precomputed sign-normalised ray instead. This removes ALU work and register pressure during traversal in scenes like the Cornell box. The cost is more kernel template instantiations, and it must reproduce the signed-zero behaviour of the transformed ray exactly.

```diff
diff --git a/include/pt_api.h b/include/pt_api.h
--- a/include/pt_api.h
+++ b/include/pt_api.h
@@ -63,7 +63,8 @@
     PT_FLAG_TIMING = 1u,
     PT_FLAG_NO_LDS_SCENE = 2u,
     PT_FLAG_TIMING_ALL = 4u,
-    PT_FLAG_NO_PRIMARY_CULL = 8u
+    PT_FLAG_NO_PRIMARY_CULL = 8u,
+    PT_FLAG_GENERAL_WALK = 16u
 };
 
 pt_ctx* pt_create(const pt_config* cfg);
@@ -157,6 +158,8 @@
     uint64_t state_bytes;
     uint64_t rays_light_closest_traced;
     uint64_t rays_primary_culled;
+    uint32_t ident_tlas;
+    uint32_t reserved_stats;
 } pt_stats;
 int pt_get_stats(pt_ctx* ctx, pt_stats* out);
 int pt_multi_get_stats(pt_multi* m, pt_stats* sum);
diff --git a/path_tracer_amd/api.py b/path_tracer_amd/api.py
--- a/path_tracer_amd/api.py
+++ b/path_tracer_amd/api.py
@@ -14,6 +14,7 @@
 FLAG_NO_LDS_SCENE = 2
 FLAG_TIMING_ALL = 4
 FLAG_NO_PRIMARY_CULL = 8
+FLAG_GENERAL_WALK = 16
 DEFAULT_SEED = 0x5EED5EED
 
 EXPORTS = [
@@ -47,7 +48,8 @@
                 ("launches_trace_closest", C.c_uint64), ("ms_trace_closest", C.c_double), ("ms_trace_any", C.c_double),
                 ("ms_trace_light", C.c_double), ("ms_shade", C.c_double), ("ms_generate", C.c_double), ("ms_accumulate", C.c_double),
                 ("ms_total", C.c_double), ("scene_bytes", C.c_uint64), ("lds_scene", C.c_uint32), ("stack_entries", C.c_uint32),
-                ("state_bytes", C.c_uint64), ("rays_light_closest_traced", C.c_uint64), ("rays_primary_culled", C.c_uint64)]
+                ("state_bytes", C.c_uint64), ("rays_light_closest_traced", C.c_uint64), ("rays_primary_culled", C.c_uint64),
+                ("ident_tlas", C.c_uint32), ("reserved_stats", C.c_uint32)]
 
     def as_dict(self):
         return {n: getattr(self, n) for n, _ in self._fields_}
diff --git a/path_tracer_amd/csrc/pt_api.cpp b/path_tracer_amd/csrc/pt_api.cpp
--- a/path_tracer_amd/csrc/pt_api.cpp
+++ b/path_tracer_amd/csrc/pt_api.cpp
@@ -113,6 +113,7 @@
     bool env_uploaded = false;
     SceneView sv{};
     bool lds_scene = false;
+    uint32_t ident_tlas = 0;
     uint32_t block_threads = 256, trace_blocks = 1024;
     bool class_present[Q_COUNT] = {true, false, false, false, false};
 
@@ -264,6 +265,7 @@
     sv.blob_bytes = (uint32_t)blob.size();
     sv.stack_entries = f.stack_entries;
     sv.has_volumes = f.has_volumes ? 1u : 0u;
+    c->ident_tlas = f.ident_tlas;
 
     c->lds_scene = blob.size() <= 48 * 1024 && !(c->cfg.flags & PT_FLAG_NO_LDS_SCENE);
     uint32_t threads = 256;
@@ -304,6 +306,7 @@
     if (tl.scene.stack_spill) tl.scene.stack_spill += (size_t)(2 * pipe + (side_stream ? 1 : 0)) * c->spill_region_words;
     tl.blob = c->d_blob.p;
     tl.lds_scene = c->lds_scene;
+    tl.ident_tlas = (c->cfg.flags & PT_FLAG_GENERAL_WALK) ? 0u : c->ident_tlas;
     tl.grid_blocks = c->trace_blocks;
     tl.n_cus = (uint32_t)c->n_cus;
     tl.block_threads = c->block_threads;
@@ -2007,6 +2010,7 @@
         sum->ms_total = std::max(sum->ms_total, s.ms_total);
         sum->state_bytes += s.state_bytes;
         sum->scene_bytes = s.scene_bytes; sum->lds_scene = s.lds_scene; sum->stack_entries = s.stack_entries;
+        sum->ident_tlas = c->scene_uploaded && !(c->cfg.flags & PT_FLAG_GENERAL_WALK) ? c->ident_tlas : 0u;
     }
     return PT_OK;
 }
@@ -2015,6 +2019,7 @@
 {
     if (!c || !out) return PT_ERR_ARG;
     *out = c->stats;
+    out->ident_tlas = c->scene_uploaded && !(c->cfg.flags & PT_FLAG_GENERAL_WALK) ? c->ident_tlas : 0u;
     return PT_OK;
 }
 
diff --git a/path_tracer_amd/csrc/pt_kernels.h b/path_tracer_amd/csrc/pt_kernels.h
--- a/path_tracer_amd/csrc/pt_kernels.h
+++ b/path_tracer_amd/csrc/pt_kernels.h
@@ -11,6 +11,7 @@
     SceneView scene;
     const void* blob;
     bool lds_scene;
+    uint32_t ident_tlas;
     uint32_t grid_blocks;
     uint32_t n_cus;
     uint32_t block_threads;
diff --git a/path_tracer_amd/csrc/pt_kernels.hip b/path_tracer_amd/csrc/pt_kernels.hip
--- a/path_tracer_amd/csrc/pt_kernels.hip
+++ b/path_tracer_amd/csrc/pt_kernels.hip
@@ -98,6 +98,9 @@
 }
 #ifndef PT_INLINE_SHADOW
 #define PT_INLINE_SHADOW 1
+#endif
+#ifndef PT_IDENT_SHADE
+#define PT_IDENT_SHADE 1
 #endif
 #ifndef PT_SHADE_WAVES_INLINE
 #define PT_SHADE_WAVES_INLINE 5
@@ -514,6 +517,31 @@
     r.d.z = (asf(r2.x) * w.d.x + asf(r2.y) * w.d.y) + asf(r2.z) * w.d.z;
     r.inv = rcp3(r.d);
     return r;
+}
+
+__device__ __forceinline__ LaneRay ident_ray(const LaneRay& w)
+{
+    const uint32_t so = asu(w.o.x) & asu(w.o.y) & asu(w.o.z) & 0x80000000u;
+    const uint32_t sd = asu(w.d.x) & asu(w.d.y) & asu(w.d.z) & 0x80000000u;
+    LaneRay r;
+    r.o.x = w.o.x != 0.0f ? w.o.x : asf(so);
+    r.o.y = w.o.y != 0.0f ? w.o.y : asf(so);
+    r.o.z = w.o.z != 0.0f ? w.o.z : asf(so);
+    r.d.x = w.d.x != 0.0f ? w.d.x : asf(sd);
+    r.d.y = w.d.y != 0.0f ? w.d.y : asf(sd);
+    r.d.z = w.d.z != 0.0f ? w.d.z : asf(sd);
+    r.inv = w.inv;
+    return r;
+}
+__device__ __forceinline__ uint32_t ray_signs(const LaneRay& w)
+{
+    return (asu(w.o.x) >> 31) | ((asu(w.o.y) >> 31) << 1) | ((asu(w.o.z) >> 31) << 2) |
+           ((asu(w.d.x) >> 31) << 3) | ((asu(w.d.y) >> 31) << 4) | ((asu(w.d.z) >> 31) << 5);
+}
+__device__ __forceinline__ f3 with_signs(const f3 v, uint32_t bits)
+{
+    return f3{asf((asu(v.x) & 0x7fffffffu) | ((bits & 1u) << 31)), asf((asu(v.y) & 0x7fffffffu) | (((bits >> 1) & 1u) << 31)),
+              asf((asu(v.z) & 0x7fffffffu) | (((bits >> 2) & 1u) << 31))};
 }
 
 template <bool LDS_SCENE>
@@ -629,7 +657,7 @@
     asm volatile("" : "+s"(p));
     return p;
 }
-template <int BVH, int MODE, bool SPILL>
+template <int BVH, int MODE, bool SPILL, bool IDENT>
 __device__ __forceinline__ void closest_body(const SceneView& sv, const Blob& bl, const uint32_t blob_words, uint4* smem, const uint32_t root, const f4* __restrict__ ra,
                                              const f4* __restrict__ rb, const uint32_t* __restrict__ n_ptr, const uint32_t cap_in,
                                              uint32_t* __restrict__ heads, const ClosestOutPtr outp)
@@ -643,6 +671,7 @@
     bool active = false, pending = false, ray_finite = false;
     uint32_t ray_idx = 0, pid = 0;
     LaneRay w{}, ob{};
+    uint32_t w_signs = 0u;
     float t_max = 0.0f, bt = 0.0f;
     float hud = 0.0f, hvd = 0.0f, hdet = 1.0f;
     uint32_t bid = MISS_ID, sp = stk.empty(), blas_base = 0, inst = 0;
@@ -682,6 +711,7 @@
             {
                 if (MODE == CLOSEST_WORLD || MODE == CLOSEST_PRIMARY)
                 {
+                    if (IDENT && pending) { w.o = with_signs(ob.o, w_signs); w.d = with_signs(ob.d, w_signs >> 3); }
                     uint64_t qm = pm;
                     if (MODE == CLOSEST_PRIMARY)
                     {
@@ -815,6 +845,7 @@
                 w.d = xyz(b);
                 w.inv = rcp3(w.d);
                 ray_finite = finite3(w.o) && finite3(w.d);
+                if (IDENT) { ob = ident_ray(w); w_signs = ray_signs(w); }
                 bid = MISS_ID;
                 any_phase = false;
                 chain_code = 2u;
@@ -826,7 +857,7 @@
                 sp = stk.empty();
                 float te;
                 const uint4 root0 = bl.nodes[2u * root];
-                const bool ok = (t_max == t_max) && slab(root0, bl.nodes[2u * root + 1u], w.o, w.inv, t_max, te);
+                const bool ok = (t_max == t_max) && (!IDENT || ray_finite) && slab(root0, bl.nodes[2u * root + 1u], IDENT ? ob.o : w.o, w.inv, t_max, te);
                 if (ok)
                 {
                     stk.put(sp, make_uint2(root0.w, 0u));
@@ -854,7 +885,7 @@
             }
 #endif
             if (!active) continue;
-            if (in_blas && sp == blas_base) in_blas = false;
+            if (!IDENT && in_blas && sp == blas_base) in_blas = false;
             if (MODE == CLOSEST_LIGHTS && any_phase)
             {
                 if (sp == stk.empty()) { active = false; pending = true; chain_code = 0u; continue; }
@@ -865,9 +896,17 @@
                 if ((link >> NODE_KIND_SHIFT) == NODE_INSTANCE)
                 {
                     uint4 r0, r1;
-                    ob = to_object<!LDS_SCENE, true>(bl, link & NODE_PAYLOAD_MASK, w, ray_finite, r0, r1);
-                    in_blas = true;
-                    blas_base = sp;
+                    if (IDENT)
+                    {
+                        const uint4* ip = bl.inst + INST_WORDS * (link & NODE_PAYLOAD_MASK) + INST_ROOT_WORD;
+                        r0 = ip[0]; r1 = ip[1];
+                    }
+                    else
+                    {
+                        ob = to_object<!LDS_SCENE, true>(bl, link & NODE_PAYLOAD_MASK, w, ray_finite, r0, r1);
+                        in_blas = true;
+                        blas_base = sp;
+                    }
                     if (!slab(r0, r1, ob.o, ob.inv, t_max, t_enter)) continue;
                     link = r0.w;
                 }
@@ -876,7 +915,7 @@
                 {
                     const uint4* cp = bl.nodes + 2u * kpay;
                     const uint4 l0 = cp[0], l1 = cp[1], r0 = cp[2], r1 = cp[3];
-                    const f3 so = in_blas ? ob.o : w.o, sinv = in_blas ? ob.inv : w.inv;
+                    const f3 so = (IDENT || in_blas) ? ob.o : w.o, sinv = (IDENT || in_blas) ? ob.inv : w.inv;
                     float tl, tr;
                     const bool hl = slab(l0, l1, so, sinv, t_max, tl);
                     const bool hr = slab(r0, r1, so, sinv, t_max, tr);
@@ -912,7 +951,7 @@
                     t_max = bt * (1.0f - PT_EPSILON);
                     float te = 0.0f;
                     const uint4 wr0 = bl.nodes[2u * lights_world_root];
-                    if (t_max == t_max && slab(wr0, bl.nodes[2u * lights_world_root + 1u], w.o, w.inv, t_max, te)) { stk.put(sp, make_uint2(wr0.w, asu(te))); sp = stk.up(sp); }
+                    if (t_max == t_max && slab(wr0, bl.nodes[2u * lights_world_root + 1u], IDENT ? ob.o : w.o, IDENT ? ob.inv : w.inv, t_max, te)) { stk.put(sp, make_uint2(wr0.w, asu(te))); sp = stk.up(sp); }
                     else { active = false; pending = true; chain_code = 0u; }
                     continue;
                 }
@@ -932,9 +971,13 @@
             {
                 uint4 root0, root1;
                 inst = link & NODE_PAYLOAD_MASK;
-                ob = to_object<!LDS_SCENE, false>(bl, inst, w, ray_finite, root0, root1);
-                in_blas = true;
-                blas_base = sp;
+                if (IDENT) root0.w = reinterpret_cast<const uint32_t*>(bl.inst + INST_WORDS * inst + INST_ROOT_WORD)[3];
+                else
+                {
+                    ob = to_object<!LDS_SCENE, false>(bl, inst, w, ray_finite, root0, root1);
+                    in_blas = true;
+                    blas_base = sp;
+                }
                 if (0.0f > t_max) continue;
                 link = root0.w;
                 t_est = 0.0f;
@@ -948,7 +991,7 @@
             {
                 const uint4* cp = bl.nodes + 2u * payload;
                 const uint4 l0 = cp[0], l1 = cp[1], r0 = cp[2], r1 = cp[3];
-                const f3 o = in_blas ? ob.o : w.o, inv = in_blas ? ob.inv : w.inv;
+                const f3 o = (IDENT || in_blas) ? ob.o : w.o, inv = (IDENT || in_blas) ? ob.inv : w.inv;
                 float tl, tr;
                 const bool hl = slab(l0, l1, o, inv, t_max, tl);
                 const bool hr = slab(r0, r1, o, inv, t_max, tr);
@@ -1032,7 +1075,7 @@
     if (MODE != CLOSEST_HOOK) add_tally(heads, valid_rays, HEAD_TALLY0);
     if (MODE == CLOSEST_LIGHTS) add_tally(heads, light_hits, HEAD_TALLY1);
 }
-template <int BVH, int MODE, bool SPILL>
+template <int BVH, int MODE, bool SPILL, bool IDENT = false>
 __global__ void __launch_bounds__(256, BVH != 0 ? PT_WAVES_LDS_BVH : PT_WAVES_GLOBAL_BVH) k_closest(const ClosestKArgs a)
 {
     constexpr bool LDS_SCENE = BVH != 0;
@@ -1041,12 +1084,12 @@
     uint32_t blob_words;
     const Blob bl = stage_scene<LDS_SCENE>(a.sv, a.gblob, smem, blob_words);
     const ClosestOutPtr outp = &((ClosestKArgsPtr)__builtin_amdgcn_kernarg_segment_ptr())->out;
-    closest_body<BVH, MODE, SPILL>(a.sv, bl, blob_words, smem, a.root, a.ra, a.rb, a.n_ptr, a.cap_in, a.heads, outp);
+    closest_body<BVH, MODE, SPILL, IDENT>(a.sv, bl, blob_words, smem, a.root, a.ra, a.rb, a.n_ptr, a.cap_in, a.heads, outp);
 }
 
 enum { ANY_SHADOW = 0, ANY_HOOK = 2 };
 
-template <int BVH, int MODE, bool SPILL>
+template <int BVH, int MODE, bool SPILL, bool IDENT>
 __device__ __forceinline__ void any_body(const SceneView& sv, const Blob& bl, const uint32_t blob_words, uint4* smem, const uint32_t root, const f4* __restrict__ ra,
                                          const f4* __restrict__ rb, const uint32_t* __restrict__ n_ptr, const uint32_t cap_in,
                                          uint32_t* __restrict__ heads, uint32_t* __restrict__ occluded,
@@ -1120,12 +1163,13 @@
                 w.d = xyz(b);
                 w.inv = rcp3(w.d);
                 ray_finite = finite3(w.o) && finite3(w.d);
+                if (IDENT) ob = ident_ray(w);
                 t_max = a.w;
                 in_blas = false;
                 sp = stk.empty();
                 float te;
                 const uint4 root0 = bl.nodes[2u * root];
-                const bool ok = (t_max == t_max) && slab(root0, bl.nodes[2u * root + 1u], w.o, w.inv, t_max, te);
+                const bool ok = (t_max == t_max) && (!IDENT || ray_finite) && slab(root0, bl.nodes[2u * root + 1u], IDENT ? ob.o : w.o, w.inv, t_max, te);
                 if (ok)
                 {
                     stk.put(sp, make_uint2(root0.w, asu(te)));
@@ -1150,7 +1194,7 @@
             }
 #endif
             if (!active) continue;
-            if (in_blas && sp == blas_base) in_blas = false;
+            if (!IDENT && in_blas && sp == blas_base) in_blas = false;
             if (sp == stk.empty())
             {
                 active = false;
@@ -1167,9 +1211,17 @@
             if ((link >> NODE_KIND_SHIFT) == NODE_INSTANCE)
             {
                 uint4 r0, r1;
-                ob = to_object<!LDS_SCENE, true>(bl, link & NODE_PAYLOAD_MASK, w, ray_finite, r0, r1);
-                in_blas = true;
-                blas_base = sp;
+                if (IDENT)
+                {
+                    const uint4* ip = bl.inst + INST_WORDS * (link & NODE_PAYLOAD_MASK) + INST_ROOT_WORD;
+                    r0 = ip[0]; r1 = ip[1];
+                }
+                else
+                {
+                    ob = to_object<!LDS_SCENE, true>(bl, link & NODE_PAYLOAD_MASK, w, ray_finite, r0, r1);
+                    in_blas = true;
+                    blas_base = sp;
+                }
                 if (!slab(r0, r1, ob.o, ob.inv, t_max, t_enter)) continue;
                 link = r0.w;
             }
@@ -1182,7 +1234,7 @@
             {
                 const uint4* cp = bl.nodes + 2u * payload;
                 const uint4 l0 = cp[0], l1 = cp[1], r0 = cp[2], r1 = cp[3];
-                const f3 o = in_blas ? ob.o : w.o, inv = in_blas ? ob.inv : w.inv;
+                const f3 o = (IDENT || in_blas) ? ob.o : w.o, inv = (IDENT || in_blas) ? ob.inv : w.inv;
                 float tl, tr;
                 const bool hl = slab(l0, l1, o, inv, t_max, tl);
                 const bool hr = slab(r0, r1, o, inv, t_max, tr);
@@ -1247,7 +1299,7 @@
     }
 #endif
 }
-template <int BVH, int MODE, bool SPILL>
+template <int BVH, int MODE, bool SPILL, bool IDENT = false>
 __global__ void __launch_bounds__(256, BVH != 0 ? PT_WAVES_LDS_BVH_ANY : PT_WAVES_GLOBAL_BVH_ANY) k_any(const SceneView sv, const uint4* __restrict__ gblob, const uint32_t root, const f4* __restrict__ ra,
                                               const f4* __restrict__ rb, const uint32_t* __restrict__ n_ptr, const uint32_t cap_in,
                                               uint32_t* __restrict__ heads, uint32_t* __restrict__ occluded,
@@ -1258,7 +1310,7 @@
     if (blockIdx.x >= fetch_plan(min(*n_ptr, cap_in), LDS_SCENE ? (uint32_t)PT_CHUNK_DIV : (uint32_t)PT_CHUNK_DIV_GLOBAL_BVH, (uint32_t)PT_TAPER_ANY).blocks) return;
     uint32_t blob_words;
     const Blob bl = stage_scene<LDS_SCENE>(sv, gblob, smem, blob_words);
-    any_body<BVH, MODE, SPILL>(sv, bl, blob_words, smem, root, ra, rb, n_ptr, cap_in, heads, occluded, radiance);
+    any_body<BVH, MODE, SPILL, IDENT>(sv, bl, blob_words, smem, root, ra, rb, n_ptr, cap_in, heads, occluded, radiance);
 }
 
 struct FusedArgs
@@ -1278,7 +1330,7 @@
     FusedArgs fa;
     ClosestOut wout, lout;
 };
-template <int BVH, bool SPILL>
+template <int BVH, bool SPILL, bool IDENT = false>
 __global__ void __launch_bounds__(256, BVH != 0 ? PT_WAVES_LDS_BVH : PT_WAVES_GLOBAL_BVH) k_trace_fused(const FusedKArgs a)
 {
     constexpr bool LDS_SCENE = BVH != 0;
@@ -1290,8 +1342,8 @@
     const Blob bl = stage_scene<LDS_SCENE>(a.sv, a.gblob, smem, blob_words);
     typedef const __attribute__((address_space(4))) FusedKArgs* FusedKArgsPtr;
     const FusedKArgsPtr k = (FusedKArgsPtr)__builtin_amdgcn_kernarg_segment_ptr();
-    closest_body<BVH, CLOSEST_WORLD, SPILL>(a.sv, bl, blob_words, smem, a.fa.world_root, a.fa.wa, a.fa.wb, a.fa.wn, a.fa.cap_in, a.fa.wheads, &k->wout);
-    closest_body<BVH, CLOSEST_LIGHTS, SPILL>(a.sv, bl, blob_words, smem, a.fa.lights_root, a.fa.la, a.fa.lb, a.fa.ln, a.fa.cap_in, a.fa.lheads, &k->lout);
+    closest_body<BVH, CLOSEST_WORLD, SPILL, IDENT>(a.sv, bl, blob_words, smem, a.fa.world_root, a.fa.wa, a.fa.wb, a.fa.wn, a.fa.cap_in, a.fa.wheads, &k->wout);
+    closest_body<BVH, CLOSEST_LIGHTS, SPILL, IDENT>(a.sv, bl, blob_words, smem, a.fa.lights_root, a.fa.la, a.fa.lb, a.fa.ln, a.fa.cap_in, a.fa.lheads, &k->lout);
 }
 
 struct PixelId { uint32_t gpixel, sample, lpixel, gx, gy; };
@@ -1497,6 +1549,7 @@
     }
 }
 
+template <bool IDENT>
 __device__ __forceinline__ bool inline_any(const Blob& bl, const Stack8<false>& stk, const uint32_t root, const f4 ra, const f4 rb, const bool want)
 {
     bool active = false, blocked = false, in_blas = false, ray_finite = false;
@@ -1509,9 +1562,10 @@
         w.d = xyz(rb);
         w.inv = rcp3(w.d);
         ray_finite = finite3(w.o) && finite3(w.d);
+        if (IDENT) ob = ident_ray(w);
         float te;
         const uint4 root0 = bl.nodes[2u * root];
-        if ((t_max == t_max) && slab(root0, bl.nodes[2u * root + 1u], w.o, w.inv, t_max, te))
+        if ((t_max == t_max) && (!IDENT || ray_finite) && slab(root0, bl.nodes[2u * root + 1u], IDENT ? ob.o : w.o, w.inv, t_max, te))
         {
             stk.put(sp, make_uint2(root0.w, asu(te)));
             sp = stk.up(sp);
@@ -1521,7 +1575,7 @@
     while (__ballot(active) != 0ull)
     {
         if (!active) continue;
-        if (in_blas && sp == blas_base) in_blas = false;
+        if (!IDENT && in_blas && sp == blas_base) in_blas = false;
         if (sp == stk.empty()) { active = false; continue; }
         sp = stk.down(sp);
         const uint2 e = stk.get(sp);
@@ -1530,9 +1584,17 @@
         if ((link >> NODE_KIND_SHIFT) == NODE_INSTANCE)
         {
             uint4 r0, r1;
-            ob = to_object<false, true>(bl, link & NODE_PAYLOAD_MASK, w, ray_finite, r0, r1);
-            in_blas = true;
-            blas_base = sp;
+            if (IDENT)
+            {
+                const uint4* ip = bl.inst + INST_WORDS * (link & NODE_PAYLOAD_MASK) + INST_ROOT_WORD;
+                r0 = ip[0]; r1 = ip[1];
+            }
+            else
+            {
+                ob = to_object<false, true>(bl, link & NODE_PAYLOAD_MASK, w, ray_finite, r0, r1);
+                in_blas = true;
+                blas_base = sp;
+            }
             if (!slab(r0, r1, ob.o, ob.inv, t_max, t_enter)) continue;
             link = r0.w;
         }
@@ -1542,7 +1604,7 @@
         {
             const uint4* cp = bl.nodes + 2u * payload;
             const uint4 l0 = cp[0], l1 = cp[1], r0 = cp[2], r1 = cp[3];
-            const f3 o = in_blas ? ob.o : w.o, inv = in_blas ? ob.inv : w.inv;
+            const f3 o = (IDENT || in_blas) ? ob.o : w.o, inv = (IDENT || in_blas) ? ob.inv : w.inv;
             float tl, tr;
             const bool hl = slab(l0, l1, o, inv, t_max, tl);
             const bool hr = slab(r0, r1, o, inv, t_max, tr);
@@ -1594,7 +1656,7 @@
     [[maybe_unused]] const SceneView& sv = ka_.sv;                                                                                 \
     [[maybe_unused]] const RenderParams& rp = ka_.rp;                                                                              \
     [[maybe_unused]] const ShadeIO& io = ka_.io;
-template <uint32_t QCLASS, bool VOLUMES, bool INLINE = false>
+template <uint32_t QCLASS, bool VOLUMES, bool INLINE = false, bool IDENT = false>
 __global__ void __launch_bounds__(PT_SHADE_THREADS, INLINE ? PT_SHADE_WAVES_INLINE : shade_waves(QCLASS, VOLUMES)) k_shade_surface(const ShadeKArgs kargs)
 {
     extern __shared__ uint4 smem_dyn[];
@@ -1912,7 +1974,7 @@
             const Stack8<false> stk{reinterpret_cast<char*>(smem_dyn), blob_words * 16u + tid * 8u, blockDim.x * 8u};
             traced += (uint32_t)__popcll(__ballot(want_shadow));
             culled += (uint32_t)__popcll(__ballot(cull_now));
-            const bool blocked = inline_any(bl, stk, ka2.world_root, sh_a, sh_b, want_shadow);
+            const bool blocked = inline_any<IDENT>(bl, stk, ka2.world_root, sh_a, sh_b, want_shadow);
             if (want_shadow)
             {
                 DPathRec* rec = shade_args().io.st.rec + pid;
@@ -2171,17 +2233,32 @@
 #endif
 }
 
+static uint32_t tlas_bits(const TraceLaunch& tl, uint32_t root, bool with_world)
+{
+    const uint32_t own = root == tl.scene.world_root ? (uint32_t)IDENT_TLAS_WORLD : root == tl.scene.lights_root ? (uint32_t)IDENT_TLAS_LIGHTS : ~0u;
+    return own | (with_world ? (uint32_t)IDENT_TLAS_WORLD : 0u);
+}
+static bool ident_walk(const TraceLaunch& tl, uint32_t bits) { return (tl.ident_tlas & bits) == bits; }
+
 template <int MODE>
 static void launch_closest_impl(hipStream_t s, const TraceLaunch& tl, uint32_t root, const RayQueue& rq, const uint32_t* n_ptr, uint32_t cap_in,
                                 uint32_t* heads, const ClosestOut& out)
 {
+    const bool ident = ident_walk(tl, tlas_bits(tl, root, MODE == CLOSEST_LIGHTS));
     const bool spill = tl.scene.stack_entries > tl.scene.stack_lds;
     const dim3 block(tl.block_threads);
     const uint4* blob = (const uint4*)tl.blob;
     const size_t lds = trace_lds_bytes(tl);
     const ClosestKArgs ka{tl.scene, blob, rq.a, rq.b, n_ptr, heads, root, cap_in, out};
 #define PT_LAUNCH1(K) hipLaunchKernelGGL(K, dim3(resident_grid(K, tl, lds)), block, lds, s, ka)
-    if (tl.lds_scene && !spill) PT_LAUNCH1((k_closest<1, MODE, false>));
+    if (ident)
+    {
+        if (tl.lds_scene && !spill) PT_LAUNCH1((k_closest<1, MODE, false, true>));
+        else if (tl.lds_scene) PT_LAUNCH1((k_closest<1, MODE, true, true>));
+        else if (!spill) PT_LAUNCH1((k_closest<0, MODE, false, true>));
+        else PT_LAUNCH1((k_closest<0, MODE, true, true>));
+    }
+    else if (tl.lds_scene && !spill) PT_LAUNCH1((k_closest<1, MODE, false>));
     else if (tl.lds_scene) PT_LAUNCH1((k_closest<1, MODE, true>));
     else if (!spill) PT_LAUNCH1((k_closest<0, MODE, false>));
     else PT_LAUNCH1((k_closest<0, MODE, true>));
@@ -2191,12 +2268,20 @@
 static void launch_any_impl(hipStream_t s, const TraceLaunch& tl, uint32_t root, const RayQueue& rq, const uint32_t* n_ptr, uint32_t cap_in,
                             uint32_t* heads, uint32_t* occluded, f4* radiance = nullptr)
 {
+    const bool ident = ident_walk(tl, tlas_bits(tl, root, false));
     const size_t lds = trace_lds_bytes(tl);
     const bool spill = tl.scene.stack_entries > tl.scene.stack_lds;
     const dim3 block(tl.block_threads);
     const uint4* blob = (const uint4*)tl.blob;
 #define PT_LAUNCH(K) hipLaunchKernelGGL(K, dim3(resident_grid(K, tl, lds)), block, lds, s, tl.scene, blob, root, rq.a, rq.b, n_ptr, cap_in, heads, occluded, radiance)
-    if (tl.lds_scene && !spill) PT_LAUNCH((k_any<1, MODE, false>));
+    if (ident)
+    {
+        if (tl.lds_scene && !spill) PT_LAUNCH((k_any<1, MODE, false, true>));
+        else if (tl.lds_scene) PT_LAUNCH((k_any<1, MODE, true, true>));
+        else if (!spill) PT_LAUNCH((k_any<0, MODE, false, true>));
+        else PT_LAUNCH((k_any<0, MODE, true, true>));
+    }
+    else if (tl.lds_scene && !spill) PT_LAUNCH((k_any<1, MODE, false>));
     else if (tl.lds_scene) PT_LAUNCH((k_any<1, MODE, true>));
     else if (!spill) PT_LAUNCH((k_any<0, MODE, false>));
     else PT_LAUNCH((k_any<0, MODE, true>));
@@ -2282,7 +2367,14 @@
     const uint4* blob = (const uint4*)tl.blob;
     const FusedKArgs ka{tl.scene, blob, fa, wout, lout};
 #define PT_LAUNCH(K) hipLaunchKernelGGL(K, dim3(resident_grid(K, tl, lds)), block, lds, s, ka)
-    if (tl.lds_scene && !spill) PT_LAUNCH((k_trace_fused<1, false>));
+    if (ident_walk(tl, IDENT_TLAS_WORLD | IDENT_TLAS_LIGHTS))
+    {
+        if (tl.lds_scene && !spill) PT_LAUNCH((k_trace_fused<1, false, true>));
+        else if (tl.lds_scene) PT_LAUNCH((k_trace_fused<1, true, true>));
+        else if (!spill) PT_LAUNCH((k_trace_fused<0, false, true>));
+        else PT_LAUNCH((k_trace_fused<0, true, true>));
+    }
+    else if (tl.lds_scene && !spill) PT_LAUNCH((k_trace_fused<1, false>));
     else if (tl.lds_scene) PT_LAUNCH((k_trace_fused<1, true>));
     else if (!spill) PT_LAUNCH((k_trace_fused<0, false>));
     else PT_LAUNCH((k_trace_fused<0, true>));
@@ -2353,7 +2445,8 @@
     {
     case Q_TERMINAL: hipLaunchKernelGGL(k_shade_terminal, dim3(grid_blocks), dim3(256), 0, s, sv, rp, io, b); break;
     case Q_LAMBERT:
-        if (inl) hipLaunchKernelGGL((k_shade_surface<Q_LAMBERT, false, true>), dim3(surface_blocks), dim3(PT_SHADE_THREADS), lds, s, ka);
+        if (inl && PT_IDENT_SHADE && ident_walk(*tl, IDENT_TLAS_WORLD)) hipLaunchKernelGGL((k_shade_surface<Q_LAMBERT, false, true, true>), dim3(surface_blocks), dim3(PT_SHADE_THREADS), lds, s, ka);
+        else if (inl) hipLaunchKernelGGL((k_shade_surface<Q_LAMBERT, false, true>), dim3(surface_blocks), dim3(PT_SHADE_THREADS), lds, s, ka);
         else if (sv.has_volumes) hipLaunchKernelGGL((k_shade_surface<Q_LAMBERT, true>), dim3(surface_blocks), dim3(PT_SHADE_THREADS), 0, s, ka);
         else hipLaunchKernelGGL((k_shade_surface<Q_LAMBERT, false>), dim3(surface_blocks), dim3(PT_SHADE_THREADS), 0, s, ka);
         break;
diff --git a/path_tracer_amd/csrc/pt_scene.cpp b/path_tracer_amd/csrc/pt_scene.cpp
--- a/path_tracer_amd/csrc/pt_scene.cpp
+++ b/path_tracer_amd/csrc/pt_scene.cpp
@@ -730,7 +730,8 @@
             }
         });
     }
-    auto put_instances = [&](const HostTlas& t) {
+    auto put_instances = [&](const HostTlas& t, uint32_t ident_bit) {
+        bool all_identity = true;
         for (const HostInstance& hi : t.instances)
         {
             DInstance d;
@@ -760,12 +761,15 @@
             {
                 static const uint32_t ident[12] = {0x3f800000u, 0, 0, 0x80000000u, 0, 0x3f800000u, 0, 0x80000000u, 0, 0, 0x3f800000u, 0x80000000u};
                 if (std::memcmp(d.inv, ident, sizeof(ident)) == 0) d.qclass |= INSTANCE_IDENTITY;
+                else all_identity = false;
             }
             f.instances.push_back(d);
         }
+        if (all_identity) f.ident_tlas |= ident_bit;
     };
-    put_instances(world);
-    put_instances(lights);
+    f.ident_tlas = 0u;
+    put_instances(world, IDENT_TLAS_WORLD);
+    put_instances(lights, IDENT_TLAS_LIGHTS);
 
     std::vector<std::vector<uint32_t>> where(blas.size());
     for (size_t i = 0; i < blas.size(); ++i)
diff --git a/path_tracer_amd/csrc/pt_scene.h b/path_tracer_amd/csrc/pt_scene.h
--- a/path_tracer_amd/csrc/pt_scene.h
+++ b/path_tracer_amd/csrc/pt_scene.h
@@ -81,6 +81,7 @@
     uint32_t world_root = MISS_ID, lights_root = MISS_ID;
     uint32_t prim_bits = 0;
     uint32_t stack_entries = 0;
+    uint32_t ident_tlas = 0;
     float light_weight_sum = 0;
     bool has_volumes = false;
 };
diff --git a/path_tracer_amd/csrc/pt_types.h b/path_tracer_amd/csrc/pt_types.h
--- a/path_tracer_amd/csrc/pt_types.h
+++ b/path_tracer_amd/csrc/pt_types.h
@@ -72,6 +72,7 @@
 enum : uint32_t { Q_TERMINAL = 0, Q_LAMBERT = 1, Q_SPECULAR = 2, Q_DIELECTRIC = 3, Q_GGX = 4, Q_COUNT = 5 };
 enum : uint32_t { ENTRY_DEAD = 0x80000000u };
 enum : uint32_t { INSTANCE_IDENTITY = 0x100u };
+enum : uint32_t { IDENT_TLAS_WORLD = 1u, IDENT_TLAS_LIGHTS = 2u };
 
 struct Counters
 {
```

Result: faster. 14880 Mray/s (median of 6 runs) (+4.8%).
